# mit-acl/dpgo

Measured on AMD Instinct MI355X. Metric: rbcd_iterations_per_sec, higher is better.
Workload: dtype f64; 1 GPU; synthetic 3-D grid 50x50x40 (100000 poses, 293500 edges), init = perturbed truth; agents=1, agents_per_gpu=1, r=5, d=3, schedule=single agent, poses_per_agent=100000, nnzb_per_agent=687000

## Files before the change

### dpgo_amd/csrc/host.h

```cpp
#pragma once
#include "kernels.h"

#include <algorithm>
#include <atomic>
#include <chrono>
#include <condition_variable>
#include <functional>
#include <memory>
#include <pthread.h>
#include <sched.h>
#include <mutex>
#include <thread>
#include <cmath>
#include <cstdio>
#include <cstdlib>
#include <cstring>
#include <string>
#include <utility>
#include <vector>

#include "../../include/dpgo_hip.h"

using namespace dpgo;

namespace dpgo_host {


inline thread_local std::string g_err;

inline int fail(int code, const std::string& msg) {
  g_err = msg;
  return code;
}

#define HIPC(expr)                                                                              \
  do {                                                                                          \
    hipError_t e_ = (expr);                                                                     \
    if (e_ != hipSuccess)                                                                       \
      return fail(DPGO_ERR_HIP, std::string(#expr) + ": " + hipGetErrorString(e_) + " (" + __FILE__ + \
                                    ":" + std::to_string(__LINE__) + ")");                      \
  } while (0)

#define CHK(expr)                \
  do {                           \
    int rc_ = (expr);            \
    if (rc_ != DPGO_OK) return rc_; \
  } while (0)

#define DPGO_FOR_DR(M) M(2, 2) M(2, 3) M(2, 4) M(2, 5) M(3, 3) M(3, 4) M(3, 5) M(3, 6)

inline bool supported(int d, int r) {
#define M(dd, rr) \
  if (d == dd && r == rr) return true;
  DPGO_FOR_DR(M)
#undef M
  return false;
}

#define DPGO_CASE(dd, rr, ...)   \
  case (dd) * 16 + (rr): {       \
    constexpr int D = dd, R = rr; \
    __VA_ARGS__;                 \
  } break;
#define DISPATCH(d, r, ...)                                                                         \
  switch ((d) * 16 + (r)) {                                                                         \
    DPGO_CASE(2, 2, __VA_ARGS__) DPGO_CASE(2, 3, __VA_ARGS__) DPGO_CASE(2, 4, __VA_ARGS__)          \
    DPGO_CASE(2, 5, __VA_ARGS__) DPGO_CASE(3, 3, __VA_ARGS__) DPGO_CASE(3, 4, __VA_ARGS__)          \
    DPGO_CASE(3, 5, __VA_ARGS__) DPGO_CASE(3, 6, __VA_ARGS__)                                       \
    default:                                                                                        \
      return fail(DPGO_ERR_UNSUPPORTED, "unsupported (d, r)");                                      \
  }

#define LAUNCH_SPLIT(p, KERNEL, GRID, ...)                                                            \
  do {                                                                                                \
    if ((p)->split == 4)                                                                              \
      hipLaunchKernelGGL((KERNEL<D, R, 4>), dim3(GRID), dim3(kBlock), 0, (p)->stream, __VA_ARGS__);   \
    else if ((p)->split == 2)                                                                         \
      hipLaunchKernelGGL((KERNEL<D, R, 2>), dim3(GRID), dim3(kBlock), 0, (p)->stream, __VA_ARGS__);   \
    else                                                                                              \
      hipLaunchKernelGGL((KERNEL<D, R, 1>), dim3(GRID), dim3(kBlock), 0, (p)->stream, __VA_ARGS__);   \
  } while (0)

inline bool aligned8(const void* q) { return ((uintptr_t)q & 7) == 0; }
inline bool aligned16(const void* q) { return ((uintptr_t)q & 15) == 0; }

struct Bsr {
  int nrows = 0, ncols = 0, nnzb = 0;
  int32_t* rowptr = nullptr;
  int32_t* colidx = nullptr;
  double* vals = nullptr;
  BsrDev dev() const { return BsrDev{rowptr, colidx, vals}; }
};

inline int free_bsr(Bsr& m) {
  if (m.rowptr) HIPC(hipFree(m.rowptr));
  if (m.colidx) HIPC(hipFree(m.colidx));
  if (m.vals) HIPC(hipFree(m.vals));
  m = Bsr();
  return DPGO_OK;
}



#define DPGO_OPTIONS(X)                                                                                                  \
  X(split,             "DPGO_SPLIT",              0,  "lane groups per pose of the SpMM-family kernels: 1, 2, 4 (0: by size)")       \
  X(spmm_symmetric,    "DPGO_SPMM_SYMMETRIC",    -1,  "symmetric storage of Q for blocks beyond the Infinity Cache: 0 / 1")          \
  X(stream_nt,         "DPGO_STREAM_NT",         -1,  "non-temporal single-use operands in the tCG-step kernels: 0 / 1")             \
  X(outer_sym,         "DPGO_OUTER_SYM",          1,  "outer RTR iteration (k_grad / k_hess) reads the symmetric copy when tCG does") \
  X(tile_walk,         "DPGO_TILE_WALK",          1,  "symmetric-storage kernels walk each XCD's tiles breadth-first over the tile graph (0: index order)") \
  X(iter_graph,        "DPGO_ITER_GRAPH",         0,  "steady tCG iterations replayed from an instantiated hipGraph (measured slower)") \
  X(tcg_ahead,         "DPGO_TCG_AHEAD",          0,  "iterations the just-in-time feed stays ahead (0: 2 multilevel / 4 otherwise)") \
  X(grid_update,       "DPGO_GRID_UPDATE",        0,  "launch cap of k_tcg_update (0: resident count)")                              \
  X(grid_hess,         "DPGO_GRID_HESS",          0,  "launch cap of k_tcg_hess (0: resident count)")                                \
  X(grid_hess_sym,     "DPGO_GRID_HESS_SYM",      0,  "launch cap of k_tcg_hess_sym (0: resident count)")                            \
  X(grid_retract,      "DPGO_GRID_RETRACT",       0,  "launch cap of k_retract (0: 1024)")                                           \
  X(grid_outer_sym,    "DPGO_GRID_OUTER_SYM",     0,  "launch cap of k_grad / k_hess on the symmetric storage (0: resident count)")  \
  X(grid_spmm_sym,     "DPGO_GRID_SPMM_SYM",      0,  "launch cap of k_spmm_sym (0: resident count, at most 1024)")                  \
  X(grid_ml,           "DPGO_GRID_ML",            0,  "launch cap of the level-0 restriction / post-smoothing (0: resident count)")  \
  X(persist,           "DPGO_PERSIST",           -1,  "one-launch solve (k_rtr_persist) off / on whatever the size: 0 / 1")          \
  X(persist_max_poses, "DPGO_PERSIST_MAX_POSES",  0,  "largest block the one-launch solve takes (0: every block it can hold)")       \
  X(persist_split,     "DPGO_PERSIST_SPLIT",      0,  "lane groups per pose of the one-launch solve: 1, 4 (0: by size)")             \
  X(persist_mt,        "DPGO_PERSIST_MT",         0,  "tiles per workgroup of the one-launch solve: 1, 2 (0: by size)")              \
  X(additive_tiles,    "DPGO_ADDITIVE_TILES",     1,  "workgroup tiles per aggregate of the additive one-launch solve: 1, 2 (opt-in: blocks up to ~28 000 poses)") \
  X(poll_first,        "DPGO_POLL_FIRST",        -1,  "s_sleep units before the first sweep of the in-kernel all-reduce")            \
  X(poll_sleep,        "DPGO_POLL_SLEEP",        -1,  "s_sleep units between sweeps of the in-kernel all-reduce")                    \
  X(poll_first_pay,    "DPGO_POLL_FIRST_PAY",    -1,  "the same before the first sweep of a reduction that carries a payload")       \
  X(persist_verbose,   "DPGO_PERSIST_VERBOSE",    0,  "per-solve phase report of the one-launch solve on stderr")                    \
  X(hess_dma,          "DPGO_HESS_DMA",           0,  "k_tcg_hess_sym's own tiles by LDS-DMA: 1 = double-buffered, 2 waves / SIMD, 4 blocks in flight; 2 = 3 waves, 2 blocks") \
  X(setup_timing,      "DPGO_SETUP_TIMING",       0,  "section times of the hierarchy's symbolic set-up on stderr")                  \
  X(setup_threads,     "DPGO_SETUP_THREADS",      0,  "host threads of the hierarchy's symbolic set-up (0: min(8, cores); 1: serial)") \
  X(setup_pin,         "DPGO_SETUP_PIN",          1,  "set-up worker threads placed in the CPU group of the thread that first used them") \
  X(auto_cost_rule,    "DPGO_AUTO_COST_RULE",     1,  "DPGO_PRECOND_AUTO on coupled blocks: cost rule (0: tCG-budget hysteresis only)") \
  X(ml_graph,          "DPGO_ML_GRAPH",           1,  "graph aggregates in the default hierarchy (0: index runs)")                   \
  X(ml_graph_size,     "DPGO_ML_GRAPH_SIZE",      0,  "growth size of the default graph aggregates (0: by size)")                    \
  X(ml_growth_chunks,  "DPGO_ML_GROWTH_CHUNKS",   0,  "index ranges the graph aggregates grow and merge in (0: 8 from 65 536 poses, else 1)") \
  X(ml_ap,             "DPGO_ML_AP",              1,  "two-level post-smoothing through A P (0: gather through Q; index runs only)") \
  X(ml_dense_sym,      "DPGO_ML_DENSE_SYM",      -1,  "dense level from the packed lower triangle on the matrix cores: 0 / 1")       \
  X(ml_early_stop,     "DPGO_ML_EARLY_STOP",      1,  "tCG's residual test in the restriction kernel, one kernel early")             \
  X(ml_operator_bits,  "DPGO_ML_OPERATOR_BITS",   0,  "level-0 operator copies of the cycle on HBM-bound blocks: 32 / 64 (0: 32)")   \
  X(ml_vector_bits,    "DPGO_ML_VECTOR_BITS",     0,  "cycle-internal vectors (pre-smoothed iterate, kept residual) beside fp32 operator copies: 32 / 64 (0: 32)") \
  X(ml_dense_bits,     "DPGO_ML_DENSE_BITS",      0,  "dense level beside fp32 cycle vectors: 32 / 64 (0: 64 -- fp32 measured neutral)") \
  X(ml_setup_serial,   "DPGO_ML_SETUP_SERIAL",    0,  "one-thread-per-aggregate set-up kernels of round 3")                          \
  X(gj_mfma,           "DPGO_GJ_MFMA",            1,  "rank-64 updates of the dense inverse on the fp64 matrix cores")               \
  X(dense_chunk,       "DPGO_DENSE_CHUNK",        0,  "tiles per workgroup of k_dense_sym_apply (0: default)")                       \
  X(coarse_nodes,      "DPGO_COARSE_NODES",       0,  "nodes per workgroup of k_ml_coarse_prolong: 1-4 (0: by size)")                \
  X(coarse_grid,       "DPGO_COARSE_GRID",        0,  "launch cap of k_ml_coarse_prolong (0: default)")                              \
  X(coarse_nt,         "DPGO_COARSE_NT",         -1,  "non-temporal loads of the dense inverse: 0 / 1")
struct Options {
#define X(field, var, unset, text) int field = unset;
  DPGO_OPTIONS(X)
#undef X
};
inline Options& options_storage() {
  static Options o;
  return o;
}
inline void options_read(Options& o) {
  o = Options();
#define X(field, var, unset, text) \
  if (const char* e_ = std::getenv(var)) o.field = (*e_ == 0) ? 1 : std::atoi(e_);
  DPGO_OPTIONS(X)
#undef X
}
inline const Options& options() {
  static const bool once = (options_read(options_storage()), true);
  (void)once;
  return options_storage();
}
inline std::string options_describe() {
  const Options& o = options();
  std::string s;
#define X(field, var, unset, text) s += std::string(var) + "=" + std::to_string(o.field) + (o.field == (unset) ? "" : " [set]") + "  # " + text + "\n";
  DPGO_OPTIONS(X)
#undef X
  return s;
}

}
using namespace dpgo_host;

struct dpgo_problem_s {
  int r = 0, d = 0, n = 0, b = 0, T = 0;
  int device = 0;
  hipStream_t own_stream = nullptr;
  hipStream_t stream = nullptr;
  Bsr Q;
  Bsr C;
  double* G0 = nullptr;
  double* G = nullptr;
  bool has_G = false;
  double* dinv = nullptr;
  double dinv_shift = -1.0;
  double *x1 = nullptr, *x2 = nullptr, *g1 = nullptr, *g2 = nullptr, *eta = nullptr, *delta = nullptr,
         *Hd = nullptr, *rr = nullptr, *z = nullptr, *S1 = nullptr, *S2 = nullptr;
  struct MlLevel {
    int n = 0;
    int k = 0;
    int split = 1;
    Bsr A;
    int32_t* slot_row = nullptr;
    double *dinv = nullptr, *Pb = nullptr;
    double *r = nullptr, *x1 = nullptr, *x = nullptr;
    Bsr AP;
    double* res1 = nullptr;
    bool graph = false;
    int32_t *lab = nullptr, *agg_ptr = nullptr, *agg_mem = nullptr, *parent = nullptr, *pslot = nullptr;
    int32_t* mem_pos = nullptr;
    int32_t *seg_info = nullptr, *seg_ptr = nullptr;
    int nseg = 0;
    int32_t* tile_perm = nullptr;
    int perm_tile = 0;
    int merge_cap = 0;
    double* tbuf = nullptr;
    float *Pb32 = nullptr, *AP32 = nullptr;
    float *x1f = nullptr, *res1f = nullptr;
    AggMap agg() const { return AggMap{graph ? lab : nullptr, k}; }
  };
  std::vector<MlLevel> ml;
  std::vector<int32_t> h_rowptr, h_colidx;
  bool ml_symbolic = false, ml_ready = false, ml_user_ks = false;
  bool ml_additive_layout = false;
  struct AddPlan {
    int split = 0, tile = 0, S = 0, cap = 0, na = 0;
    bool graph = true;
  } add_plan;
  bool add_plan_known = false;
  int add_tiles = 0;
  struct AggCache {
    int S = 0, cap = 0;
    std::vector<int32_t> lab, ptr, mem, parent, pslot;
  } add_agg;
  double ml_omega = 0.7, ml_shift = 1e-1;
  double* ml_dense = nullptr;
  float* ml_dense32 = nullptr;
  double *ml_packed = nullptr, *ml_pd = nullptr, *ml_pt = nullptr;
  DenseChunk* ml_chunks = nullptr;
  int* ml_chunk_first = nullptr;
  int ml_nchunks = 0;
  bool ml_use_dense_sym() const {
    const int env = options().ml_dense_sym;
    if (!ml_use_ap() || ml_coarse_bits != 64 || !ml_packed || env == 0) return false;
    return env == 1 || ml_lda >= 3072;
  }
  int ml_coarse_bits = 64;
  int ml_operator_bits = 32;
  bool ml_ops32_ready = false;
  bool ml_ops32_suspend = false;
  bool ml_ops32_wanted() const { return ml_operator_bits == 32 && tcg_sym && split == 1 && ml_use_ap() && sym.uvalsT != nullptr; }
  bool ml_ops32_active() const { return !ml_ops32_suspend && ml_ops32_wanted() && ml_ops32_ready; }
  bool ml_vec32_active() const { return ml_ops32_active() && options().ml_vector_bits != 64; }
  bool coarse32_active() const {
    return ml_coarse_bits == 32 || (ml_vec32_active() && !ml_use_dense_sym() && options().ml_dense_bits == 32);
  }
  int ml_lda = 0;
  double *ml_W = nullptr, *ml_Rx = nullptr;
  bool auto_ml = false, auto_decided = false;
  struct AutoCost {
    long long jac_units = 0;
    int ref = 0;
    int state = 0;
    int backoff = 0;
    int switches = 0;
    int last_used = -1, last_products = 0;
    int uj = 10, ua = 18;
  } auto_cost;
  void auto_decide() {
    if (!auto_decided) {
      auto_ml = !(has_G || C.nnzb > 0);
      auto_decided = true;
      auto_cost = AutoCost();
    }
  }
  bool ml_use_ap() const {
    const bool off = options().ml_ap == 0;
    return ml.size() == 2 && ml[0].AP.vals != nullptr && (!off || ml[0].graph);
  }
  struct SymQ {
    int nu = 0, nl = 0;
    int32_t *urow = nullptr, *ucol = nullptr, *usrc = nullptr, *lrow = nullptr, *lcol = nullptr, *lslot = nullptr,
            *lsrc = nullptr;
    double* uvalsT = nullptr;
    float* uvalsT32 = nullptr;
    int32_t* tord = nullptr;
    int* flag = nullptr;
    bool symbolic = false;
    bool pattern_ok = false;
    bool ready = false;
    bool values_ok = false;
    BsrSymDev dev() const { return BsrSymDev{urow, ucol, uvalsT, lrow, lcol, lslot, tord}; }
    BsrSymDev32 dev32() const { return BsrSymDev32{urow, ucol, uvalsT32, lrow, lcol, lslot, tord}; }
  } sym;
  int spmm_variant = DPGO_SPMM_AUTO;
  bool tcg_sym = false;
  int cap_hs = kMaxGrid;
  bool sym_wanted() const {
    if (spmm_variant == DPGO_SPMM_PLAIN || split != 1) return false;
    if (spmm_variant == DPGO_SPMM_SYMMETRIC) return true;
    if (options().spmm_symmetric >= 0) return options().spmm_symmetric != 0;
    return beyond_cache();
  }
  size_t loop_extra_bytes = 0;
  bool want_stream_nt() const {
    return options().stream_nt >= 0 ? options().stream_nt != 0 : beyond_cache();
  }
  bool beyond_cache() const {
    return sizeof(double) * ((size_t)Q.nnzb * b * b + 8 * (size_t)n * T) + sizeof(int32_t) * (size_t)Q.nnzb + loop_extra_bytes >
           ((size_t)256 << 20);
  }
  bool persist = false;
  int persist_share = 1;
  int persist_wgs = 0, persist_split = 0, persist_mt = 0;
  int persist_reserved = 0;
  bool persist_failed_once = false;
  bool stream_nt = false;
  bool persist_add = false;
  bool persist_stream_ordered = false;
  struct Pending {
    bool active = false;
    bool launched = false;
    dpgo_ropt_params resolved{};
    bool is_auto = false;
    const double* dinv = nullptr;
    double* own_x1 = nullptr;
    double* staged_x = nullptr;
    std::chrono::steady_clock::time_point t0;
    dpgo_ropt_result result{};
  } pending;
  PersistCtrl* pctrl = nullptr;
  bool pctrl_dirty = true;
  unsigned long long* pgran = nullptr;
  unsigned gran_cleared_at = 0;
  PersistCtrl* hctrl = nullptr;
  double* partials = nullptr;
  DevState* dstate = nullptr;
  DevState* hstate = nullptr;
  unsigned long long* hflag = nullptr;
  unsigned gen = 0;
  bool saw_rtr_stop = false;
  struct IterGraph {
    hipGraphExec_t exec = nullptr;
    unsigned long long key = 0;
  } iter_graph[2];
  bool capturing = false;
  bool iter_graph_failed = false;
  unsigned launch_gen() const { return capturing ? 0u : gen; }
  int em = 0;
  int32_t *e_p1 = nullptr, *e_p2 = nullptr, *c_ptr = nullptr, *c_edge = nullptr;
  double *e_R = nullptr, *e_t = nullptr, *e_kappa = nullptr, *e_tau = nullptr, *e_w = nullptr, *e_rsq = nullptr,
         *q_base = nullptr;
  uint8_t *e_fixed = nullptr, *c_kind = nullptr, *e_role = nullptr;
  int32_t* e_slot = nullptr;
  int32_t *g_ptr = nullptr, *g_edge = nullptr;
  uint8_t* g_kind = nullptr;
  double* c_base = nullptr;
  int n_shared_edges = 0;
  int* e_counts = nullptr;
  EdgeDev edges() const {
    return EdgeDev{e_p1, e_p2, e_R, e_t, e_kappa, e_tau, e_fixed, e_role, e_slot, e_w, e_rsq, em};
  }
  int cur = 0;
  size_t vec_bytes() const { return (size_t)n * T * sizeof(double); }
  double* pE() const { return partials; }
  double* pA() const { return partials + 1 * kPartialCap * kNP; }
  double* pB() const { return partials + 2 * kPartialCap * kNP; }
  double* pH() const { return partials + 3 * kPartialCap * kNP; }
  int grid() const {
    const int P = (64 / b) * kWaves;
    int tiles = (n + P - 1) / P;
    if (tiles < 1) tiles = 1;
    return tiles < cap_u ? tiles : cap_u;
  }
  int cap_u = kMaxGrid, cap_h = kMaxGrid;
  int cap_u_ml = kMaxGrid;
  int grid_u(bool ml_mode) const {
    const int P = (64 / b) * kWaves;
    const int tiles = std::max(1, (n + P - 1) / P);
    return std::min(tiles, ml_mode ? cap_u_ml : cap_u);
  }
  bool zr_from_post = false;
  int nb_zr() const { return zr_from_post ? grid_post() : grid(); }
  int split = 1;
  int grid_s() const {
    const int P = (64 / (b * split)) * kWaves;
    int tiles = (n + P - 1) / P;
    if (tiles < 1) tiles = 1;
    const int cap = tcg_sym ? cap_hs : cap_h;
    return tiles < cap ? tiles : cap;
  }
  int cap_restrict = kMaxGrid, cap_post = kMaxGrid;
  int grid_tiles(int cap) const {
    const int P = (64 / (b * split)) * kWaves;
    int tiles = (n + P - 1) / P;
    if (tiles < 1) tiles = 1;
    return tiles < cap ? tiles : cap;
  }
  int grid_restrict() const { return grid_tiles(cap_restrict); }
  int grid_post() const { return grid_tiles(cap_post); }
  int cap_outer_sym = kMaxGrid;
  int nb_grad = 0, nb_hess = 0;
  int grid_outer_sym() const {
    const int P = (64 / b) * kWaves;
    const int tiles = std::max(1, (n + P - 1) / P);
    return std::min(tiles, cap_outer_sym);
  }
  int cap_spmm_sym = kMaxGrid;
  int grid_spmm_sym() const {
    const int P = (64 / b) * kWaves;
    const int tiles = std::max(1, (n + P - 1) / P);
    return std::min(tiles, cap_spmm_sym);
  }
  int grid_spmm() const {
    const int P = (64 / (b * split)) * kWaves;
    int tiles = (n + P - 1) / P;
    if (tiles < 1) tiles = 1;
    return tiles < kMaxGrid ? tiles : kMaxGrid;
  }
  int grid_flat() const {
    size_t total = (size_t)n * T;
    size_t g = (total + kBlock - 1) / kBlock;
    if (g < 1) g = 1;
    return g < (size_t)kMaxGrid ? (int)g : kMaxGrid;
  }
};

namespace dpgo_host {

struct Counters {
  int spmm = 0;
  bool vcycle_for_additive = false;
};

template <class Tp>
inline int upload(Tp** dst, const Tp* src, size_t count, hipStream_t s) {
  HIPC(hipMalloc(dst, sizeof(Tp) * (count > 0 ? count : 1)));
  if (count > 0) HIPC(hipMemcpyAsync(*dst, src, sizeof(Tp) * count, hipMemcpyHostToDevice, s));
  return DPGO_OK;
}

class TaskPool {
 public:
  struct Batch {
    std::function<void(int)> fn;
    int count = 0;
    std::atomic<int> next{0}, done{0};
  };
  using Job = std::shared_ptr<Batch>;
  static TaskPool& get() {
    static TaskPool* pool = new TaskPool();
    return *pool;
  }
  Job submit(int count, std::function<void(int)> fn, int max_threads) {
    Job b = std::make_shared<Batch>();
    b->fn = std::move(fn);
    b->count = count;
    const int helpers = std::max(0, std::min(count, max_threads - 1));
    if (helpers > 0) {
      {
        std::lock_guard<std::mutex> lk(mu_);
        while ((int)nworkers_ < std::min(kMaxWorkers, std::max(helpers, (int)nworkers_))) {
          const int id = (int)nworkers_;
          std::thread([this, id] {
            pin(id);
            loop();
          }).detach();
          ++nworkers_;
        }
        for (int k = 0; k < helpers; ++k) queue_.push_back(b);
      }
      cv_.notify_all();
    }
    return b;
  }
  void wait(const Job& b) {
    if (!b) return;
    help(*b);
    while (b->done.load(std::memory_order_acquire) < b->count) std::this_thread::yield();
  }
  void run(int count, const std::function<void(int)>& fn, int max_threads) {
    if (count <= 0) return;
    if (count == 1 || max_threads <= 1) {
      for (int k = 0; k < count; ++k) fn(k);
      return;
    }
    wait(submit(count, fn, max_threads));
  }
  void warm(int threads) {
    bool expected = false;
    if (threads <= 1 || !warmed_.compare_exchange_strong(expected, true)) return;
    std::thread([this, threads] { wait(submit(threads - 1, [](int) {}, threads)); }).detach();
  }

 private:
  static constexpr int kMaxWorkers = 15;
  int home_cpu_ = -1;
  void pin(int) {
    if (!pin_enabled() || home_cpu_ < 0) return;
    cpu_set_t allowed, want;
    CPU_ZERO(&allowed);
    CPU_ZERO(&want);
    if (sched_getaffinity(0, sizeof(allowed), &allowed) != 0) return;
    const int lo = home_cpu_ & ~7;
    int cnt = 0;
    for (int c = lo; c < lo + 8; ++c)
      if (c < CPU_SETSIZE && CPU_ISSET(c, &allowed)) CPU_SET(c, &want), ++cnt;
    if (cnt >= 2) (void)pthread_setaffinity_np(pthread_self(), sizeof(want), &want);
  }
  static bool pin_enabled() { return options().setup_pin != 0; }
  TaskPool() { home_cpu_ = sched_getcpu(); }
  static void help(Batch& b) {
    for (;;) {
      const int k = b.next.fetch_add(1, std::memory_order_relaxed);
      if (k >= b.count) return;
      b.fn(k);
      b.done.fetch_add(1, std::memory_order_release);
    }
  }
  void loop() {
    for (;;) {
      Job b;
      {
        std::unique_lock<std::mutex> lk(mu_);
        cv_.wait(lk, [this] { return !queue_.empty(); });
        b = std::move(queue_.front());
        queue_.erase(queue_.begin());
      }
      help(*b);
    }
  }
  std::mutex mu_;
  std::condition_variable cv_;
  std::vector<Job> queue_;
  unsigned nworkers_ = 0;
  std::atomic<bool> warmed_{false};
};
struct JobGuard {
  TaskPool::Job job;
  ~JobGuard() { TaskPool::get().wait(job); }
};

struct TmpDev {
  std::vector<void*> ptrs;
  ~TmpDev() {
    for (auto q : ptrs) (void)hipFree(q);
  }
  int alloc(double** out, size_t bytes) {
    HIPC(hipMalloc(out, bytes));
    ptrs.push_back(*out);
    return DPGO_OK;
  }
};

template <typename T>
inline int sym_upload(T** dst, const std::vector<T>& v, hipStream_t stream) {
  HIPC(hipMalloc(dst, sizeof(T) * std::max<size_t>(1, v.size())));
  if (!v.empty()) HIPC(hipMemcpyAsync(*dst, v.data(), sizeof(T) * v.size(), hipMemcpyHostToDevice, stream));
  return DPGO_OK;
}

struct PersistGeo {
  int split = 0, mt = 0, wgs = 0, slots = 0;
};

enum { RUN_FULL = 0, RUN_BEGIN = 1, RUN_END = 2 };

int set_device(dpgo_problem_s* p);
int upload_bsr(Bsr& m, int nrows, int ncols, int nnzb, int b, const int32_t* rowptr, const int32_t* colidx,
               const double* vals, hipStream_t s);
int validate_bsr(int nrows, int ncols, int nnzb, const int32_t* rowptr, const int32_t* colidx, bool need_diag);
int build_dinv(dpgo_problem_s* p, double shift);
int poll_state(dpgo_problem_s* p);
int push_state(dpgo_problem_s* p);
void sym_free(dpgo_problem_s* p);
int sym_symbolic_setup(dpgo_problem_s* p);
int sym_ensure(dpgo_problem_s* p, bool* usable);
int launch_spmm_sym(dpgo_problem_s* p, const BsrSymDev& M, const double* V, const double* Gadd, double* OUT);
int launch_spmm(dpgo_problem_s* p, const Bsr& M, const double* V, const double* Gadd, double* OUT, int nrows = -1,
                bool plain_only = false);
bool outer_sym_enabled();
int launch_grad(dpgo_problem_s* p, const double* X, double* RG, double* S, double* EG,
                const DevState* st = nullptr, bool sym = false);
int launch_hess(dpgo_problem_s* p, const double* X, const double* S, const double* V, const double* Gdot,
                double* HV, double* partials, const DevState* st, int check_tcg, bool sym = false);
int launch_retract(dpgo_problem_s* p, const double* X, const double* eta, double scale, double* X2,
                   const DevState* st);
int launch_rtr_update(dpgo_problem_s* p);
int launch_precond(dpgo_problem_s* p, const double* X, const double* V, const double* dinv, double* Z);
int launch_rtr_begin(dpgo_problem_s* p, double tol, double Delta0, double Dmax, int max_inner, int tiny);
int check_ready(dpgo_problem_s* p);
int h2d(dpgo_problem_s* p, double* dst, const double* src);
int d2h(dpgo_problem_s* p, double* dst, const double* src);

int ml_tile(int b, int split);
int additive_tile(const dpgo_problem_s* p);
int ml_level_split(int n);
int ml_default_graph_size(int n, int b);
std::vector<int> ml_default_ks(int n, int b, int split0);
void ml_free(dpgo_problem_s* p);
int ml_graph_aggregates(const std::vector<int32_t>& rowptr, const std::vector<int32_t>& colidx, int n, int S,
                        std::vector<int32_t>& lab, std::vector<int32_t>& ptr, std::vector<int32_t>& mem,
                        std::vector<int32_t>& parent, std::vector<int32_t>& pslot);
int ml_merge_small_aggregates(const std::vector<int32_t>& rowptr, const std::vector<int32_t>& colidx, int n, int S, int cap,
                              std::vector<int32_t>& lab, std::vector<int32_t>& ptr, std::vector<int32_t>& mem,
                              std::vector<int32_t>& parent, std::vector<int32_t>& pslot);
int ml_symbolic_setup(dpgo_problem_s* p, const std::vector<int>& ks_in, int perm_tile = 0);
int setup_threads();
int flat_grid(size_t items);
bool gj_use_mfma();
int dense_spd_inverse(hipStream_t s, double* M, int lda, double* W, double* Rx, bool mfma);
int ml_numeric_setup(dpgo_problem_s* p);
std::vector<int> ml_current_ks(const dpgo_problem_s* p);
const dpgo_problem_s::AddPlan& additive_plan(dpgo_problem_s* p);
int additive_split_of(const dpgo_problem_s* p);
int additive_tiles(const dpgo_problem_s* p);
int additive_mt_of(const dpgo_problem_s* p);
int ml_ensure(dpgo_problem_s* p, double shift, bool additive = false);
int ml_ops32_ensure(dpgo_problem_s* p);
int persist_capacity(int device);
int launch_coarse_prolong(dpgo_problem_s* p, const dpgo_problem_s::MlLevel& L, const dpgo_problem_s::MlLevel& C,
                          const DevState* gate, double* xc_out = nullptr);
int launch_dense_sym(dpgo_problem_s* p, const dpgo_problem_s::MlLevel& C, const DevState* gate);
int launch_ml_restrict0(dpgo_problem_s* p, const double* r, const DevState* gate, int g0, bool stop_check = false);
int launch_ml_post_ap(dpgo_problem_s* p, const double* Xdev, const double* r, double* z, double* pout, const DevState* gate);
int launch_ml_tail(dpgo_problem_s* p, const double* Xdev, const double* r, double* z, double* pout,
                   const DevState* gate, bool stop_check = false);
int launch_ml_apply(dpgo_problem_s* p, const double* Xdev, const double* v, double* z);

int launch_tcg_update(dpgo_problem_s* p, const double* dinv, int first, double* z_out = nullptr,
                      double ml_omega = 0.0);
int launch_tcg_hess(dpgo_problem_s* p, int first);
int launch_tcg_hess_with(dpgo_problem_s* p, const DevState* sin, DevState* sout, int first, unsigned long long* hflag,
                         unsigned gen);
int resolve_tcg_storage(dpgo_problem_s* p);
int persist_capacity(int device);
bool persist_reserve(dpgo_problem_s* p, int slots, int limit);
void persist_release(dpgo_problem_s* p);
bool additive_available(dpgo_problem_s* p);
PersistGeo persist_geometry(const dpgo_problem_s* p, int free_slots, int share = 1, bool additive = false);
bool additive_lds_fits(const dpgo_problem_s* p, int split, int mt, int na);
int launch_rtr_persistent(dpgo_problem_s* p, const dpgo_ropt_params* prm, const double* dinv, bool* used, bool additive);
void persist_report(dpgo_problem_s* p);
int rtr_outer_iteration(dpgo_problem_s* p, const dpgo_ropt_params* prm, const double* dinv, Counters& cnt,
                        bool poll_at_end);
int auto_units_jacobi(dpgo_problem_s* p);
int auto_units_additive(dpgo_problem_s* p);
void auto_update(dpgo_problem_s* p, const dpgo_ropt_params* prm, int used, int products);
int run_optimize(dpgo_problem_s* p, const dpgo_ropt_params* prm, dpgo_ropt_result* res, int phase = RUN_FULL);
int tune_launch_caps(dpgo_problem_s* p);
int tune_persist(dpgo_problem_s* p);

int free_edges(dpgo_problem_s* p);
int rebuild_vals(dpgo_problem_s* p, int nnzb, const int32_t* cptr, const int32_t* cedge, const uint8_t* ckind,
                 const double* base, double sign, double* out);
int rebuild_Q_from_weights(dpgo_problem_s* p, const double* base, double sign, double* out);
int rebuild_C_from_weights(dpgo_problem_s* p, const double* base, double sign, double* out);
int refresh_after_weights(dpgo_problem_s* p);

}
```

### dpgo_amd/csrc/kernels/multilevel.h

```cpp
#pragma once


struct AggMap {
  const int32_t* lab;
  int k;
  __device__ __forceinline__ int of(int i) const { return lab ? lab[i] : i / k; }
};

template <int D, int R>
__global__ __launch_bounds__(kBlock) void k_ml_presmooth(const double* __restrict__ V, const double* __restrict__ dinv,
                                                         double omega, double* __restrict__ OUT,
                                                         const DevState* __restrict__ gate, int n) {
  using GEO = Geo<D, R>;
  if (gate && (gate->tcg_done || gate->rtr_stop)) return;
  __shared__ double sm[kWaves][GEO::G][GEO::T];
  const LaneId L = lane_id<D>();
  const int ntiles = (n + GEO::P - 1) / GEO::P;
  const TileIter ti_ = tile_iter(ntiles);
  for (int tile = ti_.first; tile < ti_.last; tile += ti_.step) {
    const int i = tile * GEO::P + L.wave * GEO::G + L.g;
    const bool ok = (L.g < GEO::G) && (i < n);
    const size_t off = (size_t)i * GEO::T + L.c * R;
    double* vs = ok ? &sm[L.wave][L.g][0] : nullptr;
    double v[R], z[R];
    if (ok) {
      load_col<R>(V + off, v);
      store_col<R>(vs + L.c * R, v);
    }
    wave_sync();
    if (ok) {
      jacobi_col<D, R>(vs, dinv + (size_t)i * GEO::BB + L.c * GEO::B, z);
#pragma unroll
      for (int a = 0; a < R; ++a) z[a] *= omega;
      store_col<R>(OUT + off, z);
    }
    wave_sync();
  }
}

struct TcgStopCheck {
  DevState* state = nullptr;
  const double* pin = nullptr;
  int nb = 0;
  unsigned long long* hflag = nullptr;
  unsigned gen = 0;
};
template <int D, int R, int SPLIT>
struct RestrictWaves {
  static constexpr int kMin = (SPLIT == 1 && D == 3 && R <= 5) ? DPGO_RESTRICT_WAVES : 1;
};
template <int D, int R, int SPLIT, class MAT = BsrDev, class PT = double, class XT = double>
__global__ __launch_bounds__(kBlock) __attribute__((amdgpu_waves_per_eu(RestrictWaves<D, R, SPLIT>::kMin, 8))) void k_ml_restrict(MAT A, const XT* __restrict__ x1,
                                                        const double* __restrict__ r, const PT* __restrict__ Pb,
                                                        double shift, int k, double* __restrict__ rc,
                                                        float* __restrict__ rc32,
                                                        const double* __restrict__ dinv_next, double omega,
                                                        double* __restrict__ x1c, const DevState* gate,
                                                        int n, XT* __restrict__ res_out = nullptr,
                                                        double* __restrict__ tbuf = nullptr,
                                                        const int32_t* __restrict__ tpos = nullptr,
                                                        TcgStopCheck stop = TcgStopCheck()) {
  using GEO = Geo<D, R, SPLIT>;
  DPGO_TL_TILES_DECL;
  if (gate && (gate->tcg_done || gate->rtr_stop)) return;
  DPGO_STAMP_ENTRY_IN(g_tl_restrict);
  __shared__ double res_s[kWaves][GEO::G][GEO::T];
  __shared__ double t_s[GEO::P][GEO::T];
  const LaneId L = lane_id<D, SPLIT>();
  const int ntiles = (n + GEO::P - 1) / GEO::P;
  const TileIter ti_ = tile_iter(ntiles);
  if (stop.state && blockIdx.x == gridDim.x - 1) {
    double rr_sum[1];
    load_partials<1>(stop.pin, stop.nb, rr_sum, &t_s[0][0]);
    if (threadIdx.x == 0) {
      const DevState* st = stop.state;
      const double norm_r = sqrt(rr_sum[0]), nr0 = st->norm_r0, theta = st->theta, kappa = st->kappa;
      const double pw = (theta == 1.0) ? nr0 : pow(nr0, theta);
      const int j = st->tcg_j;
      if (j >= st->min_inner && norm_r <= nr0 * (pw < kappa ? pw : kappa)) {
        stop.state->tcg_status = (kappa < pw) ? TCG_LCON : TCG_SCON;
        stop.state->tcg_done = 1;
        if (stop.hflag) {
          const unsigned g_ = stop.gen ? stop.gen : (unsigned)st->pad0;
          const unsigned long long w = ((unsigned long long)g_ << 32) |
                                       ((unsigned long long)((unsigned)j & 0xFFFFFFu) << 8) | 1ull;
          __hip_atomic_store(stop.hflag, w, __ATOMIC_RELAXED, __HIP_MEMORY_SCOPE_SYSTEM);
        }
      }
    }
    __syncthreads();
  }
  DPGO_STAMP_AT_IN(g_tl_restrict, 1);
  for (int tk = ti_.first; tk < ti_.last; tk += ti_.step) {
    DPGO_STAMP_TILE_IN(g_tl_restrict, 0);
    const int tile = tile_of(A, tk);
    const int lp = L.wave * GEO::G + L.g;
    const int i = tile * GEO::P + lp;
    const bool okp = (L.g < GEO::G) && (i < n);
    const bool ok = okp && (L.s == 0);
    const size_t off = (size_t)i * GEO::T + L.c * R;
    double h[R];
    q_gather<D, R, SPLIT>(A, x1, i, L.s, L.c, okp, h);
    DPGO_TL_USE(h[0]);
    DPGO_STAMP_TILE_IN(g_tl_restrict, 1);
    if constexpr (SPLIT == 1 && Span<D, R, 1>::kOk && DPGO_CYCLE_SPAN) {
      const int p0 = tile * GEO::P + L.wave * GEO::G;
      const int npose = (n - p0) < GEO::G ? (n - p0) : GEO::G;
      const int valid = npose > 0 ? npose * GEO::T : 0;
      const size_t base = (size_t)p0 * GEO::T;
      double* rw = &res_s[L.wave][0][0];
      span_to_lds<D, R>(r + base, rw, valid);
      span_to_lds<D, R>(x1 + base, &t_s[L.wave * GEO::G][0], valid);
      wave_sync();
      if (ok) {
        const double* rr = &res_s[L.wave][L.g][L.c * R];
        const double* xr = &t_s[lp][L.c * R];
#pragma unroll
        for (int a = 0; a < R; ++a) h[a] = rr[a] - h[a] - shift * xr[a];
        store_col<R>(&res_s[L.wave][L.g][L.c * R], h);
      }
      wave_sync();
      if (res_out) span_from_lds<D, R>(res_out + base, rw, valid);
    } else {
      if (ok) {
        XT xr[R];
        double rr[R];
#pragma unroll
        for (int a = 0; a < R; ++a) xr[a] = x1[off + a];
        load_col<R>(r + off, rr);
#pragma unroll
        for (int a = 0; a < R; ++a) h[a] = rr[a] - h[a] - shift * (double)xr[a];
        store_col<R>(&res_s[L.wave][L.g][L.c * R], h);
        if (res_out) store_col_t<R>(res_out + off, h);
      }
      wave_sync();
    }
    DPGO_STAMP_TILE_IN(g_tl_restrict, 2);
    if (L.s == 0 && L.g < GEO::G) {
      double t[R];
#pragma unroll
      for (int a = 0; a < R; ++a) t[a] = 0.0;
      if (ok) {
        const PT* __restrict__ pb = Pb + (size_t)i * GEO::BB;
#pragma unroll
        for (int cc = 0; cc < GEO::B; ++cc) {
          const double pv = (double)pb[cc * GEO::B + L.c];
#pragma unroll
          for (int a = 0; a < R; ++a) t[a] = fma(pv, res_s[L.wave][L.g][cc * R + a], t[a]);
        }
      }
      store_col<R>(&t_s[lp][L.c * R], t);
    }
    DPGO_STAMP_TILE_IN(g_tl_restrict, 3);
    if (tbuf) {
      wave_sync();
      if (ok) {
        const int info = tpos[i];
        if (info >= 0) {
          const int len = info & 31;
          double acc[R];
#pragma unroll
          for (int a = 0; a < R; ++a) acc[a] = t_s[lp][L.c * R + a];
          for (int m = 1; m < len; ++m) {
#pragma unroll
            for (int a = 0; a < R; ++a) acc[a] += t_s[lp + m][L.c * R + a];
          }
          store_col<R>(tbuf + (size_t)(info >> 5) * GEO::T + L.c * R, acc);
        }
      }
      wave_sync();
      DPGO_STAMP_TILE_IN(g_tl_restrict, 4);
      DPGO_TILE_NEXT;
      continue;
    }
    __syncthreads();
    const int mstep = (k >= 16) ? 8 : 1;
    if (mstep == 8) {
      const int nseg = (k + 7) / 8, nagg = GEO::P / k;
      for (int tsk = threadIdx.x; tsk < nagg * nseg * GEO::T; tsk += kBlock) {
        const int e = tsk % GEO::T, sg = (tsk / GEO::T) % nseg, ag = tsk / (GEO::T * nseg);
        const int row0 = ag * k + sg * 8;
        double sacc = t_s[row0][e];
        for (int m = 1; m < 8 && sg * 8 + m < k; ++m) sacc += t_s[row0 + m][e];
        t_s[row0][e] = sacc;
      }
      __syncthreads();
    }
    const bool head = ok && (i % k) == 0;
    double acc[R];
    if (head) {
#pragma unroll
      for (int a = 0; a < R; ++a) acc[a] = 0.0;
      for (int m = 0; m < k && lp + m < GEO::P; m += mstep) {
#pragma unroll
        for (int a = 0; a < R; ++a) acc[a] += t_s[lp + m][L.c * R + a];
      }
      int cr = L.c * R;
      asm volatile("" : "+v"(cr));
      if (rc32) {
#pragma unroll
        for (int a = 0; a < R; ++a) rc32[(size_t)(i / k) * GEO::T + cr + a] = (float)acc[a];
      } else {
        store_col<R>(rc + (size_t)(i / k) * GEO::T + cr, acc);
      }
    }
    __syncthreads();
    if (dinv_next) {
      if (head) store_col<R>(&t_s[lp][L.c * R], acc);
      wave_sync();
      if (head) {
        double z[R];
        jacobi_col<D, R>(&t_s[lp][0], dinv_next + (size_t)(i / k) * GEO::BB + L.c * GEO::B, z);
#pragma unroll
        for (int a = 0; a < R; ++a) z[a] *= omega;
        store_col<R>(x1c + (size_t)(i / k) * GEO::T + L.c * R, z);
      }
      __syncthreads();
    }
  }
}

template <int D, int R>
__global__ __launch_bounds__(kBlock) void k_ml_agg_sum(const double* __restrict__ t, const int32_t* __restrict__ agg_ptr,
                                                       int na, double* __restrict__ rc, float* __restrict__ rc32,
                                                       const DevState* __restrict__ gate) {
  constexpr int T = (D + 1) * R, NG = kBlock / T;
  if (gate && (gate->tcg_done || gate->rtr_stop)) return;
  __shared__ double part[NG][T];
  const int e = threadIdx.x % T, g = threadIdx.x / T;
  for (int a = blockIdx.x; a < na; a += gridDim.x) {
    const int m0 = agg_ptr[a], m1 = agg_ptr[a + 1];
    if (g < NG) {
      double acc = 0.0;
#pragma unroll 8
      for (int m = m0 + g; m < m1; m += NG) acc += t[(size_t)m * T + e];
      part[g][e] = acc;
    }
    __syncthreads();
    if (threadIdx.x < T) {
      double acc = part[0][threadIdx.x];
#pragma unroll
      for (int q = 1; q < NG; ++q) acc += part[q][threadIdx.x];
      if (rc32)
        rc32[(size_t)a * T + threadIdx.x] = (float)acc;
      else
        rc[(size_t)a * T + threadIdx.x] = acc;
    }
    __syncthreads();
  }
}

#ifndef DPGO_COARSE_WAVES
#define DPGO_COARSE_WAVES 2
#endif
#ifndef DPGO_COARSE_UNROLL
#define DPGO_COARSE_UNROLL 1
#endif
template <int D, int R, int NODES, class MT>
__global__ __launch_bounds__(kBlock) __attribute__((amdgpu_waves_per_eu(DPGO_COARSE_WAVES, DPGO_COARSE_WAVES))) void k_ml_coarse_prolong(const MT* __restrict__ M, int lda,
                                                              const MT* __restrict__ rc,
                                                              const double* __restrict__ x1,
                                                              const double* __restrict__ Pb, int k,
                                                              double* __restrict__ x, const DevState* __restrict__ gate,
                                                              int n, int nc, double* __restrict__ xc_out = nullptr,
                                                              int stream_hint = 1) {
  constexpr int B = D + 1, T = B * R, BB = B * B, NR = NODES * B;
  constexpr int CPL = 16 / (int)sizeof(MT);
  struct alignas(16) Pack {
    MT v[CPL];
  };
  if (gate && (gate->tcg_done || gate->rtr_stop)) return;
  constexpr int NV = B * R, SEG = 8, SEGLEN = kBlock / SEG;
  __shared__ double xc_s[NR][R];
  __shared__ double all_s[NV][kBlock];
  __shared__ double seg_s[NV][SEG];
  const int lane = threadIdx.x & 63, wave = threadIdx.x >> 6;
  const int N = nc * B;
  const int ngroups = (nc + NODES - 1) / NODES;
  for (int grp = blockIdx.x; grp < ngroups; grp += gridDim.x) {
    const int a0 = grp * NODES;
    {
      const MT* __restrict__ m = M + (size_t)(a0 * B) * lda;
      double acc[NR][R];
#pragma unroll
      for (int c = 0; c < NR; ++c)
#pragma unroll
        for (int q = 0; q < R; ++q) acc[c][q] = 0.0;
      const int npack = (N + CPL - 1) / CPL;
      const dbl2* __restrict__ rc2 = reinterpret_cast<const dbl2*>(rc);
      struct alignas(16) RPack {
        MT v[CPL * R];
      };
      auto stream_rows = [&](auto nt) {
#pragma unroll DPGO_COARSE_UNROLL
        for (int j = wave * 64 + lane; j < npack; j += kBlock) {
          Pack mv[NR];
#pragma unroll
          for (int c = 0; c < NR; ++c) {
            const dbl2* src = reinterpret_cast<const dbl2*>(m + (size_t)c * lda + CPL * j);
            dbl2 raw;
            if constexpr (decltype(nt)::value)
              raw = __builtin_nontemporal_load(src);
            else
              raw = *src;
            __builtin_memcpy(&mv[c], &raw, 16);
          }
          RPack rp;
          if (CPL * j + CPL <= N) {
            dbl2 raw[R];
#pragma unroll
            for (int q = 0; q < R; ++q) raw[q] = rc2[(size_t)j * R + q];
            __builtin_memcpy(&rp, raw, sizeof(rp));
          } else {
#pragma unroll
            for (int e = 0; e < CPL * R; ++e)
              rp.v[e] = (CPL * j + e / R < N) ? rc[(size_t)(CPL * j) * R + e] : (MT)0;
          }
          double rv[CPL * R];
#pragma unroll
          for (int e = 0; e < CPL * R; ++e) rv[e] = (double)rp.v[e];
#pragma unroll
          for (int c = 0; c < NR; ++c) {
#pragma unroll
            for (int q = 0; q < R; ++q) {
#pragma unroll
              for (int cc = 0; cc < CPL; ++cc) acc[c][q] = fma((double)mv[c].v[cc], rv[cc * R + q], acc[c][q]);
            }
          }
        }
      };
      if (stream_hint)
        stream_rows(std::true_type{});
      else
        stream_rows(std::false_type{});
#pragma unroll
      for (int nd = 0; nd < NODES; ++nd) {
#pragma unroll
        for (int c = 0; c < B; ++c)
#pragma unroll
          for (int q = 0; q < R; ++q) all_s[c * R + q][threadIdx.x] = acc[nd * B + c][q];
        __syncthreads();
        for (int tsk = threadIdx.x; tsk < NV * SEG; tsk += kBlock) {
          const int v = tsk / SEG, sg = tsk % SEG;
          double sum = 0.0;
#pragma unroll 8
          for (int e = 0; e < SEGLEN; ++e)
            sum += all_s[v][sg * SEGLEN + ((e + tsk) & (SEGLEN - 1))];
          seg_s[v][sg] = sum;
        }
        __syncthreads();
        if (threadIdx.x < NV) {
          double sum = seg_s[threadIdx.x][0];
#pragma unroll
          for (int sg = 1; sg < SEG; ++sg) sum += seg_s[threadIdx.x][sg];
          xc_s[nd * B + threadIdx.x / R][threadIdx.x % R] = sum;
        }
      }
    }
    __syncthreads();
    if (xc_out) {
      if (threadIdx.x < NR * R && a0 * B + threadIdx.x / R < N)
        xc_out[(size_t)(a0 * B) * R + threadIdx.x] = xc_s[threadIdx.x / R][threadIdx.x % R];
      __syncthreads();
      continue;
    }
    for (int tsk = threadIdx.x; tsk < NODES * k * B; tsk += kBlock) {
      const int i = a0 * k + tsk / B, c = tsk % B;
      if (i < n) {
        const int an = (tsk / B) / k;
        const double* __restrict__ pb = Pb + (size_t)i * BB + c * B;
        const size_t off = (size_t)i * T + c * R;
#pragma unroll
        for (int q = 0; q < R; ++q) {
          double v = x1[off + q];
#pragma unroll
          for (int cc = 0; cc < B; ++cc) v = fma(pb[cc], xc_s[an * B + cc][q], v);
          x[off + q] = v;
        }
      }
    }
    __syncthreads();
  }
}

template <int D, int R, int SPLIT>
__global__ __launch_bounds__(kBlock) void k_ml_post_mid(BsrDev A, const double* __restrict__ xv,
                                                        const double* __restrict__ r, const double* __restrict__ dinv,
                                                        double omega, const double* __restrict__ x1f,
                                                        const double* __restrict__ Pbf, int kf, double* __restrict__ xf,
                                                        int nf, const DevState* __restrict__ gate, int n) {
  using GEO = Geo<D, R, SPLIT>;
  if (gate && (gate->tcg_done || gate->rtr_stop)) return;
  __shared__ double sm[kWaves][2][GEO::G][GEO::T];
  const LaneId L = lane_id<D, SPLIT>();
  const int ntiles = (n + GEO::P - 1) / GEO::P;
  const TileIter ti_ = tile_iter(ntiles);
  for (int tile = ti_.first; tile < ti_.last; tile += ti_.step) {
    const int i = tile * GEO::P + L.wave * GEO::G + L.g;
    const bool okp = (L.g < GEO::G) && (i < n);
    const bool ok = okp && (L.s == 0);
    const size_t off = (size_t)i * GEO::T + L.c * R;
    double* vs = ok ? &sm[L.wave][0][L.g][0] : nullptr;
    double* zs = ok ? &sm[L.wave][1][L.g][0] : nullptr;
    double h[R], xr[R], z[R];
    spmm_col<D, R, SPLIT>(A.rowptr, A.colidx, A.vals, xv, i, L.s, L.c, okp, h);
    if (ok) {
      double rr[R];
      load_col<R>(xv + off, xr);
      load_col<R>(r + off, rr);
#pragma unroll
      for (int a = 0; a < R; ++a) h[a] = rr[a] - h[a];
      store_col<R>(vs + L.c * R, h);
    }
    wave_sync();
    if (ok) {
      jacobi_col<D, R>(vs, dinv + (size_t)i * GEO::BB + L.c * GEO::B, z);
#pragma unroll
      for (int a = 0; a < R; ++a) z[a] = fma(omega, z[a], xr[a]);
      store_col<R>(zs + L.c * R, z);
    }
    wave_sync();
    if (ok) {
      for (int m = 0; m < kf; ++m) {
        const int fi = i * kf + m;
        if (fi < nf) {
          const double* __restrict__ pb = Pbf + (size_t)fi * GEO::BB + L.c * GEO::B;
          const size_t foff = (size_t)fi * GEO::T + L.c * R;
          double out[R];
          load_col<R>(x1f + foff, out);
#pragma unroll
          for (int cc = 0; cc < GEO::B; ++cc) {
            const double pv = pb[cc];
#pragma unroll
            for (int a = 0; a < R; ++a) out[a] = fma(pv, zs[cc * R + a], out[a]);
          }
          store_col<R>(xf + foff, out);
        }
      }
    }
    wave_sync();
  }
}

#ifndef DPGO_POST_RR_LDS
#define DPGO_POST_RR_LDS 1
#endif
#ifndef DPGO_POST_WAVES
#define DPGO_POST_WAVES 4
#endif
template <int D, int R, int SPLIT, class MAT = BsrDev>
__global__ __launch_bounds__(kBlock) __attribute__((amdgpu_waves_per_eu(SPLIT == 1 ? DPGO_POST_WAVES : 1))) void k_ml_post(MAT Q, const double* __restrict__ X,
                                                    const double* __restrict__ xv, const double* __restrict__ r,
                                                    const double* __restrict__ dinv, double omega, double shift,
                                                    double* __restrict__ Z, double* __restrict__ pout,
                                                    const DevState* __restrict__ gate, int n) {
  using GEO = Geo<D, R, SPLIT>;
  if (gate && (gate->tcg_done || gate->rtr_stop)) return;
  __shared__ double sm[kWaves][3][GEO::G][GEO::T];
  __shared__ double red[kWaves * kNP];
  const LaneId L = lane_id<D, SPLIT>();
  const int ntiles = (n + GEO::P - 1) / GEO::P;
  const TileIter ti_ = tile_iter(ntiles);
  double part[2] = {0.0, 0.0};
  for (int tk = ti_.first; tk < ti_.last; tk += ti_.step) {
    const int tile = tile_of(Q, tk);
    const int i = tile * GEO::P + L.wave * GEO::G + L.g;
    const bool okp = (L.g < GEO::G) && (i < n);
    const bool ok = okp && (L.s == 0);
    const size_t off = (size_t)i * GEO::T + L.c * R;
    double* ys = ok ? &sm[L.wave][0][L.g][0] : nullptr;
    double* vs = ok ? &sm[L.wave][1][L.g][0] : nullptr;
    double* zs = ok ? &sm[L.wave][2][L.g][0] : nullptr;
    double h[R], xr[R], rr[R], z[R];
    q_gather<D, R, SPLIT>(Q, xv, i, L.s, L.c, okp, h);
    if (ok) {
      double x[R];
      load_col<R>(X + off, x);
      load_col<R>(xv + off, xr);
      load_col<R>(r + off, rr);
#pragma unroll
      for (int a = 0; a < R; ++a) {
        h[a] = rr[a] - h[a] - shift * xr[a];
        part[0] = fma(rr[a], rr[a], part[0]);
      }
      store_col<R>(ys + L.c * R, x);
      store_col<R>(vs + L.c * R, h);
    }
    wave_sync();
    if (ok) {
      jacobi_col<D, R>(vs, dinv + (size_t)i * GEO::BB + L.c * GEO::B, z);
#pragma unroll
      for (int a = 0; a < R; ++a) z[a] = fma(omega, z[a], xr[a]);
      store_col<R>(zs + L.c * R, z);
    }
    wave_sync();
    if (ok) {
      double out[R], s[D];
      proj_col<D, R>(ys, zs, L.c, z, out, s);
      store_col<R>(Z + off, out);
#pragma unroll
      for (int a = 0; a < R; ++a) part[1] = fma(out[a], rr[a], part[1]);
    }
    wave_sync();
  }
  if (pout) store_partials<2>(part, pout, red);
}

template <int D, int R, int SPLIT, class VT = double, class RT = VT>
__global__ __launch_bounds__(kBlock) __attribute__((amdgpu_waves_per_eu(SPLIT == 1 ? DPGO_POST_WAVES : 1))) void k_ml_post_ap(BsrDevT<VT> AP, const double* __restrict__ X,
                                                       const double* __restrict__ r, const RT* __restrict__ res1,
                                                       const double* __restrict__ xc, const VT* __restrict__ Pb, AggMap am,
                                                       const double* __restrict__ dinv, double omega,
                                                       double* __restrict__ Z, double* __restrict__ pout,
                                                       const DevState* __restrict__ gate, int n) {
  using GEO = Geo<D, R, SPLIT>;
  DPGO_TL_TILES_DECL;
  if (gate && (gate->tcg_done || gate->rtr_stop)) return;
  DPGO_STAMP_ENTRY_IN(g_tl_post);
  __shared__ double sm[kWaves][3][GEO::G][GEO::T];
  __shared__ double red[kWaves * kNP];
  const LaneId L = lane_id<D, SPLIT>();
  const int ntiles = (n + GEO::P - 1) / GEO::P;
  const TileIter ti_ = tile_iter(ntiles);
  double part[2] = {0.0, 0.0};
  for (int tile = ti_.first; tile < ti_.last; tile += ti_.step) {
    DPGO_STAMP_TILE_IN(g_tl_post, 0);
    const int i = tile * GEO::P + L.wave * GEO::G + L.g;
    const bool okp = (L.g < GEO::G) && (i < n);
    const bool ok = okp && (L.s == 0);
    const size_t off = (size_t)i * GEO::T + L.c * R;
    double* ys = ok ? &sm[L.wave][0][L.g][0] : nullptr;
    double* vs = ok ? &sm[L.wave][1][L.g][0] : nullptr;
    double* zs = ok ? &sm[L.wave][2][L.g][0] : nullptr;
    double h[R], rr[R], xcol[R], z[R], dr[GEO::B];
    spmm_col<D, R, SPLIT>(AP.rowptr, AP.colidx, AP.vals, xc, i, L.s, L.c, okp, h);
    DPGO_TL_USE(h[0]);
    DPGO_STAMP_TILE_IN(g_tl_post, 1);
    constexpr bool kSpan = (SPLIT == 1) && Span<D, R, 1>::kOk && DPGO_CYCLE_SPAN;
    [[maybe_unused]] int valid = 0;
    [[maybe_unused]] size_t base = 0;
    if constexpr (kSpan) {
      const int p0 = tile * GEO::P + L.wave * GEO::G;
      const int npose = (n - p0) < GEO::G ? (n - p0) : GEO::G;
      valid = npose > 0 ? npose * GEO::T : 0;
      base = (size_t)p0 * GEO::T;
      span_to_lds<D, R>(X + base, &sm[L.wave][0][0][0], valid);
      span_to_lds<D, R>(r + base, &sm[L.wave][1][0][0], valid);
      span_to_lds<D, R>(res1 + base, &sm[L.wave][2][0][0], valid);
      if (ok) {
#pragma unroll
        for (int q = 0; q < GEO::B; ++q) dr[q] = dinv[(size_t)i * GEO::BB + L.c * GEO::B + q];
      }
      wave_sync();
      if (ok) {
#pragma unroll
        for (int a = 0; a < R; ++a) {
          rr[a] = vs[L.c * R + a];
          h[a] = zs[L.c * R + a] - h[a];
          part[0] = fma(rr[a], rr[a], part[0]);
        }
        store_col<R>(zs + L.c * R, h);
      }
    } else if (ok) {
      double x[R], rs[R];
      load_col<R>(X + off, x);
      load_col<R>(r + off, rr);
      load_col_t<R>(res1 + off, rs);
#pragma unroll
      for (int q = 0; q < GEO::B; ++q) dr[q] = dinv[(size_t)i * GEO::BB + L.c * GEO::B + q];
#pragma unroll
      for (int a = 0; a < R; ++a) {
        h[a] = rs[a] - h[a];
        part[0] = fma(rr[a], rr[a], part[0]);
      }
      store_col<R>(ys + L.c * R, x);
      store_col<R>(vs + L.c * R, rr);
      store_col<R>(zs + L.c * R, h);
    }
    wave_sync();
    DPGO_STAMP_TILE_IN(g_tl_post, 2);
    if (ok) {
      double x1c[R], zc[R];
      jacobi_col<D, R>(vs, dr, x1c);
      jacobi_col<D, R>(zs, dr, zc);
      const VT* __restrict__ pb = Pb + (size_t)i * GEO::BB + L.c * GEO::B;
      const double* __restrict__ xa = xc + (size_t)am.of(i) * GEO::T;
#pragma unroll
      for (int a = 0; a < R; ++a) xcol[a] = omega * x1c[a];
#pragma unroll
      for (int cc = 0; cc < GEO::B; ++cc) {
        const double pv = (double)pb[cc];
#pragma unroll
        for (int a = 0; a < R; ++a) xcol[a] = fma(pv, xa[cc * R + a], xcol[a]);
      }
#pragma unroll
      for (int a = 0; a < R; ++a) z[a] = fma(omega, zc[a], xcol[a]);
      DPGO_TL_USE(z[0]);
    }
    DPGO_STAMP_TILE_IN(g_tl_post, 3);
    wave_sync();
    if (ok) store_col<R>(zs + L.c * R, z);
    wave_sync();
    DPGO_STAMP_TILE_IN(g_tl_post, 4);
    if (ok) {
      double out[R], sdummy[D];
      proj_col<D, R>(ys, zs, L.c, z, out, sdummy);
      if constexpr (DPGO_POST_RR_LDS) {
#pragma unroll
        for (int a = 0; a < R; ++a) part[1] = fma(out[a], vs[L.c * R + a], part[1]);
      } else {
#pragma unroll
        for (int a = 0; a < R; ++a) part[1] = fma(out[a], rr[a], part[1]);
      }
      if constexpr (kSpan)
        store_col<R>(vs + L.c * R, out);
      else
        store_col<R>(Z + off, out);
    }
    wave_sync();
// ... 417 lines not shown
```

### dpgo_amd/csrc/multilevel.hip

```cpp
#include "host.h"

namespace dpgo_host {

int ml_tile(int b, int split) { return (64 / (b * split)) * kWaves; }
int additive_tile(const dpgo_problem_s* p) { return ml_tile(p->b, 4); }
int ml_level_split(int n) { return n < 40000 ? 4 : 1; }

constexpr int kMlDense = 3200, kMlDenseMax = 6400;
constexpr int kMlGraphMax = 512, kMlGraphUnknownsPerPose = 1600;
int ml_default_graph_size(int n, int b) {
  if (options().ml_graph == 0) return 0;
  if (options().ml_graph_size >= 2) return options().ml_graph_size;
  const long long S = std::max<long long>(4, ((long long)n * b + kMlGraphUnknownsPerPose - 1) / kMlGraphUnknownsPerPose);
  return S <= kMlGraphMax ? (int)S : 0;
}
constexpr int kMlMergeFrom = 12, kMlMergedUnknownsPerPose = 2200;
std::vector<int> ml_default_ks(int n, int b, int split0) {
  if (const int S = ml_default_graph_size(n, b)) {
    const bool forced = options().ml_graph_size >= 2;
    if (!forced && S >= kMlMergeFrom) {
      const int Sm = (int)(((long long)n * b + kMlMergedUnknownsPerPose - 1) / kMlMergedUnknownsPerPose);
      const int cap = Sm + Sm / 2;
      if (cap <= kMlGraphMax) return std::vector<int>{-Sm, -cap};
    }
    return std::vector<int>{-S};
  }
  std::vector<int> ks;
  int cur = n, split = split0;
  for (int guard = 0; guard < 16; ++guard) {
    const int P = ml_tile(b, split);
    int pick = 0;
    for (int limit : {kMlDense, kMlDenseMax}) {
      for (int k = 4; k <= P && !pick; ++k)
        if (P % k == 0 && (long long)((cur + k - 1) / k) * b <= limit) pick = k;
      if (pick) break;
    }
    if (pick) {
      ks.push_back(pick);
      return ks;
    }
    int k = 2;
    for (int c = 2; c <= 8; ++c)
      if (P % c == 0) k = c;
    ks.push_back(k);
    cur = (cur + k - 1) / k;
    split = ml_level_split(cur);
  }
  return ks;
}

void ml_free(dpgo_problem_s* p) {
  p->ml_additive_layout = false;
  for (auto& L : p->ml) {
    free_bsr(L.A);
    free_bsr(L.AP);
    void* ptrs[] = {L.slot_row, L.dinv, L.Pb, L.r, L.x1, L.x, L.res1, L.lab, L.agg_ptr, L.agg_mem, L.parent, L.pslot, L.tbuf, L.tile_perm, L.mem_pos,
                    L.seg_info, L.seg_ptr, L.Pb32, L.AP32, L.x1f, L.res1f};
    for (void* q : ptrs)
      if (q) (void)hipFree(q);
  }
  p->ml.clear();
  void* ptrs[] = {p->ml_dense, p->ml_W, p->ml_Rx, p->ml_dense32, p->ml_packed, p->ml_pd, p->ml_pt, p->ml_chunks,
                  p->ml_chunk_first};
  for (void* q : ptrs)
    if (q) (void)hipFree(q);
  p->ml_dense = p->ml_W = p->ml_Rx = nullptr;
  p->ml_dense32 = nullptr;
  p->ml_packed = p->ml_pd = p->ml_pt = nullptr;
  p->ml_chunks = nullptr;
  p->ml_chunk_first = nullptr;
  p->ml_nchunks = 0;
  p->ml_lda = 0;
  p->ml_symbolic = p->ml_ready = false;
  p->ml_ops32_ready = false;
}

int ml_growth_chunks(int n) {
  const int forced = options().ml_growth_chunks;
  if (forced > 0) return std::max(1, std::min(forced, std::max(1, n / 64)));
  return n >= 65536 ? 8 : 1;
}
namespace {
int grow_range(const std::vector<int32_t>& rowptr, const std::vector<int32_t>& colidx, int lo, int hi, int S,
               std::vector<int32_t>& lab, std::vector<int32_t>& ptr, std::vector<int32_t>& mem,
               std::vector<int32_t>& parent, std::vector<int32_t>& pslot) {
  mem.clear();
  mem.reserve(hi - lo);
  ptr.assign(1, 0);
  int na = 0;
  for (int s = lo; s < hi; ++s) {
    if (lab[s] >= 0) continue;
    const size_t first = mem.size();
    lab[s] = na;
    mem.push_back(s);
    for (size_t head = first; head < mem.size() && (int)(mem.size() - first) < S; ++head) {
      const int u = mem[head];
      for (int t = rowptr[u]; t < rowptr[u + 1] && (int)(mem.size() - first) < S; ++t) {
        const int v = colidx[t];
        if (v < lo || v >= hi || lab[v] >= 0) continue;
        lab[v] = na;
        parent[v] = u;
        pslot[v] = t;
        mem.push_back(v);
      }
    }
    ptr.push_back((int32_t)mem.size());
    ++na;
  }
  return na;
}

int merge_range(const std::vector<int32_t>& rowptr, const std::vector<int32_t>& colidx, int lo, int hi, int S, int cap,
                std::vector<int32_t>& lab, std::vector<int32_t>& ptr, std::vector<int32_t>& mem,
                std::vector<int32_t>& parent, std::vector<int32_t>& pslot) {
  const int na = (int)ptr.size() - 1;
  const int n = hi - lo;
  std::vector<std::vector<int32_t>> members(na);
  for (int a = 0; a < na; ++a) members[a].assign(mem.begin() + ptr[a], mem.begin() + ptr[a + 1]);
  std::vector<int> cnt(na, 0);
  std::vector<int> touched;
  for (bool changed = true; changed;) {
    changed = false;
    for (int a = 0; a < na; ++a) {
      if (members[a].empty() || 2 * (int)members[a].size() > S) continue;
      touched.clear();
      for (int i : members[a])
        for (int t = rowptr[i]; t < rowptr[i + 1]; ++t) {
          const int v = colidx[t];
          if (v < lo || v >= hi) continue;
          const int c = lab[v];
          if (c == a) continue;
          if (cnt[c]++ == 0) touched.push_back(c);
        }
      std::sort(touched.begin(), touched.end());
      int best = -1, best_n = 0;
      for (int c : touched) {
        if ((int)(members[c].size() + members[a].size()) <= cap && cnt[c] > best_n) best = c, best_n = cnt[c];
        cnt[c] = 0;
      }
      if (best >= 0) {
        members[best].insert(members[best].end(), members[a].begin(), members[a].end());
        for (int i : members[a]) lab[i] = best;
        members[a].clear();
        changed = true;
      }
    }
  }
  std::vector<char> grew(na, 0);
  for (int a = 0; a < na; ++a)
    if (!members[a].empty() && (int)members[a].size() != ptr[a + 1] - ptr[a]) grew[a] = 1;
  std::vector<int32_t> first_member(na, -1);
  for (int i = hi - 1; i >= lo; --i) first_member[lab[i]] = i;
  std::vector<int> alive;
  for (int a = 0; a < na; ++a)
    if (!members[a].empty()) alive.push_back(a);
  std::sort(alive.begin(), alive.end(), [&](int x, int y) { return first_member[x] < first_member[y]; });
  std::vector<int32_t> sorted_mem, sorted_ptr(na + 1, 0);
  {
    for (int a = 0; a < na; ++a) sorted_ptr[a + 1] = sorted_ptr[a] + (grew[a] ? (int32_t)members[a].size() : 0);
    sorted_mem.resize(sorted_ptr[na]);
    std::vector<int32_t> fill(sorted_ptr.begin(), sorted_ptr.end() - 1);
    for (int i = lo; i < hi; ++i)
      if (grew[lab[i]]) sorted_mem[fill[lab[i]]++] = i;
  }
  std::vector<int32_t> new_lab(n, -1), new_mem;
  std::vector<int32_t> old_parent(parent.begin() + lo, parent.begin() + hi), old_pslot(pslot.begin() + lo, pslot.begin() + hi);
  std::fill(parent.begin() + lo, parent.begin() + hi, -1);
  std::fill(pslot.begin() + lo, pslot.begin() + hi, 0);
  new_mem.reserve(n);
  std::vector<int32_t> new_ptr(1, 0);
  for (size_t k = 0; k < alive.size(); ++k) {
    const int a = alive[k];
    if (!grew[a]) {
      for (int m = ptr[a]; m < ptr[a + 1]; ++m) {
        const int v = mem[m];
        new_lab[v - lo] = (int32_t)k;
        parent[v] = old_parent[v - lo];
        pslot[v] = old_pslot[v - lo];
        new_mem.push_back(v);
      }
      new_ptr.push_back((int32_t)new_mem.size());
      continue;
    }
    for (int q = sorted_ptr[a]; q < sorted_ptr[a + 1]; ++q) {
      const int root = sorted_mem[q];
      if (new_lab[root - lo] >= 0) continue;
      size_t head = new_mem.size();
      new_lab[root - lo] = (int32_t)k;
      new_mem.push_back(root);
      for (; head < new_mem.size(); ++head) {
        const int u = new_mem[head];
        for (int t = rowptr[u]; t < rowptr[u + 1]; ++t) {
          const int v = colidx[t];
          if (v < lo || v >= hi || lab[v] != a || new_lab[v - lo] >= 0) continue;
          new_lab[v - lo] = (int32_t)k;
          parent[v] = u;
          pslot[v] = t;
          new_mem.push_back(v);
        }
      }
    }
    new_ptr.push_back((int32_t)new_mem.size());
  }
  mem.swap(new_mem);
  ptr.swap(new_ptr);
  std::copy(new_lab.begin(), new_lab.end(), lab.begin() + lo);
  return (int)alive.size();
}
}

template <class F>
void parallel_ranges(int n, int chunks, F&& fn);
int setup_threads();

int ml_grow_and_merge(const std::vector<int32_t>& rowptr, const std::vector<int32_t>& colidx, int n, int S, int cap,
                      bool do_grow, std::vector<int32_t>& lab, std::vector<int32_t>& ptr, std::vector<int32_t>& mem,
                      std::vector<int32_t>& parent, std::vector<int32_t>& pslot, int chunks) {
  chunks = std::max(1, std::min(chunks, std::max(1, n)));
  if (do_grow) {
    lab.assign(n, -1);
    parent.assign(n, -1);
    pslot.assign(n, 0);
  }
  struct Part {
    std::vector<int32_t> ptr, mem;
    int na = 0;
  };
  std::vector<Part> parts(chunks);
  auto bound = [&](int c) { return (int)((long long)n * c / chunks); };
  if (!do_grow) {
    const int na_in = (int)ptr.size() - 1;
    std::vector<int> first_agg(chunks + 1, na_in);
    bool split_ok = chunks > 1;
    if (split_ok) {
      int c = 0;
      first_agg[0] = 0;
      for (int a = 0; a < na_in && split_ok; ++a) {
        if (ptr[a + 1] <= ptr[a]) { split_ok = false; break; }
        int lo_m = n, hi_m = -1;
        for (int m = ptr[a]; m < ptr[a + 1]; ++m) lo_m = std::min(lo_m, (int)mem[m]), hi_m = std::max(hi_m, (int)mem[m]);
        while (c + 1 < chunks && lo_m >= bound(c + 1)) first_agg[++c] = a;
        if (lo_m < bound(c) || hi_m >= bound(c + 1)) split_ok = false;
      }
      while (c + 1 < chunks) first_agg[++c] = na_in;
      first_agg[chunks] = na_in;
    }
    if (!split_ok) {
      chunks = 1;
      parts.resize(1);
      parts[0].ptr = ptr;
      parts[0].mem = mem;
      parts[0].na = na_in;
    } else {
      for (int c = 0; c < chunks; ++c) {
        const int a0 = first_agg[c], a1 = first_agg[c + 1];
        Part& P = parts[c];
        P.na = a1 - a0;
        P.ptr.assign(1, 0);
        for (int a = a0; a < a1; ++a) P.ptr.push_back(ptr[a + 1] - ptr[a0]);
        P.mem.assign(mem.begin() + ptr[a0], mem.begin() + ptr[a1]);
        if (a0 > 0)
          for (int i = bound(c); i < bound(c + 1); ++i) lab[i] -= a0;
      }
    }
  }
  const bool timing_ = options().setup_timing > 1;
  const auto tA = std::chrono::steady_clock::now();
  std::vector<double> tch(chunks, 0.0);
  parallel_ranges(chunks, std::min(chunks, setup_threads()), [&](int, int c0, int c1) {
    for (int c = c0; c < c1; ++c) {
      const auto t0 = std::chrono::steady_clock::now();
      Part& P = parts[c];
      const int lo = bound(c), hi = bound(c + 1);
      if (do_grow) P.na = grow_range(rowptr, colidx, lo, hi, S, lab, P.ptr, P.mem, parent, pslot);
      if (cap > 0) P.na = merge_range(rowptr, colidx, lo, hi, S, cap, lab, P.ptr, P.mem, parent, pslot);
      tch[c] = 1e3 * std::chrono::duration<double>(std::chrono::steady_clock::now() - t0).count();
    }
  });
  const auto tB = std::chrono::steady_clock::now();
  std::vector<int> agg_off(chunks + 1, 0);
  std::vector<size_t> mem_off(chunks + 1, 0);
  for (int c = 0; c < chunks; ++c) agg_off[c + 1] = agg_off[c] + parts[c].na, mem_off[c + 1] = mem_off[c] + parts[c].mem.size();
  const int na = agg_off[chunks];
  mem.resize(mem_off[chunks]);
  ptr.assign((size_t)na + 1, 0);
  parallel_ranges(chunks, std::min(chunks, setup_threads()), [&](int, int c0, int c1) {
    for (int c = c0; c < c1; ++c) {
      const Part& P = parts[c];
      if (agg_off[c] > 0)
        for (int i = bound(c); i < bound(c + 1); ++i) lab[i] += agg_off[c];
      for (int a = 0; a < P.na; ++a) ptr[(size_t)agg_off[c] + a + 1] = (int32_t)(mem_off[c] + P.ptr[a + 1]);
      if (!P.mem.empty()) std::memcpy(mem.data() + mem_off[c], P.mem.data(), sizeof(int32_t) * P.mem.size());
    }
  });
  if (timing_) {
    std::fprintf(stderr, "dpgo_hip: grow / merge (%d ranges): parallel section %.3f ms, join %.3f ms; per range:", chunks,
                 1e3 * std::chrono::duration<double>(tB - tA).count(),
                 1e3 * std::chrono::duration<double>(std::chrono::steady_clock::now() - tB).count());
    for (double t : tch) std::fprintf(stderr, " %.3f", t);
    std::fprintf(stderr, "\n");
  }
  return na;
}
int ml_graph_aggregates(const std::vector<int32_t>& rowptr, const std::vector<int32_t>& colidx, int n, int S,
                        std::vector<int32_t>& lab, std::vector<int32_t>& ptr, std::vector<int32_t>& mem,
                        std::vector<int32_t>& parent, std::vector<int32_t>& pslot) {
  return ml_grow_and_merge(rowptr, colidx, n, S, 0, true, lab, ptr, mem, parent, pslot, ml_growth_chunks(n));
}
int ml_merge_small_aggregates(const std::vector<int32_t>& rowptr, const std::vector<int32_t>& colidx, int n, int S, int cap,
                              std::vector<int32_t>& lab, std::vector<int32_t>& ptr, std::vector<int32_t>& mem,
                              std::vector<int32_t>& parent, std::vector<int32_t>& pslot) {
  return ml_grow_and_merge(rowptr, colidx, n, S, cap, false, lab, ptr, mem, parent, pslot, ml_growth_chunks(n));
}

int setup_threads() {
  const int want = options().setup_threads;
  if (want > 0) return std::min(want, 64);
  const unsigned hw = std::thread::hardware_concurrency();
  return (int)std::max(1u, std::min(8u, hw ? hw : 1u));
}
template <class F>
void parallel_ranges(int n, int chunks, F&& fn) {
  chunks = std::max(1, std::min(chunks, n > 0 ? n : 1));
  TaskPool::get().run(chunks, [&](int c) {
    fn(c, (int)((long long)n * c / chunks), (int)((long long)n * (c + 1) / chunks));
  }, setup_threads());
}
template <class F>
void pattern_by_ranges(int n, int threads, int grain, size_t reserve_hint, F&& row, std::vector<int32_t>& rowptr_out,
                       std::vector<int32_t>& col_out) {
  const int chunks = std::max(1, std::min(threads, n / grain + 1));
  std::vector<std::vector<int32_t>> cols(chunks), cnt(chunks);
  parallel_ranges(n, chunks, [&](int c, int lo, int hi) {
    auto& cc = cols[c];
    auto& nn = cnt[c];
    cc.reserve(reserve_hint / chunks + 16);
    nn.resize(hi - lo);
    for (int i = lo; i < hi; ++i) {
      const size_t first = cc.size();
      row(c, i, cc);
      nn[i - lo] = (int32_t)(cc.size() - first);
    }
  });
  rowptr_out.assign(n + 1, 0);
  size_t total = 0;
  for (auto& cc : cols) total += cc.size();
  col_out.resize(total);
  std::vector<size_t> base(chunks + 1, 0);
  for (int c = 0; c < chunks; ++c) base[c + 1] = base[c] + cols[c].size();
  parallel_ranges(chunks, chunks, [&](int, int c0, int c1) {
    for (int c = c0; c < c1; ++c) {
      const int lo = (int)((long long)n * c / chunks);
      if (!cols[c].empty()) std::memcpy(col_out.data() + base[c], cols[c].data(), sizeof(int32_t) * cols[c].size());
      size_t at = base[c];
      for (size_t k = 0; k < cnt[c].size(); ++k) {
        at += cnt[c][k];
        rowptr_out[lo + k + 1] = (int32_t)at;
      }
    }
  });
}

void ml_ap_pattern(const std::vector<int32_t>& rowptr, const std::vector<int32_t>& colidx, const std::vector<int32_t>& lab,
                   int n, std::vector<int32_t>& arow, std::vector<int32_t>& acol) {
  pattern_by_ranges(n, setup_threads(), 1024, colidx.size(), [&](int, int i, std::vector<int32_t>& out) {
    const size_t first = out.size();
    for (int t = rowptr[i]; t < rowptr[i + 1]; ++t) out.push_back(lab[colidx[t]]);
    std::sort(out.begin() + first, out.end());
    out.erase(std::unique(out.begin() + first, out.end()), out.end());
  }, arow, acol);
}

int ml_run_table(const std::vector<int32_t>& lab, int n, int na, int G, std::vector<int32_t>& seg_info,
                 std::vector<int32_t>& seg_ptr) {
  seg_info.assign(n, -1);
  seg_ptr.assign(na + 1, 0);
  int nruns = 0;
  for (int i = 0; i < n;) {
    int j = i + 1;
    while (j < n && j % G != 0 && lab[j] == lab[i]) ++j;
    seg_info[i] = j - i;
    seg_ptr[lab[i] + 1] += 1;
    ++nruns;
    i = j;
  }
  for (int a = 0; a < na; ++a) seg_ptr[a + 1] += seg_ptr[a];
  std::vector<int32_t> next(seg_ptr.begin(), seg_ptr.end() - 1);
  for (int i = 0; i < n;) {
    const int len = seg_info[i];
    seg_info[i] = len + 32 * next[lab[i]]++;
    i += len;
  }
  return nruns;
}

int ml_symbolic_setup(dpgo_problem_s* p, const std::vector<int>& ks_in, int perm_tile) {
  const bool timing = options().setup_timing != 0;
  auto t_last = std::chrono::steady_clock::now();
  const auto t_first = t_last;
  auto lap = [&](const char* what) {
    if (!timing) return;
    const auto t = std::chrono::steady_clock::now();
    std::fprintf(stderr, "dpgo_hip: symbolic set-up: %-44s %7.3f ms\n", what, 1e3 * std::chrono::duration<double>(t - t_last).count());
    t_last = t;
  };
  ml_free(p);
  lap("previous hierarchy freed");
  if ((int)p->h_rowptr.size() != p->n + 1) return fail(DPGO_ERR_STATE, "multilevel: Q's block pattern is not set");
  const int b = p->b, bb = b * b;
  const size_t tb = sizeof(double) * p->T;
  std::vector<int32_t> rowptr = p->h_rowptr, colidx = p->h_colidx;
  int cur = p->n;
  const bool merged = ks_in.size() == 2 && ks_in[0] < 0 && ks_in[1] < 0;
  const bool graph = (ks_in.size() == 1 && ks_in[0] < 0) || merged;
  std::vector<int> ks = ks_in;
  if (merged) ks.pop_back();
  if (graph) ks[0] = -ks_in[0];
  const int merge_cap = merged ? -ks_in[1] : 0;
  if (merged && merge_cap < ks[0]) return fail(DPGO_ERR_INVALID, "multilevel: the merge bound is at least the growth size");
  for (int k : ks)
    if (k < 0) return fail(DPGO_ERR_INVALID, "multilevel: graph aggregates (a negative size) make a two-level hierarchy");
  p->ml.resize(ks.size() + 1);
  for (size_t l = 0; l <= ks.size(); ++l) {
    auto& L = p->ml[l];
    L.n = cur;
    L.split = (l == 0) ? p->split : ml_level_split(cur);
    L.k = (l < ks.size()) ? ks[l] : 0;
    if (l == 0 && graph) {
      if (L.k < 2) return fail(DPGO_ERR_INVALID, "multilevel: graph aggregates hold at least 2 poses");
      std::vector<int32_t> lab, ptr, mem, parent, pslot;
      int na;
      hipError_t alloc_err = hipSuccess;
      const int dev_ = p->device;
      const int nthreads = setup_threads();
      JobGuard alloc_job{TaskPool::get().submit(1, [&, dev_](int) {
        hipError_t e = hipSetDevice(dev_);
        if (e == hipSuccess) e = hipMalloc(&L.tbuf, tb * cur);
        if (e == hipSuccess) e = hipMalloc(&L.res1, tb * cur);
        if (e == hipSuccess) e = hipMalloc(&L.Pb, sizeof(double) * (size_t)cur * bb);
        if (e == hipSuccess) e = hipMalloc(&L.x1, tb * cur);
        if (e == hipSuccess) e = hipMalloc(&L.x, tb * cur);
        alloc_err = e;
      }, nthreads)};
      if (p->add_plan_known && p->add_agg.S == L.k && p->add_agg.cap == merge_cap && (int)p->add_agg.lab.size() == cur) {
        const auto& A = p->add_agg;
        lab = A.lab, ptr = A.ptr, mem = A.mem, parent = A.parent, pslot = A.pslot;
        na = (int)ptr.size() - 1;
      } else {
        na = ml_graph_aggregates(rowptr, colidx, cur, L.k, lab, ptr, mem, parent, pslot);
        lap("greedy growth of the aggregates");
        if (merge_cap) na = ml_merge_small_aggregates(rowptr, colidx, cur, L.k, merge_cap, lab, ptr, mem, parent, pslot);
        lap("merge of the growth's fragments");
      }
      L.graph = true;
      L.merge_cap = merge_cap;
      std::vector<int32_t> arow, acol, crow, ccol;
      JobGuard pattern_job{TaskPool::get().submit(2, [&](int which) {
        if (which == 0) {
          ml_ap_pattern(rowptr, colidx, lab, cur, arow, acol);
          return;
        }
        const int chunks = std::max(1, std::min(std::max(1, nthreads / 2), na / 16 + 1));
        std::vector<std::vector<int32_t>> marks(chunks);
        pattern_by_ranges(na, chunks, 16, colidx.size() / 8, [&](int c, int a, std::vector<int32_t>& out) {
          auto& mark = marks[c];
          if (mark.empty()) mark.assign(na, -1);
          const size_t first = out.size();
          for (int m = ptr[a]; m < ptr[a + 1]; ++m) {
            const int i = mem[m];
            for (int t = rowptr[i]; t < rowptr[i + 1]; ++t) {
              const int cl = lab[colidx[t]];
              if (mark[cl] != a) {
                mark[cl] = a;
                out.push_back(cl);
              }
            }
          }
          std::sort(out.begin() + first, out.end());
        }, crow, ccol);
      }, nthreads)};
      CHK(upload(&L.lab, lab.data(), lab.size(), p->stream));
      CHK(upload(&L.agg_ptr, ptr.data(), ptr.size(), p->stream));
      CHK(upload(&L.agg_mem, mem.data(), mem.size(), p->stream));
      CHK(upload(&L.parent, parent.data(), parent.size(), p->stream));
      CHK(upload(&L.pslot, pslot.data(), pslot.size(), p->stream));
      std::vector<int32_t> mpos(cur);
      for (int m = 0; m < cur; ++m) mpos[mem[m]] = m;
      CHK(upload(&L.mem_pos, mpos.data(), mpos.size(), p->stream));
      lap("labels, members, trees uploaded");
      std::vector<int32_t> seg_info, seg_ptr;
      L.nseg = ml_run_table(lab, cur, na, 64 / (b * L.split), seg_info, seg_ptr);
      CHK(upload(&L.seg_info, seg_info.data(), seg_info.size(), p->stream));
      CHK(upload(&L.seg_ptr, seg_ptr.data(), seg_ptr.size(), p->stream));
      std::vector<int32_t> tperm;
      if (!perm_tile && !merge_cap && L.k == additive_tile(p)) perm_tile = L.k;
      if (perm_tile) {
        if (std::max(L.k, merge_cap) > perm_tile) return fail(DPGO_ERR_INVALID, "multilevel: aggregates larger than the tile");
        tperm.assign((size_t)na * perm_tile, -1);
        for (int a = 0; a < na; ++a)
          for (int m = ptr[a]; m < ptr[a + 1]; ++m) tperm[(size_t)a * perm_tile + (m - ptr[a])] = mem[m];
        CHK(upload(&L.tile_perm, tperm.data(), tperm.size(), p->stream));
        L.perm_tile = perm_tile;
      }
      lap("run table, tile table");
      TaskPool::get().wait(pattern_job.job);
      lap("patterns of A P and of the dense level joined");
      CHK(upload_bsr(L.AP, cur, na, (int)acol.size(), b, arow.data(), acol.data(), nullptr, p->stream));
      lap("A P allocated, pattern uploaded");
      TaskPool::get().wait(alloc_job.job);
      if (alloc_err != hipSuccess) return fail(DPGO_ERR_HIP, std::string("hipMalloc (level-0 buffers): ") + hipGetErrorString(alloc_err));
      lap("level-0 vectors joined");
      HIPC(hipStreamSynchronize(p->stream));
      lap("stream synchronised");
      rowptr.swap(crow);
      colidx.swap(ccol);
      cur = na;
      continue;
    }
    if (L.k) {
      if (L.k < 2 || ml_tile(b, L.split) % L.k)
        return fail(DPGO_ERR_INVALID, "multilevel: aggregate size must divide the workgroup tile of its level (" +
                                          std::to_string(ml_tile(b, L.split)) + " nodes)");
    }
    if (l > 0) {
      CHK(upload_bsr(L.A, cur, cur, (int)colidx.size(), b, rowptr.data(), colidx.data(), nullptr, p->stream));
      std::vector<int32_t> srow(colidx.size());
      for (int i = 0; i < cur; ++i)
        for (int t = rowptr[i]; t < rowptr[i + 1]; ++t) srow[t] = i;
      CHK(upload(&L.slot_row, srow.data(), srow.size(), p->stream));
      HIPC(hipStreamSynchronize(p->stream));
      HIPC(hipMalloc(&L.r, tb * cur));
      if (!L.k) HIPC(hipMalloc(&L.x, tb * cur));
    }
    if (l == 0 && L.k) {
      const int k = L.k;
      std::vector<int32_t> arow(cur + 1, 0), acol;
      acol.reserve(colidx.size());
      for (int i = 0; i < cur; ++i) {
        const size_t first = acol.size();
        for (int t = rowptr[i]; t < rowptr[i + 1]; ++t) acol.push_back(colidx[t] / k);
        std::sort(acol.begin() + first, acol.end());
        acol.erase(std::unique(acol.begin() + first, acol.end()), acol.end());
        arow[i + 1] = (int32_t)acol.size();
      }
      CHK(upload_bsr(L.AP, cur, (cur + k - 1) / k, (int)acol.size(), b, arow.data(), acol.data(), nullptr, p->stream));
      HIPC(hipMalloc(&L.res1, tb * cur));
    }
    if (L.k) {
      if (l > 0) HIPC(hipMalloc(&L.dinv, sizeof(double) * (size_t)cur * bb));
      HIPC(hipMalloc(&L.Pb, sizeof(double) * (size_t)cur * bb));
      HIPC(hipMalloc(&L.x1, tb * cur));
      HIPC(hipMalloc(&L.x, tb * cur));
      const int k = L.k, nc = (cur + k - 1) / k;
      std::vector<int32_t> crow(nc + 1, 0), ccol;
      std::vector<int32_t> mark(nc, -1);
      for (int a = 0; a < nc; ++a) {
        const size_t first = ccol.size();
        for (int i = a * k; i < std::min(cur, a * k + k); ++i)
          for (int t = rowptr[i]; t < rowptr[i + 1]; ++t) {
            const int c = colidx[t] / k;
            if (mark[c] != a) {
              mark[c] = a;
              ccol.push_back(c);
            }
          }
        std::sort(ccol.begin() + first, ccol.end());
        crow[a + 1] = (int32_t)ccol.size();
      }
      rowptr.swap(crow);
      colidx.swap(ccol);
      cur = nc;
    }
  }
  const int N = cur * b;
  if (N > 16384) return fail(DPGO_ERR_INVALID, "multilevel: dense coarsest operator too large (" + std::to_string(N) +
                                                   " unknowns): use more levels / larger aggregates");
  p->ml_lda = ((N + kNB - 1) / kNB) * kNB;
  HIPC(hipMalloc(&p->ml_dense, sizeof(double) * (size_t)p->ml_lda * (p->ml_lda + 8)));
  HIPC(hipMalloc(&p->ml_dense32, sizeof(float) * (size_t)p->ml_lda * (p->ml_lda + 8)));
  if (p->ml.size() == 2) {
    const int nT = p->ml_lda / kNB;
    int chunk = kDenseChunk;
    if (options().dense_chunk > 0) chunk = options().dense_chunk;
    std::vector<DenseChunk> chunks;
    std::vector<int> first(nT + 1, 0);
    for (int I = 0; I < nT; ++I) {
      first[I] = (int)chunks.size();
      for (int J0 = 0; J0 <= I; J0 += chunk) chunks.push_back(DenseChunk{I, J0, std::min(chunk, I + 1 - J0), 0});
    }
    first[nT] = (int)chunks.size();
    p->ml_nchunks = (int)chunks.size();
    CHK(upload(&p->ml_chunks, chunks.data(), chunks.size(), p->stream));
    CHK(upload(&p->ml_chunk_first, first.data(), first.size(), p->stream));
    HIPC(hipMalloc(&p->ml_packed, sizeof(double) * (size_t)nT * (nT + 1) / 2 * kNB * kNB));
    HIPC(hipMalloc(&p->ml_pd, sizeof(double) * (size_t)p->ml_nchunks * kNB * p->r));
    HIPC(hipMalloc(&p->ml_pt, sizeof(double) * (size_t)nT * p->ml_lda * p->r));
    HIPC(hipStreamSynchronize(p->stream));
  }
  HIPC(hipMalloc(&p->ml_W, sizeof(double) * (size_t)p->ml_lda * kNB));
  HIPC(hipMalloc(&p->ml_Rx, sizeof(double) * (size_t)p->ml_lda * kNB));
  HIPC(hipStreamSynchronize(p->stream));
  lap("coarser levels, dense level allocated");
  if (timing)
    std::fprintf(stderr, "dpgo_hip: symbolic set-up: %-44s %7.3f ms\n", "total",
                 1e3 * std::chrono::duration<double>(std::chrono::steady_clock::now() - t_first).count());
  p->ml_symbolic = true;
  return DPGO_OK;
}

int flat_grid(size_t items) {
  size_t g = (items + kBlock - 1) / kBlock;
  if (g < 1) g = 1;
  return g < (size_t)kMaxGrid ? (int)g : kMaxGrid;
}

bool gj_use_mfma() {
  return options().gj_mfma != 0;
}

int dense_spd_inverse(hipStream_t s, double* M, int lda, double* W, double* Rx, bool mfma) {
  const int nt = lda / kNB;
  for (int kb = 0; kb < nt; ++kb) {
    hipLaunchKernelGGL(k_sweep_panel, dim3(nt), dim3(kBlock), 0, s, M, lda, kb, W, Rx);
    if (mfma)
      hipLaunchKernelGGL(k_sweep_update<true>, dim3(nt, nt), dim3(kBlock), 0, s, M, lda, kb, W, Rx);
    else
      hipLaunchKernelGGL(k_sweep_update<false>, dim3(nt, nt), dim3(kBlock), 0, s, M, lda, kb, W, Rx);
  }
  hipLaunchKernelGGL(k_sweep_finish, dim3(nt, nt), dim3(kBlock), 0, s, M, lda);
  HIPC(hipGetLastError());
  return DPGO_OK;
}

template <int D>
int ml_numeric_setup_d(dpgo_problem_s* p) {
  const int nl = (int)p->ml.size();
  long long stride = 1;
  for (int l = 0; l + 1 < nl; ++l) {
    auto& L = p->ml[l];
    auto& C = p->ml[l + 1];
    const long long span = stride * L.k;
    const bool serial = options().ml_setup_serial != 0;
    auto wave_grid = [](int items) { return std::max(1, std::min(kMaxGrid, (items + kWaves - 1) / kWaves)); };
    if (L.graph && !serial)
      hipLaunchKernelGGL(k_ml_build_P_tree_wave<D>, dim3(wave_grid(C.n)), dim3(kBlock), 0, p->stream, p->Q.dev(), L.agg_ptr,
                         L.agg_mem, L.parent, L.pslot, L.mem_pos, L.Pb, C.n);
    else if (L.graph)
      hipLaunchKernelGGL(k_ml_build_P_tree<D>, dim3(flat_grid(C.n)), dim3(kBlock), 0, p->stream, p->Q.dev(), L.agg_ptr,
                         L.agg_mem, L.parent, L.pslot, L.Pb, C.n);
    else
      hipLaunchKernelGGL(k_ml_build_P<D>, dim3(flat_grid(C.n)), dim3(kBlock), 0, p->stream, p->Q.dev(), p->n, (int)stride,
                         (int)span, L.Pb, C.n);
    const BsrDev A = (l == 0) ? p->Q.dev() : L.A.dev();
    const bool have_ap = l == 0 && L.AP.vals;
    if (have_ap)
      hipLaunchKernelGGL(k_ml_build_AP<D>, dim3(flat_grid(L.n)), dim3(kBlock), 0, p->stream, p->Q.dev(), p->ml_shift, L.Pb,
                         L.agg(), L.n, L.AP.dev(), L.AP.vals);
    if (have_ap && !serial)
      hipLaunchKernelGGL(k_ml_galerkin_ap<D>, dim3(wave_grid(C.A.nnzb)), dim3(kBlock), 0, p->stream, L.AP.dev(), L.Pb,
                         L.agg(), L.agg_ptr, L.agg_mem, L.n, C.slot_row, C.A.colidx, C.A.vals, C.A.nnzb);
    else
      hipLaunchKernelGGL(k_ml_galerkin<D>, dim3(flat_grid(C.A.nnzb)), dim3(kBlock), 0, p->stream, A,
                         (l == 0) ? p->ml_shift : 0.0, L.Pb, L.agg(), L.agg_ptr, L.agg_mem, L.n, C.slot_row, C.A.colidx,
                         C.A.vals, C.A.nnzb);
    if (C.k)
      hipLaunchKernelGGL(k_build_dinv<D>, dim3(flat_grid(C.n)), dim3(kBlock), 0, p->stream, C.A.dev(), 0.0, C.dinv, C.n);
    stride = span;
  }
  HIPC(hipGetLastError());
  auto& Lc = p->ml.back();
  const int lda = p->ml_lda, N = Lc.n * p->b;
  HIPC(hipMemsetAsync(p->ml_dense, 0, sizeof(double) * (size_t)lda * (lda + 8), p->stream));
  hipLaunchKernelGGL(k_dense_pad_identity, dim3(1), dim3(kBlock), 0, p->stream, p->ml_dense, lda, N);
  hipLaunchKernelGGL(k_ml_dense_assemble<D>, dim3(flat_grid(Lc.A.nnzb)), dim3(kBlock), 0, p->stream, Lc.A.dev(),
                     Lc.slot_row, p->ml_dense, lda, Lc.A.nnzb);
  HIPC(hipGetLastError());
  CHK(dense_spd_inverse(p->stream, p->ml_dense, lda, p->ml_W, p->ml_Rx, gj_use_mfma()));
  if (p->ml_packed) {
    const int nT = lda / kNB;
    hipLaunchKernelGGL(k_dense_pack_lower, dim3(nT, nT), dim3(kBlock), 0, p->stream, p->ml_dense, lda, p->ml_packed);
    HIPC(hipGetLastError());
  }
  {
    const size_t total = (size_t)lda * (lda + 8);
    if (p->ml_coarse_bits == 32)
      hipLaunchKernelGGL(k_dense_round_f32, dim3(flat_grid(total)), dim3(kBlock), 0, p->stream, p->ml_dense, p->ml_dense32,
                         total);
    else
      hipLaunchKernelGGL(k_copy_f32, dim3(flat_grid(total)), dim3(kBlock), 0, p->stream, p->ml_dense, p->ml_dense32, total);
    HIPC(hipGetLastError());
  }
  return DPGO_OK;
}

int ml_numeric_setup(dpgo_problem_s* p) {
  if (!p->ml_symbolic) return fail(DPGO_ERR_STATE, "multilevel: symbolic setup missing");
  CHK(build_dinv(p, p->ml_shift));
  if (p->d == 2)
    CHK(ml_numeric_setup_d<2>(p));
  else
    CHK(ml_numeric_setup_d<3>(p));
  p->ml_ready = true;
  p->ml_ops32_ready = false;
  return DPGO_OK;
}

std::vector<int> ml_current_ks(const dpgo_problem_s* p) {
  std::vector<int> ks;
  for (size_t l = 0; l + 1 < p->ml.size(); ++l) ks.push_back(p->ml[l].graph ? -p->ml[l].k : p->ml[l].k);
  if (p->ml.size() == 2 && p->ml[0].graph && p->ml[0].merge_cap) ks.push_back(-p->ml[0].merge_cap);
  return ks;
}

int additive_tiles(const dpgo_problem_s* p) {
  const int t = p->add_tiles ? p->add_tiles : options().additive_tiles;
  return t == 2 ? 2 : 1;
}
const dpgo_problem_s::AddPlan& additive_plan(dpgo_problem_s* p) {
  if (p->add_plan_known) return p->add_plan;
  p->add_plan = dpgo_problem_s::AddPlan();
  p->add_plan_known = true;
  p->add_agg = dpgo_problem_s::AggCache();
  if (p->split != 4 || (int)p->h_rowptr.size() != p->n + 1) return p->add_plan;
  const int P4 = ml_tile(p->b, 4), P1 = ml_tile(p->b, 1), n = p->n;
  const bool graph_ok = options().ml_graph != 0;
  if (graph_ok) {
    auto& A = p->add_agg;
    auto &lab = A.lab, &ptr = A.ptr, &mem = A.mem, &parent = A.parent, &pslot = A.pslot;
    if ((long long)n <= (long long)kPersistMax * P4) {
      const int na = ml_graph_aggregates(p->h_rowptr, p->h_colidx, n, P4, lab, ptr, mem, parent, pslot);
      if (na <= kPersistMax) {
        p->add_plan = dpgo_problem_s::AddPlan{4, P4, P4, 0, na, true};
        A.S = P4, A.cap = 0;
        return p->add_plan;
      }
    }
    if ((long long)n <= (long long)kPersistMax * P1) {
      const int want = (p->persist_share > 1 && (long long)n * 10 <= (long long)(kPersistMax / 2) * P1 * 8) ? kPersistMax / 2 : kPersistMax;
      for (int S = std::max(8, (n + (want * 9) / 10 - 1) / ((want * 9) / 10)); S <= P1; S += std::max(2, S / 8)) {
        const int cap = std::min(P1, S + S / 2);
        ml_graph_aggregates(p->h_rowptr, p->h_colidx, n, S, lab, ptr, mem, parent, pslot);
        const int na = ml_merge_small_aggregates(p->h_rowptr, p->h_colidx, n, S, cap, lab, ptr, mem, parent, pslot);
        if (na <= want) {
          p->add_plan = dpgo_problem_s::AddPlan{1, P1, S, cap, na, true};
          A.S = S, A.cap = cap;
          return p->add_plan;
        }
      }
      if (want < kPersistMax) {
        for (int S = std::max(8, (n + 229) / 230); S <= P1; S += std::max(2, S / 8)) {
          const int cap = std::min(P1, S + S / 2);
          ml_graph_aggregates(p->h_rowptr, p->h_colidx, n, S, lab, ptr, mem, parent, pslot);
          const int na = ml_merge_small_aggregates(p->h_rowptr, p->h_colidx, n, S, cap, lab, ptr, mem, parent, pslot);
          if (na <= kPersistMax) {
            p->add_plan = dpgo_problem_s::AddPlan{1, P1, S, cap, na, true};
            A.S = S, A.cap = cap;
            return p->add_plan;
          }
        }
      }
    }
    p->add_agg = dpgo_problem_s::AggCache();
  }
  if ((n + P4 - 1) / P4 <= kPersistMax)
    p->add_plan = dpgo_problem_s::AddPlan{4, P4, P4, 0, (n + P4 - 1) / P4, false};
  else if ((n + P1 - 1) / P1 <= kPersistMax)
    p->add_plan = dpgo_problem_s::AddPlan{1, P1, P1, 0, (n + P1 - 1) / P1, false};
  const int P2 = 2 * P1;
  if (!p->add_plan.split && graph_ok && additive_tiles(p) == 2 && (long long)n <= (long long)kPersistMax * P2) {
    auto& A = p->add_agg;
    for (int S = std::max(8, (n + 229) / 230); S <= P2; S += std::max(2, S / 8)) {
      const int cap = std::min(P2, S + S / 2);
      ml_graph_aggregates(p->h_rowptr, p->h_colidx, n, S, A.lab, A.ptr, A.mem, A.parent, A.pslot);
      const int na = ml_merge_small_aggregates(p->h_rowptr, p->h_colidx, n, S, cap, A.lab, A.ptr, A.mem, A.parent, A.pslot);
      if (na <= kPersistMax) {
        if (!additive_lds_fits(p, 1, 2, na)) break;
        p->add_plan = dpgo_problem_s::AddPlan{1, P2, S, cap, na, true};
        A.S = S, A.cap = cap;
        return p->add_plan;
      }
    }
    p->add_agg = dpgo_problem_s::AggCache();
  }
  return p->add_plan;
}

int additive_split_of(const dpgo_problem_s* p) {
  if (!p->ml_symbolic || p->ml.size() != 2 || p->split != 4 || p->ml[1].n > kPersistMax) return 0;
  const auto& L = p->ml[0];
  const int P4 = ml_tile(p->b, 4), P1 = ml_tile(p->b, 1);
  const int tile = L.graph ? (L.tile_perm ? L.perm_tile : 0) : L.k;
  return tile == P4 ? 4 : (tile == P1 || (tile == 2 * P1 && L.graph && additive_tiles(p) == 2) ? 1 : 0);
}
int additive_mt_of(const dpgo_problem_s* p) {
  return additive_split_of(p) == 1 && p->ml[0].perm_tile == 2 * ml_tile(p->b, 1) ? 2 : 1;
}

int ml_ensure(dpgo_problem_s* p, double shift, bool additive) {
  if (additive && !additive_split_of(p)) {
    const auto& plan = additive_plan(p);
    if (!plan.split) return fail(DPGO_ERR_UNSUPPORTED, "additive preconditioner: the block does not fit 256 aggregates of one workgroup tile" +
                                                           std::string(additive_tiles(p) == 2 ? " or two" : ""));
    std::vector<int> ks{plan.graph ? -plan.S : plan.S};
    if (plan.graph && plan.cap) ks.push_back(-plan.cap);
    CHK(ml_symbolic_setup(p, ks, plan.graph ? plan.tile : 0));
    if (!additive_split_of(p)) return fail(DPGO_ERR_STATE, "additive preconditioner: hierarchy does not match its plan");
    p->ml_additive_layout = true;
    p->ml_user_ks = false;
  } else if (!additive && p->ml_additive_layout && !p->ml_user_ks) {
    CHK(ml_symbolic_setup(p, ml_default_ks(p->n, p->b, p->split)));
    p->ml_additive_layout = false;
  }
  if (p->ml_ready && p->ml_shift == shift) return build_dinv(p, shift);
  if (!p->ml_symbolic) CHK(ml_symbolic_setup(p, ml_default_ks(p->n, p->b, p->split)));
  p->ml_shift = shift;
  return ml_numeric_setup(p);
}

int ml_ops32_ensure(dpgo_problem_s* p) {
  if (!p->ml_ops32_wanted() || p->ml_ops32_ready) return DPGO_OK;
  auto& L0 = p->ml[0];
  const size_t bb = (size_t)p->b * p->b;
  const size_t nu = (size_t)p->sym.nu * bb, nap = (size_t)L0.AP.nnzb * bb, npb = (size_t)L0.n * bb;
  if (!p->sym.uvalsT32) HIPC(hipMalloc(&p->sym.uvalsT32, sizeof(float) * nu));
  if (!L0.AP32) HIPC(hipMalloc(&L0.AP32, sizeof(float) * nap));
  if (!L0.Pb32) HIPC(hipMalloc(&L0.Pb32, sizeof(float) * npb));
  if (!L0.x1f) HIPC(hipMalloc(&L0.x1f, sizeof(float) * (size_t)L0.n * p->T));
  if (!L0.res1f) HIPC(hipMalloc(&L0.res1f, sizeof(float) * (size_t)L0.n * p->T));
  auto copy = [&](const double* in, float* out, size_t total) {
    hipLaunchKernelGGL(k_copy_f32, dim3(flat_grid(total)), dim3(kBlock), 0, p->stream, in, out, total);
  };
  copy(p->sym.uvalsT, p->sym.uvalsT32, nu);
  copy(L0.AP.vals, L0.AP32, nap);
  copy(L0.Pb, L0.Pb32, npb);
  HIPC(hipGetLastError());
  p->ml_ops32_ready = true;
  return DPGO_OK;
}

int persist_capacity(int device);
int launch_coarse_prolong(dpgo_problem_s* p, const dpgo_problem_s::MlLevel& L, const dpgo_problem_s::MlLevel& C,
                          const DevState* gate, double* xc_out) {
  const bool f32 = p->coarse32_active();
  const int cus = persist_capacity(p->device) / 2;
  int nodes = C.n >= 512 ? 2 : 1;
  if (nodes == 2 && !f32 && (C.n + 1) / 2 > cus && (C.n + 2) / 3 <= cus) nodes = 3;
  if (const int v = options().coarse_nodes)
    nodes = (v == 4 || v == 2 || (v == 3 && !f32)) ? v : 1;
  const int groups = (C.n + nodes - 1) / nodes;
  int cap = kMaxGrid;
  if (options().coarse_grid > 0) cap = options().coarse_grid;
  const int rounds = (groups + cap - 1) / cap;
  const int gc = std::max(1, (groups + rounds - 1) / rounds);
  int hint = p->beyond_cache();
  if (options().coarse_nt >= 0) hint = options().coarse_nt != 0;
#define COARSE_LAUNCH(NODES, MT, MPTR)                                                                               \
  hipLaunchKernelGGL((k_ml_coarse_prolong<D, R, NODES, MT>), dim3(gc), dim3(kBlock), 0, p->stream, MPTR, p->ml_lda,   \
                     reinterpret_cast<const MT*>(C.r), L.x1, L.Pb, L.k, L.x, gate, L.n, C.n, xc_out, hint)
  DISPATCH(p->d, p->r, {
    if (nodes == 4 && f32)
      COARSE_LAUNCH(4, float, p->ml_dense32);
    else if (nodes == 4)
      COARSE_LAUNCH(4, double, p->ml_dense);
    else if (nodes == 3)
      COARSE_LAUNCH(3, double, p->ml_dense);
    else if (nodes == 2 && f32)
      COARSE_LAUNCH(2, float, p->ml_dense32);
    else if (nodes == 2)
      COARSE_LAUNCH(2, double, p->ml_dense);
    else if (f32)
      COARSE_LAUNCH(1, float, p->ml_dense32);
    else
      COARSE_LAUNCH(1, double, p->ml_dense);
  });
#undef COARSE_LAUNCH
  HIPC(hipGetLastError());
  return DPGO_OK;
}

int launch_dense_sym(dpgo_problem_s* p, const dpgo_problem_s::MlLevel& C, const DevState* gate) {
  const int N = C.n * p->b, nT = p->ml_lda / kNB;
  switch (p->r) {
#define DENSE_SYM_CASE(RR)                                                                                              \
  case RR:                                                                                                              \
    hipLaunchKernelGGL((k_dense_sym_apply<RR>), dim3(p->ml_nchunks), dim3(kBlock), 0, p->stream, p->ml_packed,          \
                       p->ml_chunks, C.r, N, p->ml_lda, p->ml_pd, p->ml_pt, gate);                                       \
    hipLaunchKernelGGL((k_dense_sym_finish<RR>), dim3(nT, 4), dim3(kBlock), 0, p->stream, p->ml_pd, p->ml_pt,            \
                       p->ml_chunk_first, nT, N, p->ml_lda, C.x, gate);                                                  \
    break;
    DENSE_SYM_CASE(2)
    DENSE_SYM_CASE(3)
    DENSE_SYM_CASE(4)
    DENSE_SYM_CASE(5)
    DENSE_SYM_CASE(6)
#undef DENSE_SYM_CASE
    default:
      return fail(DPGO_ERR_UNSUPPORTED, "unsupported r");
  }
  HIPC(hipGetLastError());
  return DPGO_OK;
}

int launch_ml_restrict0(dpgo_problem_s* p, const double* r, const DevState* gate, int g0, bool stop_check) {
  auto& L = p->ml[0];
  auto& C = p->ml[1];
  TcgStopCheck stop;
  if (stop_check && gate) {
    stop.state = const_cast<DevState*>(gate);
    stop.pin = p->pB();
    stop.nb = p->grid_u(true);
    stop.hflag = p->hflag;
    stop.gen = p->launch_gen();
  }
  float* rc32 = (C.k == 0 && p->coarse32_active()) ? reinterpret_cast<float*>(C.r) : (float*)nullptr;
  double* res_out = p->ml_use_ap() ? L.res1 : nullptr;
  const double* dnext = C.k ? C.dinv : (const double*)nullptr;
  if (p->ml_vec32_active()) {
    DISPATCH(p->d, p->r, hipLaunchKernelGGL((k_ml_restrict<D, R, 1, BsrSymDev32, float, float>), dim3(g0), dim3(kBlock), 0,
                                            p->stream, p->sym.dev32(), L.x1f, r, L.Pb32, p->ml_shift, L.k, C.r, rc32, dnext,
                                            p->ml_omega, C.x1, gate, L.n, L.res1f, L.tbuf, L.seg_info, stop));
  } else if (p->ml_ops32_active()) {
    DISPATCH(p->d, p->r, hipLaunchKernelGGL((k_ml_restrict<D, R, 1, BsrSymDev32, float, double>), dim3(g0), dim3(kBlock), 0,
                                            p->stream, p->sym.dev32(), L.x1, r, L.Pb32, p->ml_shift, L.k, C.r, rc32, dnext,
                                            p->ml_omega, C.x1, gate, L.n, res_out, L.tbuf, L.seg_info, stop));
  } else if (p->tcg_sym) {
    DISPATCH(p->d, p->r, hipLaunchKernelGGL((k_ml_restrict<D, R, 1, BsrSymDev>), dim3(g0), dim3(kBlock), 0, p->stream,
                                            p->sym.dev(), L.x1, r, L.Pb, p->ml_shift, L.k, C.r, rc32, dnext, p->ml_omega,
                                            C.x1, gate, L.n, res_out, L.tbuf, L.seg_info, stop));
  } else {
    DISPATCH(p->d, p->r, LAUNCH_SPLIT(p, k_ml_restrict, g0, p->Q.dev(), L.x1, r, L.Pb, p->ml_shift, L.k, C.r, rc32, dnext,
                                      p->ml_omega, C.x1, gate, L.n, res_out, L.tbuf, L.seg_info, stop));
  }
  if (L.graph)
    DISPATCH(p->d, p->r, hipLaunchKernelGGL((k_ml_agg_sum<D, R>), dim3(std::min(C.n, kMaxGrid)), dim3(kBlock), 0, p->stream,
                                            L.tbuf, L.seg_ptr, C.n, C.r, rc32, gate));
  HIPC(hipGetLastError());
  return DPGO_OK;
}

int launch_ml_post_ap(dpgo_problem_s* p, const double* Xdev, const double* r, double* z, double* pout, const DevState* gate) {
  auto& L0 = p->ml[0];
  if (p->ml_ops32_active()) {
    const BsrDev32 ap32{L0.AP.rowptr, L0.AP.colidx, L0.AP32};
    if (p->ml_vec32_active()) {
      DISPATCH(p->d, p->r, hipLaunchKernelGGL((k_ml_post_ap<D, R, 1, float, float>), dim3(p->grid_post()), dim3(kBlock), 0,
                                              p->stream, ap32, Xdev, r, L0.res1f, p->ml[1].x, L0.Pb32, L0.agg(), p->dinv,
                                              p->ml_omega, z, pout, gate, p->n));
    } else {
      DISPATCH(p->d, p->r, hipLaunchKernelGGL((k_ml_post_ap<D, R, 1, float, double>), dim3(p->grid_post()), dim3(kBlock), 0,
                                              p->stream, ap32, Xdev, r, L0.res1, p->ml[1].x, L0.Pb32, L0.agg(), p->dinv,
                                              p->ml_omega, z, pout, gate, p->n));
    }
    HIPC(hipGetLastError());
    return DPGO_OK;
  }
  DISPATCH(p->d, p->r, LAUNCH_SPLIT(p, k_ml_post_ap, p->grid_post(), L0.AP.dev(), Xdev, r, L0.res1, p->ml[1].x, L0.Pb,
                                    L0.agg(), p->dinv, p->ml_omega, z, pout, gate, p->n));
  HIPC(hipGetLastError());
  return DPGO_OK;
}

int launch_ml_tail(dpgo_problem_s* p, const double* Xdev, const double* r, double* z, double* pout,
                   const DevState* gate, bool stop_check) {
  const int nl = (int)p->ml.size();
  auto rc32_of = [&](const dpgo_problem_s::MlLevel& C) {
    return (C.k == 0 && p->coarse32_active()) ? reinterpret_cast<float*>(C.r) : (float*)nullptr;
  };
  auto A_of = [&](int l) { return l == 0 ? p->Q.dev() : p->ml[l].A.dev(); };
  auto r_of = [&](int l) { return l == 0 ? r : (const double*)p->ml[l].r; };
  int g0 = p->grid_restrict();
  auto grid_of = [&](const dpgo_problem_s::MlLevel& L) {
    if (&L == &p->ml[0]) return g0;
    const int P = ml_tile(p->b, L.split);
    return std::max(1, std::min(kMaxGrid, (L.n + P - 1) / P));
  };
#define ML_SPLIT_LAUNCH(L, KERNEL, ...)                                                                  \
  do {                                                                                                   \
    const int g_ = grid_of(L);                                                                           \
    if ((L).split == 4)                                                                                  \
      hipLaunchKernelGGL((KERNEL<D, R, 4>), dim3(g_), dim3(kBlock), 0, p->stream, __VA_ARGS__);          \
    else if ((L).split == 2)                                                                             \
      hipLaunchKernelGGL((KERNEL<D, R, 2>), dim3(g_), dim3(kBlock), 0, p->stream, __VA_ARGS__);          \
    else                                                                                                 \
      hipLaunchKernelGGL((KERNEL<D, R, 1>), dim3(g_), dim3(kBlock), 0, p->stream, __VA_ARGS__);          \
  } while (0)
  const bool ap = p->ml_use_ap();
  CHK(launch_ml_restrict0(p, r, gate, g0, stop_check));
  for (int l = 1; l + 1 < nl; ++l) {
    auto& L = p->ml[l];
    auto& C = p->ml[l + 1];
    DISPATCH(p->d, p->r, ML_SPLIT_LAUNCH(L, k_ml_restrict, A_of(l), L.x1, r_of(l), L.Pb, 0.0, L.k, C.r, rc32_of(C),
                                         C.k ? C.dinv : (const double*)nullptr, p->ml_omega, C.x1, gate, L.n,
                                         (double*)nullptr, (double*)nullptr, (const int32_t*)nullptr));
  }
  {
    auto& L = p->ml[nl - 2];
    auto& C = p->ml[nl - 1];
    if (p->ml_use_dense_sym())
      CHK(launch_dense_sym(p, C, gate));
    else
      CHK(launch_coarse_prolong(p, L, C, gate, ap ? C.x : nullptr));
  }
  g0 = p->grid_post();
  if (ap) return launch_ml_post_ap(p, Xdev, r, z, pout, gate);
  for (int l = nl - 2; l >= 1; --l) {
    auto& L = p->ml[l];
    auto& F = p->ml[l - 1];
    DISPATCH(p->d, p->r, ML_SPLIT_LAUNCH(L, k_ml_post_mid, L.A.dev(), L.x, L.r, L.dinv, p->ml_omega, F.x1, F.Pb, F.k, F.x,
                                         F.n, gate, L.n));
  }
  if (p->tcg_sym) {
    DISPATCH(p->d, p->r, hipLaunchKernelGGL((k_ml_post<D, R, 1, BsrSymDev>), dim3(g0), dim3(kBlock), 0, p->stream,
                                            p->sym.dev(), Xdev, p->ml[0].x, r, p->dinv, p->ml_omega, p->ml_shift, z, pout,
                                            gate, p->n));
  } else {
    DISPATCH(p->d, p->r, ML_SPLIT_LAUNCH(p->ml[0], k_ml_post, p->Q.dev(), Xdev, p->ml[0].x, r, p->dinv, p->ml_omega,
                                         p->ml_shift, z, pout, gate, p->n));
  }
#undef ML_SPLIT_LAUNCH
  HIPC(hipGetLastError());
  return DPGO_OK;
}

int launch_ml_apply(dpgo_problem_s* p, const double* Xdev, const double* v, double* z) {
  DISPATCH(p->d, p->r, hipLaunchKernelGGL((k_ml_presmooth<D, R>), dim3(p->grid()), dim3(kBlock), 0, p->stream, v, p->dinv,
                                          p->ml_omega, p->ml[0].x1, (const DevState*)nullptr, p->n));
  HIPC(hipGetLastError());
  p->ml_ops32_suspend = true;
  const int rc = launch_ml_tail(p, Xdev, v, z, nullptr, nullptr);
  p->ml_ops32_suspend = false;
  return rc;
}

}

extern "C" {


int dpgo_multilevel_default_ks(int n, int d, int* ks, int* nks) {
  if (n <= 0 || d < 2 || d > 3 || !nks) return fail(DPGO_ERR_INVALID, "bad arguments");
  int split = (n < 40000) ? 4 : 1;
  if (const int v = options().split)
    if (v == 1 || v == 2 || v == 4) split = v;
  const std::vector<int> v = ml_default_ks(n, d + 1, split);
  if (ks)
    for (size_t l = 0; l < v.size() && (int)l < *nks; ++l) ks[l] = v[l];
  *nks = (int)v.size();
  return DPGO_OK;
}


int dpgo_multilevel_graph_aggregates(int n, const int32_t* rowptr, const int32_t* colidx, int max_size, int32_t* label,
                                     int32_t* parent, int* n_aggregates) {
  if (n <= 0 || !rowptr || !colidx || max_size < 2 || !label) return fail(DPGO_ERR_INVALID, "bad arguments");
  const std::vector<int32_t> rp(rowptr, rowptr + n + 1), ci(colidx, colidx + rowptr[n]);
  for (int32_t c : ci)
    if (c < 0 || c >= n) return fail(DPGO_ERR_INVALID, "block column out of range");
  std::vector<int32_t> lab, ptr, mem, par, pslot;
  const int na = ml_graph_aggregates(rp, ci, n, max_size, lab, ptr, mem, par, pslot);
  std::copy(lab.begin(), lab.end(), label);
  if (parent) std::copy(par.begin(), par.end(), parent);
  if (n_aggregates) *n_aggregates = na;
  return DPGO_OK;
}


int dpgo_multilevel_merged_aggregates(int n, const int32_t* rowptr, const int32_t* colidx, int max_size, int merge_cap,
                                      int32_t* label, int32_t* parent, int* n_aggregates) {
  if (n <= 0 || !rowptr || !colidx || max_size < 2 || merge_cap < max_size || !label) return fail(DPGO_ERR_INVALID, "bad arguments");
  const std::vector<int32_t> rp(rowptr, rowptr + n + 1), ci(colidx, colidx + rowptr[n]);
  for (int32_t c : ci)
    if (c < 0 || c >= n) return fail(DPGO_ERR_INVALID, "block column out of range");
  std::vector<int32_t> lab, ptr, mem, par, pslot;
  ml_graph_aggregates(rp, ci, n, max_size, lab, ptr, mem, par, pslot);
  const int na = ml_merge_small_aggregates(rp, ci, n, max_size, merge_cap, lab, ptr, mem, par, pslot);
  std::copy(lab.begin(), lab.end(), label);
  if (parent) std::copy(par.begin(), par.end(), parent);
  if (n_aggregates) *n_aggregates = na;
  return DPGO_OK;
}


int dpgo_problem_additive_plan(dpgo_problem_t p, int* lane_groups, int* tile, int* growth, int* merge_cap, int* aggregates,
                               int* graph) {
  if (!p) return fail(DPGO_ERR_INVALID, "null handle");
  if ((int)p->h_rowptr.size() != p->n + 1) return fail(DPGO_ERR_STATE, "Q's block pattern is not set");
  const auto& plan = additive_plan(p);
  if (lane_groups) *lane_groups = plan.split;
  if (tile) *tile = plan.tile;
  if (growth) *growth = plan.S;
  if (merge_cap) *merge_cap = plan.cap;
  if (aggregates) *aggregates = plan.na;
  if (graph) *graph = plan.graph ? 1 : 0;
  return DPGO_OK;
}


int dpgo_problem_additive_tiles(dpgo_problem_t p, int* tiles) {
  if (!p || !tiles) return fail(DPGO_ERR_INVALID, "null handle / pointer");
  if (*tiles < 0 || *tiles > 2) return fail(DPGO_ERR_INVALID, "additive tiles: 1 or 2 (0 queries)");
  if (*tiles > 0 && *tiles != additive_tiles(p)) {
    p->add_tiles = *tiles;
    p->add_plan_known = false;
    p->add_agg = dpgo_problem_s::AggCache();
    if (p->ml_additive_layout && !p->ml_user_ks) ml_free(p);
  }
  *tiles = additive_tiles(p);
  return DPGO_OK;
}


int dpgo_problem_setup_multilevel(dpgo_problem_t p, int nks, const int* ks, double omega, double shift) {
  CHK(check_ready(p));
  if (nks < 0 || nks > 8 || (nks > 0 && !ks) || !(omega > 0.0) || !(shift >= 0.0))
    return fail(DPGO_ERR_INVALID, "bad multilevel arguments");
  std::vector<int> v = nks > 0 ? std::vector<int>(ks, ks + nks) : ml_default_ks(p->n, p->b, p->split);
  const bool same = p->ml_symbolic && ml_current_ks(p) == v;
  if (!same) {
    int perm_tile = 0;
    if (v.size() == 2 && v[0] < 0 && v[1] < 0 && p->split == 4)
      perm_tile = -v[1] <= ml_tile(p->b, 4) ? ml_tile(p->b, 4) : (-v[1] <= ml_tile(p->b, 1) ? ml_tile(p->b, 1) : 0);
    if (!perm_tile && v.size() == 2 && v[0] < 0 && v[1] < 0 && p->split == 4 && additive_tiles(p) == 2 && -v[1] <= 2 * ml_tile(p->b, 1))
      perm_tile = 2 * ml_tile(p->b, 1);
    CHK(ml_symbolic_setup(p, v, perm_tile));
  }
  p->ml_user_ks = nks > 0;
  p->ml_additive_layout = false;
  p->ml_omega = omega;
  p->ml_shift = shift;
  CHK(ml_numeric_setup(p));
  HIPC(hipStreamSynchronize(p->stream));
  return DPGO_OK;
}


int dpgo_problem_multilevel_path(dpgo_problem_t p, int* flags) {
  if (!p || !flags) return fail(DPGO_ERR_INVALID, "null handle / pointer");
  if (!p->ml_symbolic) return fail(DPGO_ERR_STATE, "multilevel hierarchy not set up");
  *flags = (p->ml_use_ap() ? DPGO_ML_PATH_AP : 0) | (p->ml_use_dense_sym() ? DPGO_ML_PATH_PACKED_DENSE : 0);
  return DPGO_OK;
}


int dpgo_problem_multilevel_coarse_bits(dpgo_problem_t p, int* bits) {
  if (!p || !bits) return fail(DPGO_ERR_INVALID, "null handle / pointer");
  if (*bits < 0) {
    *bits = p->ml_coarse_bits;
    return DPGO_OK;
  }
  if (*bits != 32 && *bits != 64) return fail(DPGO_ERR_INVALID, "the coarsest inverse is stored in 32 or 64 bits");
  if (*bits != p->ml_coarse_bits) {
    p->ml_coarse_bits = *bits;
    p->ml_ready = false;
  }
  return DPGO_OK;
}


int dpgo_problem_multilevel_operator_bits(dpgo_problem_t p, int* bits, int* active) {
  if (!p || !bits) return fail(DPGO_ERR_INVALID, "null handle / pointer");
  if (*bits >= 0) {
    if (*bits != 32 && *bits != 64) return fail(DPGO_ERR_INVALID, "the cycle's operator copies are stored in 32 or 64 bits");
    p->ml_operator_bits = *bits;
  }
  *bits = p->ml_operator_bits;
  if (active) *active = (p->ml_ops32_active() ? 1 : 0) | (p->ml_vec32_active() ? 2 : 0) | (p->coarse32_active() ? 4 : 0);
  return DPGO_OK;
}

int dpgo_problem_multilevel_info(dpgo_problem_t p, int* nlevels, int* sizes, int* ks, int* nnzb) {
  if (!p) return fail(DPGO_ERR_INVALID, "null handle");
  if (!p->ml_symbolic) return fail(DPGO_ERR_STATE, "multilevel hierarchy not set up");
  const int cap = nlevels ? *nlevels : 0;
  for (int l = 0; l < (int)p->ml.size() && l < cap; ++l) {
    if (sizes) sizes[l] = p->ml[l].n;
    if (ks) ks[l] = p->ml[l].graph ? -p->ml[l].k : p->ml[l].k;
    if (ks && l > 0 && l + 1 == (int)p->ml.size() && p->ml[0].graph && p->ml[0].merge_cap) ks[l] = -p->ml[0].merge_cap;
    if (nnzb) nnzb[l] = (l == 0) ? p->Q.nnzb : p->ml[l].A.nnzb;
  }
  if (nlevels) *nlevels = (int)p->ml.size();
  return DPGO_OK;
}


int dpgo_problem_multilevel_get(dpgo_problem_t p, int level, int what, void* out_host) {
  CHK(check_ready(p));
  if (!p->ml_ready) return fail(DPGO_ERR_STATE, "multilevel hierarchy not built");
  if (!out_host || level < 0 || level >= (int)p->ml.size()) return fail(DPGO_ERR_INVALID, "bad level / null pointer");
  auto& L = p->ml[level];
  const int bb = p->b * p->b;
  const void* src = nullptr;
  size_t bytes = 0;
  switch (what) {
    case DPGO_ML_P_BLOCKS:
      src = L.Pb, bytes = sizeof(double) * (size_t)L.n * bb;
      break;
    case DPGO_ML_A_ROWPTR:
      src = L.A.rowptr, bytes = sizeof(int32_t) * ((size_t)L.n + 1);
      break;
    case DPGO_ML_A_COLIDX:
      src = L.A.colidx, bytes = sizeof(int32_t) * (size_t)L.A.nnzb;
      break;
    case DPGO_ML_A_VALUES:
      src = L.A.vals, bytes = sizeof(double) * (size_t)L.A.nnzb * bb;
      break;
    case DPGO_ML_AGG_LABELS:
      src = L.graph ? L.lab : nullptr, bytes = sizeof(int32_t) * (size_t)L.n;
      break;
    case DPGO_ML_AP_NNZB: {
      if (!L.AP.vals) return fail(DPGO_ERR_INVALID, "this level does not hold that item");
      *static_cast<int32_t*>(out_host) = L.AP.nnzb;
      return DPGO_OK;
    }
    case DPGO_ML_RESTRICT_PARTIALS: {
      if (!L.graph) return fail(DPGO_ERR_INVALID, "this level does not hold that item");
      *static_cast<int32_t*>(out_host) = L.nseg;
      return DPGO_OK;
    }
    case DPGO_ML_DENSE_INVERSE: {
      if (level + 1 != (int)p->ml.size()) return fail(DPGO_ERR_INVALID, "the dense inverse belongs to the last level");
      const int N = L.n * p->b;
      HIPC(hipMemcpy2DAsync(out_host, sizeof(double) * N, p->ml_dense, sizeof(double) * p->ml_lda, sizeof(double) * N, N,
                            hipMemcpyDeviceToHost, p->stream));
      HIPC(hipStreamSynchronize(p->stream));
      return DPGO_OK;
    }
    default:
      return fail(DPGO_ERR_INVALID, "unknown item");
  }
  if (!src) return fail(DPGO_ERR_INVALID, "this level does not hold that item");
  HIPC(hipMemcpyAsync(out_host, src, bytes, hipMemcpyDeviceToHost, p->stream));
  HIPC(hipStreamSynchronize(p->stream));
  return DPGO_OK;
}


int dpgo_dense_spd_inverse(int N, const double* A_host, double* Ainv_host, int device, int use_mfma) {
  if (N <= 0 || N > 16384 || !A_host || !Ainv_host) return fail(DPGO_ERR_INVALID, "bad arguments");
  int cnt = 0;
  CHK(dpgo_device_count(&cnt));
  if (cnt <= 0) return fail(DPGO_ERR_HIP, "no HIP device (this library has no CPU fallback)");
  if (device < 0 || device >= cnt) return fail(DPGO_ERR_INVALID, "device index out of range");
  HIPC(hipSetDevice(device));
  const int lda = ((N + kNB - 1) / kNB) * kNB;
  TmpDev tmp;
  double *M = nullptr, *W = nullptr, *Rx = nullptr;
  CHK(tmp.alloc(&M, sizeof(double) * (size_t)lda * lda));
  CHK(tmp.alloc(&W, sizeof(double) * (size_t)lda * kNB));
  CHK(tmp.alloc(&Rx, sizeof(double) * (size_t)lda * kNB));
  HIPC(hipMemset(M, 0, sizeof(double) * (size_t)lda * lda));
  HIPC(hipMemcpy2D(M, sizeof(double) * lda, A_host, sizeof(double) * N, sizeof(double) * N, N, hipMemcpyHostToDevice));
  hipLaunchKernelGGL(k_dense_pad_identity, dim3(1), dim3(kBlock), 0, (hipStream_t) nullptr, M, lda, N);
  CHK(dense_spd_inverse(nullptr, M, lda, W, Rx, use_mfma != 0));
  HIPC(hipMemcpy2D(Ainv_host, sizeof(double) * N, M, sizeof(double) * lda, sizeof(double) * N, N, hipMemcpyDeviceToHost));
  return DPGO_OK;
}
#ifdef DPGO_TIMELINE
int dpgo_debug_timeline_cycle(long long* out ) {
  HIPC(hipDeviceSynchronize());
  HIPC(hipMemcpyFromSymbol(out, HIP_SYMBOL(g_tl_restrict), sizeof(long long) * 3 * 64));
  HIPC(hipMemcpyFromSymbol(out + 3 * 64, HIP_SYMBOL(g_tl_post), sizeof(long long) * 3 * 64));
  return DPGO_OK;
}
#endif

}
```

### dpgo_amd/csrc/solve.hip

```cpp
#include "host.h"

namespace dpgo_host {

int launch_tcg_update(dpgo_problem_s* p, const double* dinv, int first, double* z_out,
                      double ml_omega) {
  const bool ml_mode = ml_omega > 0.0;
  const int g = p->grid_u(ml_mode);
  double* zt = z_out ? z_out : p->z;
  float* z32 = (ml_omega > 0.0 && !p->ml.empty() && z_out == p->ml[0].x1 && p->ml_vec32_active()) ? p->ml[0].x1f : nullptr;
  DISPATCH(p->d, p->r, {
    if constexpr (Span<D, R, 1>::kOk) {
      if (ml_mode)
        hipLaunchKernelGGL((k_tcg_update_span<D, R, 1>), dim3(g), dim3(kBlock), 0, p->stream, p->x1, p->g1, dinv, p->delta,
                           p->Hd, p->eta, p->rr, zt, p->pA(), p->grid_s(), p->pB(), p->dstate + p->cur,
                           p->dstate + (p->cur ^ 1), first, p->n, p->hflag, p->launch_gen(), ml_omega, z32);
      else
        hipLaunchKernelGGL((k_tcg_update_span<D, R, 0>), dim3(g), dim3(kBlock), 0, p->stream, p->x1, p->g1, dinv, p->delta,
                           p->Hd, p->eta, p->rr, zt, p->pA(), p->grid_s(), p->pB(), p->dstate + p->cur,
                           p->dstate + (p->cur ^ 1), first, p->n, p->hflag, p->launch_gen(), ml_omega, z32);
    } else {
      if (z32) return fail(DPGO_ERR_STATE, "fp32 cycle vectors need the span kernels (even pose tile size)");
      hipLaunchKernelGGL((k_tcg_update<D, R>), dim3(g), dim3(kBlock), 0, p->stream, p->x1, p->g1, dinv, p->delta,
                         p->Hd, p->eta, p->rr, zt, p->pA(), p->grid_s(), p->pB(), p->dstate + p->cur,
                         p->dstate + (p->cur ^ 1), first, p->n, p->hflag, p->launch_gen(), ml_omega);
    }
  });
  HIPC(hipGetLastError());
  p->cur ^= 1;
  return DPGO_OK;
}

#define LAUNCH_TCG_HESS(p, SIN, SOUT, FIRST, HFLAG, GEN)                                                          \
  do {                                                                                                            \
    if constexpr (Span<D, R, 1>::kOk) {                                                                           \
      if ((p)->tcg_sym && options().hess_dma == 1)                                                                \
        hipLaunchKernelGGL((k_tcg_hess_sym_dma<D, R, 1, 2, 4, 1>), dim3((p)->grid_s()), dim3(kBlock), 0,          \
                           (p)->stream, (p)->sym.dev(), (p)->x1, (p)->S1, (p)->z, (p)->delta, (p)->Hd, (p)->pB(), \
                           (p)->nb_zr(), (p)->pA(), SIN, SOUT, FIRST, (p)->n, HFLAG, GEN);                         \
      else if ((p)->tcg_sym && options().hess_dma == 2)                                                           \
        hipLaunchKernelGGL((k_tcg_hess_sym_dma<D, R, 1, 3, 2, 0>), dim3((p)->grid_s()), dim3(kBlock), 0,          \
                           (p)->stream, (p)->sym.dev(), (p)->x1, (p)->S1, (p)->z, (p)->delta, (p)->Hd, (p)->pB(), \
                           (p)->nb_zr(), (p)->pA(), SIN, SOUT, FIRST, (p)->n, HFLAG, GEN);                         \
      else if ((p)->tcg_sym && (p)->stream_nt)                                                                    \
        hipLaunchKernelGGL((k_tcg_hess_sym<D, R, 1>), dim3((p)->grid_s()), dim3(kBlock), 0, (p)->stream,          \
                           (p)->sym.dev(), (p)->x1, (p)->S1, (p)->z, (p)->delta, (p)->Hd, (p)->pB(), (p)->nb_zr(), \
                           (p)->pA(), SIN, SOUT, FIRST, (p)->n, HFLAG, GEN);                                      \
      else if ((p)->tcg_sym)                                                                                      \
        hipLaunchKernelGGL((k_tcg_hess_sym<D, R, 0>), dim3((p)->grid_s()), dim3(kBlock), 0, (p)->stream,          \
                           (p)->sym.dev(), (p)->x1, (p)->S1, (p)->z, (p)->delta, (p)->Hd, (p)->pB(), (p)->nb_zr(), \
                           (p)->pA(), SIN, SOUT, FIRST, (p)->n, HFLAG, GEN);                                      \
      else if ((p)->stream_nt && (p)->split == 1)                                                                 \
        hipLaunchKernelGGL((k_tcg_hess_span<D, R, 1, 1>), dim3((p)->grid_s()), dim3(kBlock), 0, (p)->stream,      \
                           (p)->Q.dev(), (p)->x1, (p)->S1, (p)->z, (p)->delta, (p)->Hd, (p)->pB(), (p)->nb_zr(),   \
                           (p)->pA(), SIN, SOUT, FIRST, (p)->n, HFLAG, GEN);                                      \
      else                                                                                                        \
      LAUNCH_SPLIT(p, k_tcg_hess_span, (p)->grid_s(), (p)->Q.dev(), (p)->x1, (p)->S1, (p)->z, (p)->delta, (p)->Hd, \
                   (p)->pB(), (p)->nb_zr(), (p)->pA(), SIN, SOUT, FIRST, (p)->n, HFLAG, GEN);                   \
    } else                                                                                                        \
      LAUNCH_SPLIT(p, k_tcg_hess, (p)->grid_s(), (p)->Q.dev(), (p)->x1, (p)->S1, (p)->z, (p)->delta, (p)->Hd,      \
                   (p)->pB(), (p)->nb_zr(), (p)->pA(), SIN, SOUT, FIRST, (p)->n, HFLAG, GEN);                   \
  } while (0)

int launch_tcg_hess_with(dpgo_problem_s* p, const DevState* sin, DevState* sout, int first, unsigned long long* hflag,
                         unsigned gen) {
  DISPATCH(p->d, p->r, LAUNCH_TCG_HESS(p, sin, sout, first, hflag, gen));
  HIPC(hipGetLastError());
  return DPGO_OK;
}
int launch_tcg_hess(dpgo_problem_s* p, int first) {
  CHK(launch_tcg_hess_with(p, p->dstate + p->cur, p->dstate + (p->cur ^ 1), first, p->hflag, p->launch_gen()));
  p->cur ^= 1;
  return DPGO_OK;
}

int resolve_tcg_storage(dpgo_problem_s* p) {
  p->tcg_sym = false;
  p->stream_nt = p->want_stream_nt();
  bool span = false;
  DISPATCH(p->d, p->r, { span = Span<D, R, 1>::kOk; });
  if (!span || !p->sym_wanted()) return DPGO_OK;
  bool usable = false;
  CHK(sym_ensure(p, &usable));
  p->tcg_sym = usable;
  return DPGO_OK;
}

constexpr int kMaxDevices = 64;
std::atomic<int> g_warnings{0};
std::atomic<int> g_persist_used[kMaxDevices];
std::atomic<int> g_persist_cap[kMaxDevices];

int persist_capacity(int device) {
  int cap = g_persist_cap[device % kMaxDevices].load();
  if (cap == 0) {
    int cus = 0;
    if (hipDeviceGetAttribute(&cus, hipDeviceAttributeMultiprocessorCount, device) != hipSuccess || cus <= 0) cus = 1;
    cap = 2 * cus;
    g_persist_cap[device % kMaxDevices].store(cap);
  }
  return cap;
}
bool persist_reserve(dpgo_problem_s* p, int slots, int limit) {
  auto& used = g_persist_used[p->device % kMaxDevices];
  int cur = used.load();
  while (cur + slots <= limit)
    if (used.compare_exchange_weak(cur, cur + slots)) {
      p->persist_reserved = slots;
      return true;
    }
  return false;
}
void persist_release(dpgo_problem_s* p) {
  if (p->persist_reserved > 0) g_persist_used[p->device % kMaxDevices].fetch_sub(p->persist_reserved);
  p->persist_reserved = 0;
}

bool additive_available(dpgo_problem_s* p) {
  return p->persist && !p->persist_failed_once && additive_plan(p).split != 0;
}
constexpr size_t kPersistLds = 160 * 1024;
bool additive_lds_fits(const dpgo_problem_s* p, int split, int mt, int na) {
  hipFuncAttributes a{};
  bool ok = false;
  auto query = [&]() -> int {
    DISPATCH(p->d, p->r, {
      const void* f = split == 4 ? reinterpret_cast<const void*>(&k_rtr_persist<D, R, 4, 1, true>)
                                 : mt == 2 ? reinterpret_cast<const void*>(&k_rtr_persist<D, R, 1, 2, true>)
                                           : reinterpret_cast<const void*>(&k_rtr_persist<D, R, 1, 1, true>);
      ok = hipFuncGetAttributes(&a, f) == hipSuccess;
    });
    return DPGO_OK;
  };
  if (query() != DPGO_OK || !ok) return false;
  return a.sharedSizeBytes + sizeof(double) * (size_t)p->b * p->b * na <= kPersistLds;
}
PersistGeo persist_geometry(const dpgo_problem_s* p, int free_slots, int share, bool additive) {
  if (additive) {
    const int sp = additive_split_of(p);
    if (!sp) return PersistGeo();
    PersistGeo g{sp, additive_mt_of(p), p->ml[1].n, 0};
    if (g.mt == 2 && !additive_lds_fits(p, sp, g.mt, g.wgs)) return PersistGeo();
    g.slots = g.wgs * persist_slots_per_wg(sp, 1, true);
    if (g.wgs > kPersistMax || g.slots > free_slots) return PersistGeo();
    return g;
  }
  const int env_split = options().persist_split, env_mt = options().persist_mt;
  const int cand[4][2] = {{4, 1}, {4, 2}, {1, 1}, {1, 2}};
  PersistGeo compact;
  for (auto& c : cand) {
    if (env_split && c[0] != env_split) continue;
    if (env_mt && c[1] != env_mt) continue;
    const int P = (64 / (p->b * c[0])) * kWaves;
    const int tiles = std::max(1, (p->n + P - 1) / P);
    const int wgs = (tiles + c[1] - 1) / c[1];
    const int slots = wgs * persist_slots_per_wg(c[0], c[1]);
    if (wgs > kPersistMax || slots > free_slots) continue;
    const PersistGeo g{c[0], c[1], wgs, slots};
    if ((long long)slots * std::max(1, share) <= free_slots) return g;
    if (compact.wgs == 0 || slots < compact.slots) compact = g;
  }
  return compact;
}

int launch_rtr_persistent(dpgo_problem_s* p, const dpgo_ropt_params* prm, const double* dinv, bool* used, bool additive) {
  *used = false;
  p->gen += 1;
  if (p->persist_stream_ordered) {
    const PersistGeo g = persist_geometry(p, persist_capacity(p->device), 1, additive);
    if (g.wgs <= 0) return DPGO_OK;
    p->persist_split = g.split;
    p->persist_mt = g.mt;
    p->persist_wgs = g.wgs;
    p->persist_add = additive;
  } else if (p->persist_reserved == 0) {
    const int cap = persist_capacity(p->device);
    auto& used = g_persist_used[p->device % kMaxDevices];
    PersistGeo g;
    if (p->persist_share <= 1) {
      g = persist_geometry(p, cap - used.load(), 1, additive);
      if (g.wgs <= 0 || !persist_reserve(p, g.slots, cap)) return DPGO_OK;
    } else {
      const int limit = additive ? cap : cap - cap / 5;
      g = persist_geometry(p, limit, p->persist_share, additive);
      if (g.wgs <= 0) return DPGO_OK;
      const auto t0 = std::chrono::steady_clock::now();
      while (!persist_reserve(p, g.slots, limit)) {
        if (std::chrono::duration<double>(std::chrono::steady_clock::now() - t0).count() > 0.05) return DPGO_OK;
        std::this_thread::yield();
      }
    }
    p->persist_split = g.split;
    p->persist_mt = g.mt;
    p->persist_wgs = g.wgs;
    p->persist_add = additive;
  }
  if (p->pctrl_dirty) {
    HIPC(hipMemsetAsync(p->pctrl, 0, sizeof(PersistCtrl), p->stream));
    p->pctrl_dirty = false;
  }
  if (p->gen - p->gran_cleared_at >= 0x7ffu) {
    HIPC(hipMemsetAsync(p->pgran, 0, sizeof(unsigned long long) * kGranWords, p->stream));
    p->gran_cleared_at = p->gen;
  }
  const unsigned salt = ((p->gen & 0x7ffu) + 1u) << 20;
  const int env_first = options().poll_first, env_sleep = options().poll_sleep;
  const int first = env_first >= 0 ? std::min(255, env_first)
                                   : (p->persist_split == 4 ? (p->persist_wgs <= 160 ? kPollFirstSleep : 30) : 32);
  const int between = env_sleep >= 0 ? std::min(255, env_sleep) : kPollSleep;
  const int env_first_pay = options().poll_first_pay;
  const int first_pay = env_first_pay >= 0 ? std::min(255, env_first_pay) : kPollFirstPaySleep;
  const int poll = (first_pay << 16) | (first << 8) | between;

  AddDev add{};
  size_t lds = 0;
  if (additive) {
    auto& L0 = p->ml[0];
    auto& C = p->ml[1];
    add = AddDev{L0.Pb, p->ml_dense, p->ml_lda, C.n, C.r, 1.0, L0.graph ? L0.tile_perm : nullptr,
                 L0.graph ? L0.lab : nullptr, L0.graph ? L0.mem_pos : nullptr, L0.graph ? L0.agg_ptr : nullptr};
    lds = sizeof(double) * (size_t)p->b * C.n * p->b;
  }
  const RtrArgs ra{prm->gradnorm_tol, prm->RTR_initial_radius, 5.0 * prm->RTR_initial_radius, prm->RTR_tCG_iterations,
                   prm->RTR_iterations, prm->accept_tiny_decrease};
  const double* Glin = p->has_G ? p->G : nullptr;
#define PERSIST_LAUNCH(SP, MT_, ADD_, LDS_)                                                                           \
  do {                                                                                                                \
    if ((LDS_) > 0) {               \
      static std::atomic<int> hw_[kMaxDevices];                                                                       \
      auto& h_ = hw_[p->device % kMaxDevices];                                                                        \
      if ((int)(LDS_) > h_.load()) {                                                                                  \
        HIPC(hipFuncSetAttribute(reinterpret_cast<const void*>(&k_rtr_persist<D, R, SP, MT_, ADD_>),                   \
                                 hipFuncAttributeMaxDynamicSharedMemorySize, (int)(LDS_)));                           \
        int cur_ = h_.load();                                                                                         \
        while (cur_ < (int)(LDS_) && !h_.compare_exchange_weak(cur_, (int)(LDS_))) {}                                 \
      }                                                                                                               \
    }                                                                                                                 \
    hipLaunchKernelGGL((k_rtr_persist<D, R, SP, MT_, ADD_>), dim3(p->persist_wgs), dim3(kBlock), LDS_, p->stream,     \
                       p->Q.dev(), p->x1, Glin, dinv, p->x2, p->eta, p->z, p->pgran, salt, p->dstate, p->pctrl, p->n, \
                       p->hflag, p->gen, poll, ra, add);                                                              \
  } while (0)
  DISPATCH(p->d, p->r, {
    if (additive && p->persist_split == 4) PERSIST_LAUNCH(4, 1, true, lds);
    else if (additive && p->persist_mt == 2) PERSIST_LAUNCH(1, 2, true, lds);
    else if (additive) PERSIST_LAUNCH(1, 1, true, lds);
    else if (p->persist_split == 4 && p->persist_mt == 1) PERSIST_LAUNCH(4, 1, false, 0);
    else if (p->persist_split == 4) PERSIST_LAUNCH(4, 2, false, 0);
    else if (p->persist_mt == 1) PERSIST_LAUNCH(1, 1, false, 0);
    else PERSIST_LAUNCH(1, 2, false, 0);
  });
#undef PERSIST_LAUNCH
  {
    const size_t count = (size_t)p->n * p->T;
    const int grid = (int)std::min<size_t>(1024, (count + kBlock - 1) / kBlock);
    hipLaunchKernelGGL(k_persist_commit, dim3(grid), dim3(kBlock), 0, p->stream, p->dstate, p->pctrl, p->x2, p->x1, count,
                       p->hstate, p->hctrl);
  }
  HIPC(hipGetLastError());
  p->cur = 0;
  *used = true;
  return DPGO_OK;
}

void persist_report(dpgo_problem_s* p) {
  if (!options().persist_verbose) return;
  const double it = std::max<double>(1.0, (double)p->hctrl->ticks[4]);
  std::fprintf(stderr,
               "dpgo_hip: persistent tCG: %u workgroups (%d lane groups per pose, %d tiles each)%s, %u iterations; per "
               "iteration (us): Hessian phase %.2f, all-reduce %.2f, update phase %.2f, all-reduce %.2f; per solve (us): "
               "set-up + initial statistics %.1f, first updates %.1f, retraction / trial point / rho test %.1f\n",
               p->hctrl->members, p->persist_split, p->persist_mt, p->hctrl->error ? " TIMED OUT" : "", p->hctrl->iters,
               0.01 * (double)p->hctrl->ticks[0] / it, 0.01 * (double)p->hctrl->ticks[1] / it,
               0.01 * (double)p->hctrl->ticks[2] / it, 0.01 * (double)p->hctrl->ticks[3] / it,
               0.01 * (double)p->hctrl->ticks[5], 0.01 * (double)p->hctrl->ticks[6], 0.01 * (double)p->hctrl->ticks[7]);
}

struct KeyHash {
  unsigned long long h = 1469598103934665603ull;
  void add(const void* ptr) { mix((unsigned long long)(uintptr_t)ptr); }
  void add(long long v) { mix((unsigned long long)v); }
  void add(double v) {
    unsigned long long u;
    std::memcpy(&u, &v, sizeof(u));
    mix(u);
  }
  void mix(unsigned long long v) {
    for (int k = 0; k < 8; ++k) {
      h ^= (v >> (8 * k)) & 0xffull;
      h *= 1099511628211ull;
    }
  }
};
void key_bsr(KeyHash& k, const Bsr& m) {
  k.add((long long)m.nrows), k.add((long long)m.ncols), k.add((long long)m.nnzb);
  k.add(m.rowptr), k.add(m.colidx), k.add(m.vals);
}
unsigned long long iter_graph_key(const dpgo_problem_s* p, const double* dinv, bool ml, bool early_stop) {
  KeyHash k;
  k.add((long long)p->d), k.add((long long)p->r), k.add((long long)p->n), k.add((long long)p->split), k.add((long long)p->cur);
  k.add((long long)p->tcg_sym), k.add((long long)p->stream_nt), k.add((long long)ml), k.add((long long)early_stop);
  k.add((long long)p->grid()), k.add((long long)p->grid_u(true)), k.add((long long)p->grid_s()), k.add((long long)p->grid_restrict()), k.add((long long)p->grid_post());
  k.add((long long)p->zr_from_post), k.add((long long)p->nb_zr()), k.add((long long)p->device);
  key_bsr(k, p->Q);
  const auto& y = p->sym;
  k.add(y.urow), k.add(y.ucol), k.add(y.uvalsT), k.add(y.lrow), k.add(y.lcol), k.add(y.lslot), k.add(y.tord);
  const void* vecs[] = {p->x1, p->g1, p->S1, p->z, p->delta, p->Hd, p->eta, p->rr, dinv, p->dinv, p->partials, p->dstate, p->hflag};
  for (auto v : vecs) k.add(v);
  if (!ml) return k.h;
  k.add(p->ml_omega), k.add(p->ml_shift), k.add((long long)p->ml_coarse_bits), k.add((long long)p->ml_lda);
  k.add((long long)p->ml_use_ap()), k.add((long long)p->ml_use_dense_sym()), k.add((long long)p->beyond_cache());
  k.add(p->ml_dense), k.add(p->ml_dense32), k.add(p->ml_packed), k.add(p->ml_pd), k.add(p->ml_pt), k.add(p->ml_chunks);
  k.add(p->ml_chunk_first), k.add((long long)p->ml_nchunks), k.add((long long)p->ml.size());
  k.add((long long)p->ml_ops32_active()), k.add((long long)p->ml_vec32_active()), k.add((long long)p->coarse32_active());
  k.add(p->sym.uvalsT32);
  for (const auto& L : p->ml) {
    k.add((long long)L.n), k.add((long long)L.k), k.add((long long)L.split), k.add((long long)L.graph), k.add((long long)L.nseg);
    key_bsr(k, L.A), key_bsr(k, L.AP);
    const void* ptrs[] = {L.slot_row, L.dinv, L.Pb, L.r, L.x1, L.x, L.res1, L.lab, L.agg_ptr, L.agg_mem, L.parent, L.pslot,
                          L.mem_pos, L.seg_info, L.seg_ptr, L.tile_perm, L.tbuf, L.Pb32, L.AP32, L.x1f, L.res1f};
    for (auto v : ptrs) k.add(v);
  }
  return k.h;
}

int rtr_outer_iteration(dpgo_problem_s* p, const dpgo_ropt_params* prm, const double* dinv, Counters& cnt,
                        bool poll_at_end) {
  p->gen += 1;
  const bool add = prm->precond == DPGO_PRECOND_ADDITIVE;
  const bool ml = prm->precond == DPGO_PRECOND_MULTILEVEL || add;
  p->zr_from_post = ml;
  if (add) cnt.vcycle_for_additive = true;
  auto update = [&](int first) -> int {
    if (ml) {
      CHK(launch_tcg_update(p, dinv, first, p->ml[0].x1, p->ml_omega));
      const bool early_stop = options().ml_early_stop != 0;
      return launch_ml_tail(p, p->x1, p->rr, p->z, p->pB(), p->dstate + p->cur, early_stop && !first);
    }
    return launch_tcg_update(p, dinv, first);
  };
  CHK(update(1));
  const int max_inner = prm->RTR_tCG_iterations;
  const bool graph_wanted = options().iter_graph != 0, early_stop_ = options().ml_early_stop != 0;
  const bool use_graph = graph_wanted && !p->iter_graph_failed && prm->tcg_poll_interval <= 0 && max_inner > 1 && p->own_stream;
  auto replay = [&]() -> int {
    auto& g = p->iter_graph[p->cur & 1];
    const unsigned long long key = iter_graph_key(p, dinv, ml, early_stop_);
    if (!g.exec || g.key != key) {
      if (g.exec) (void)hipGraphExecDestroy(g.exec);
      g.exec = nullptr;
      hipStream_t own = p->own_stream, keep = p->stream;
      const int cur0 = p->cur;
      if (keep == own) HIPC(hipStreamSynchronize(own));
      if (hipStreamBeginCapture(own, hipStreamCaptureModeThreadLocal) != hipSuccess) {
        (void)hipGetLastError();
        p->iter_graph_failed = true;
        return DPGO_ERR_UNSUPPORTED;
      }
      p->stream = own;
      p->capturing = true;
      int rc = launch_tcg_hess(p, 0);
      if (rc == DPGO_OK) rc = update(0);
      p->capturing = false;
      p->stream = keep;
      p->cur = cur0;
      hipGraph_t graph = nullptr;
      const hipError_t e1 = hipStreamEndCapture(own, &graph);
      hipError_t e2 = hipSuccess;
      if (rc == DPGO_OK && e1 == hipSuccess && graph) e2 = hipGraphInstantiate(&g.exec, graph, nullptr, nullptr, 0);
      if (graph) (void)hipGraphDestroy(graph);
      if (rc != DPGO_OK || e1 != hipSuccess || e2 != hipSuccess || !g.exec) {
        (void)hipGetLastError();
        g.exec = nullptr;
        p->iter_graph_failed = true;
        return DPGO_ERR_UNSUPPORTED;
      }
      g.key = key;
    }
    if (hipGraphLaunch(g.exec, p->stream) != hipSuccess) {
      (void)hipGetLastError();
      p->iter_graph_failed = true;
      return DPGO_ERR_UNSUPPORTED;
    }
    return DPGO_OK;
  };
  auto step = [&](int j) -> int {
    if (j >= 1 && use_graph && !p->iter_graph_failed) {
      if (replay() == DPGO_OK) return DPGO_OK;
      if (options().persist_verbose) std::fprintf(stderr, "dpgo_hip: hipGraph replay of a tCG iteration unavailable; plain launches\n");
    }
    CHK(launch_tcg_hess(p, j == 0 ? 1 : 0));
    return update(0);
  };
  if (max_inner <= 0) CHK(launch_tcg_hess(p, 1));
  bool done = false;
  if (prm->tcg_poll_interval > 0) {
    const int poll = prm->tcg_poll_interval;
    int j = 0;
    while (j < max_inner) {
      const int chunk = (max_inner - j) < poll ? (max_inner - j) : poll;
      for (int c = 0; c < chunk; ++c) CHK(step(j + c));
      j += chunk;
      CHK(poll_state(p));
      if (p->hstate->tcg_done || p->hstate->rtr_stop) {
        done = true;
        break;
      }
    }
  } else {
    int kAhead = ml ? 2 : 4;
    if (options().tcg_ahead > 0) kAhead = std::max(2, options().tcg_ahead);
    int enq = 0, last_j = -1;
    auto t_progress = std::chrono::steady_clock::now();
    while (true) {
      const unsigned long long w = __atomic_load_n(p->hflag, __ATOMIC_ACQUIRE);
      int dev_j = 0;
      if ((unsigned)(w >> 32) == p->gen) {
        dev_j = (int)((w >> 8) & 0xFFFFFFu);
        if (w & 3ull) {
          done = true;
          if (w & 2ull) p->saw_rtr_stop = true;
          break;
        }
      }
      if (enq >= max_inner) break;
      if (dev_j != last_j) {
        last_j = dev_j;
        t_progress = std::chrono::steady_clock::now();
      }
      if (enq < dev_j + kAhead) {
        CHK(step(enq));
        enq += 1;
      } else {
        __builtin_ia32_pause();
        if (std::chrono::duration<double>(std::chrono::steady_clock::now() - t_progress).count() > 60.0) {
          HIPC(hipStreamSynchronize(p->stream));
          return fail(DPGO_ERR_HIP, "tCG progress word did not advance for 60 s");
        }
      }
    }
  }
  if (!done) CHK(launch_tcg_hess(p, 0));
  if (p->saw_rtr_stop) return DPGO_OK;
  CHK(launch_retract(p, p->x1, p->eta, 1.0, p->x2, p->dstate + p->cur));
  CHK(launch_grad(p, p->x2, p->g2, p->S2, nullptr, p->dstate + p->cur, p->tcg_sym && outer_sym_enabled()));
  cnt.spmm += 1;
  CHK(launch_hess(p, p->x1, p->S1, p->eta, p->g1, p->Hd, p->pH(), p->dstate + p->cur, 0, p->tcg_sym && outer_sym_enabled()));
  cnt.spmm += 1;
  CHK(launch_rtr_update(p));
  if (poll_at_end) CHK(poll_state(p));
  return DPGO_OK;
}

constexpr int kAutoUnitsJacobi = 10, kAutoUnitsAdditive = 13, kAutoSetupUnits = 2800, kAutoMinProducts = 6;
constexpr int kAutoUnitsAdditive2 = 22;
int auto_units_jacobi(dpgo_problem_s* p) {
  const int share = std::max(1, p->persist_share);
  if (share == 1 || !p->persist) return kAutoUnitsJacobi;
  const int cap = persist_capacity(p->device), limit = cap - cap / 5;
  const PersistGeo g = persist_geometry(p, limit, share, false);
  if (g.wgs <= 0) return kAutoUnitsJacobi;
  const double part = std::max((double)g.slots / limit, 1.0 / share);
  const double two_tiles = g.mt == 2 ? (g.split == 1 ? 2.1 : 1.25) : 1.0;
  return std::max(1, (int)std::lround(kAutoUnitsJacobi * two_tiles * part * share));
}
int auto_units_additive(dpgo_problem_s* p) {
  const int share = std::max(1, p->persist_share);
  const int units = p->add_plan.tile == 2 * ml_tile(p->b, 1) ? kAutoUnitsAdditive2 : kAutoUnitsAdditive;
  if (share == 1) return units;
  const int cap = persist_capacity(p->device);
  const double part = std::max((double)(p->add_plan.na * persist_slots_per_wg(p->add_plan.split, 1, true)) / cap, 1.0 / share);
  return std::max(1, (int)std::lround(units * part * share));
}
void auto_update(dpgo_problem_s* p, const dpgo_ropt_params* prm, int used, int products) {
  const int budget = std::max(1, prm->RTR_iterations) * std::max(1, prm->RTR_tCG_iterations);
  const bool coupled = p->has_G || p->C.nnzb > 0;
  auto& a = p->auto_cost;
  a.last_used = used;
  a.last_products = products;
  if (!coupled) {
    if (!p->auto_ml && 2 * products >= budget) p->auto_ml = true;
    return;
  }
  const bool cost_rule = options().auto_cost_rule != 0;
  if (!p->auto_ml) {
    a.state = 0;
    a.uj = auto_units_jacobi(p);
    a.jac_units += (long long)kAutoUnitsJacobi * products;
    const bool binds = 2 * products >= budget;
    const bool paid = cost_rule && products >= kAutoMinProducts && a.jac_units >= ((long long)kAutoSetupUnits << a.backoff);
    if (binds || paid) {
      const bool add = cost_rule && !p->ml_user_ks && additive_available(p);
      if (add) a.ua = auto_units_additive(p);
      const bool hopeless = add && !binds && (long long)a.ua * kAutoMinProducts >= (long long)a.uj * products;
      if (hopeless) {
        a.jac_units = 0;
        a.backoff = std::min(a.backoff + 1, 6);
      } else if (binds || add) {
        p->auto_ml = true;
        if (add) {
          a.state = 1;
          a.ref = products;
          a.switches += 1;
        }
      }
    }
    return;
  }
  if (a.state == 0) {
    if (10 * products <= budget) p->auto_ml = false;
    return;
  }
  a.ua = auto_units_additive(p);
  const long long cost = (long long)a.ua * products * 100, ref = (long long)a.uj * a.ref * (a.state == 2 ? 115 : 100);
  if (cost < ref) {
    a.state = 2;
  } else {
    p->auto_ml = false;
    a.state = 0;
    a.jac_units = 0;
    a.backoff = std::min(a.backoff + 1, 6);
  }
}

int run_optimize(dpgo_problem_s* p, const dpgo_ropt_params* prm, dpgo_ropt_result* res, int phase) {
  auto t0 = std::chrono::steady_clock::now();
  Counters cnt;
  std::memset(res, 0, sizeof(*res));
  res->tCGStatus = DPGO_TCG_MAXITER;
  const bool resume = phase == RUN_END;
  if (p->hctrl && !resume) std::memset(p->hctrl, 0, sizeof(PersistCtrl));
  struct SlotGuard {
    dpgo_problem_s* p;
    bool armed;
    ~SlotGuard() {
      if (armed) persist_release(p);
    }
  } slot_guard{p, true};
  dpgo_ropt_params resolved = resume ? p->pending.resolved : *prm;
  if (!resume) {
    if (prm->precond == DPGO_PRECOND_AUTO) p->auto_decide();
    if (prm->precond == DPGO_PRECOND_AUTO)
      resolved.precond = (p->auto_ml && prm->method == DPGO_METHOD_RTR)
                             ? ((additive_available(p) && !p->ml_user_ks) ? DPGO_PRECOND_ADDITIVE : DPGO_PRECOND_MULTILEVEL)
                             : DPGO_PRECOND_BLOCK_JACOBI;
  }
  const bool is_auto = resume ? p->pending.is_auto : prm->precond == DPGO_PRECOND_AUTO;
  if (resume) t0 = p->pending.t0;
  prm = &resolved;
  const double* dinv = nullptr;
  if (resume) {
    dinv = p->pending.dinv;
  } else
  if (prm->precond == DPGO_PRECOND_BLOCK_JACOBI) {
    CHK(build_dinv(p, prm->precond_shift));
    dinv = p->dinv;
  } else if (prm->precond == DPGO_PRECOND_MULTILEVEL) {
    CHK(ml_ensure(p, prm->precond_shift));
    dinv = p->dinv;
  } else if (prm->precond == DPGO_PRECOND_ADDITIVE) {
    if (prm->method != DPGO_METHOD_RTR) return fail(DPGO_ERR_UNSUPPORTED, "the additive preconditioner exists inside the tCG loop only");
    if (!additive_split_of(p) && !additive_plan(p).split)
      return fail(DPGO_ERR_UNSUPPORTED, "additive preconditioner: block too large (at most 256 aggregates of one workgroup tile, " +
                                            std::to_string(ml_tile(p->b, 1)) + " poses" +
                                            (additive_tiles(p) == 2 ? ", or of two" : "; dpgo_problem_additive_tiles: two") + ")");
    CHK(ml_ensure(p, prm->precond_shift, true));
    dinv = p->dinv;
  } else if (prm->precond != DPGO_PRECOND_NONE) {
    return fail(DPGO_ERR_INVALID, "unknown preconditioner");
  }
  if (!resume) {
    p->loop_extra_bytes = 0;
    if (prm->precond == DPGO_PRECOND_MULTILEVEL && !p->ml.empty()) {
      const size_t nd = (size_t)p->ml_lda;
      size_t bytes = nd * nd * (size_t)(p->ml_coarse_bits / 8) / (p->ml_use_dense_sym() ? 2 : 1);
      const auto& L0 = p->ml[0];
      bytes += (size_t)L0.AP.nnzb * (sizeof(double) * p->b * p->b + sizeof(int32_t)) + sizeof(double) * (size_t)p->n * p->b * p->b;
      bytes += 3 * p->vec_bytes();
      p->loop_extra_bytes = bytes;
    }
    CHK(resolve_tcg_storage(p));
    if (prm->precond == DPGO_PRECOND_MULTILEVEL) CHK(ml_ops32_ensure(p));
  }
  const bool add = prm->precond == DPGO_PRECOND_ADDITIVE;
  const bool epochs_fit = (long long)std::max(1, prm->RTR_iterations) * (3LL * std::max(0, prm->RTR_tCG_iterations) + 4) + 1 < (1LL << 20);
  if (resume || (prm->method == DPGO_METHOD_RTR && prm->RTR_iterations != 1 && prm->tcg_poll_interval <= 0 && p->persist && epochs_fit &&
                 !p->persist_failed_once && (add || prm->precond == DPGO_PRECOND_BLOCK_JACOBI || prm->precond == DPGO_PRECOND_NONE))) {
    bool used = resume;
    if (!resume) CHK(launch_rtr_persistent(p, prm, dinv, &used, add));
    if (used) {
      if (!resume) {
        if (phase == RUN_BEGIN) {
          auto& pd = p->pending;
          pd.launched = true;
          pd.resolved = resolved;
          pd.is_auto = is_auto;
          pd.dinv = dinv;
          pd.t0 = t0;
          slot_guard.armed = false;
          return DPGO_OK;
        }
      }
      HIPC(hipStreamSynchronize(p->stream));
      persist_report(p);
      if (p->hstate->rtr_stop != kPersistPoison && !p->hctrl->error) {
        const DevState& h = *p->hstate;
        res->fInit = h.fInit;
        res->gradNormInit = h.gnInit;
        res->fOpt = h.f1;
        res->gradNormOpt = h.ngf;
        res->tCGStatus = h.outer_iter > 0 ? h.tcg_status : DPGO_TCG_MAXITER;
        res->rtr_iterations = h.outer_iter;
        res->rtr_accepted = h.n_accept;
        res->latest_step_accepted = h.accepted_last;
        res->tcg_iterations = h.n_hess;
        res->precond_used = prm->precond;
        res->spmm_count = 1 + 2 * h.outer_iter + h.n_hess;
        if (is_auto) auto_update(p, prm, prm->precond, h.n_hess);
        res->success = 1;
        res->elapsedMs = 1e3 * std::chrono::duration<double>(std::chrono::steady_clock::now() - t0).count();
        return DPGO_OK;
      }
      p->persist_failed_once = true;
// ... 529 lines not shown
```

Baseline: 261.7 it/s.

## Fuse graph-aggregate restriction into one kernel with per-aggregate work items

```diff
diff --git a/dpgo_amd/csrc/host.h b/dpgo_amd/csrc/host.h
--- a/dpgo_amd/csrc/host.h
+++ b/dpgo_amd/csrc/host.h
@@ -206,12 +206,14 @@
     bool graph = false;
     int32_t *lab = nullptr, *agg_ptr = nullptr, *agg_mem = nullptr, *parent = nullptr, *pslot = nullptr;
     int32_t* mem_pos = nullptr;
-    int32_t *seg_info = nullptr, *seg_ptr = nullptr;
-    int nseg = 0;
+    struct ItemPlan {
+      int4* dev = nullptr;
+      int n = 0, S = 1, grid = 1;
+      int lo[9] = {0, 0, 0, 0, 0, 0, 0, 0, 0};
+    } items1, items2;
     int32_t* tile_perm = nullptr;
     int perm_tile = 0;
     int merge_cap = 0;
-    double* tbuf = nullptr;
     float *Pb32 = nullptr, *AP32 = nullptr;
     float *x1f = nullptr, *res1f = nullptr;
     AggMap agg() const { return AggMap{graph ? lab : nullptr, k}; }
@@ -620,6 +622,8 @@
                           const DevState* gate, double* xc_out = nullptr);
 int launch_dense_sym(dpgo_problem_s* p, const dpgo_problem_s::MlLevel& C, const DevState* gate);
 int launch_ml_restrict0(dpgo_problem_s* p, const double* r, const DevState* gate, int g0, bool stop_check = false);
+const dpgo_problem_s::MlLevel::ItemPlan& ml_restrict_plan(const dpgo_problem_s* p);
+inline size_t ml_rc_stride(int na, int T) { return ((size_t)na * T + 1) & ~(size_t)1; }
 int launch_ml_post_ap(dpgo_problem_s* p, const double* Xdev, const double* r, double* z, double* pout, const DevState* gate);
 int launch_ml_tail(dpgo_problem_s* p, const double* Xdev, const double* r, double* z, double* pout,
                    const DevState* gate, bool stop_check = false);
diff --git a/dpgo_amd/csrc/kernels/multilevel.h b/dpgo_amd/csrc/kernels/multilevel.h
--- a/dpgo_amd/csrc/kernels/multilevel.h
+++ b/dpgo_amd/csrc/kernels/multilevel.h
@@ -45,6 +45,27 @@
   unsigned long long* hflag = nullptr;
   unsigned gen = 0;
 };
+__device__ __forceinline__ void tcg_stop_check(const TcgStopCheck& stop, double* red) {
+  double rr_sum[1];
+  load_partials<1>(stop.pin, stop.nb, rr_sum, red);
+  if (threadIdx.x == 0) {
+    const DevState* st = stop.state;
+    const double norm_r = sqrt(rr_sum[0]), nr0 = st->norm_r0, theta = st->theta, kappa = st->kappa;
+    const double pw = (theta == 1.0) ? nr0 : pow(nr0, theta);
+    const int j = st->tcg_j;
+    if (j >= st->min_inner && norm_r <= nr0 * (pw < kappa ? pw : kappa)) {
+      stop.state->tcg_status = (kappa < pw) ? TCG_LCON : TCG_SCON;
+      stop.state->tcg_done = 1;
+      if (stop.hflag) {
+        const unsigned g_ = stop.gen ? stop.gen : (unsigned)st->pad0;
+        const unsigned long long w = ((unsigned long long)g_ << 32) |
+                                     ((unsigned long long)((unsigned)j & 0xFFFFFFu) << 8) | 1ull;
+        __hip_atomic_store(stop.hflag, w, __ATOMIC_RELAXED, __HIP_MEMORY_SCOPE_SYSTEM);
+      }
+    }
+  }
+  __syncthreads();
+}
 template <int D, int R, int SPLIT>
 struct RestrictWaves {
   static constexpr int kMin = (SPLIT == 1 && D == 3 && R <= 5) ? DPGO_RESTRICT_WAVES : 1;
@@ -57,8 +78,6 @@
                                                         const double* __restrict__ dinv_next, double omega,
                                                         double* __restrict__ x1c, const DevState* gate,
                                                         int n, XT* __restrict__ res_out = nullptr,
-                                                        double* __restrict__ tbuf = nullptr,
-                                                        const int32_t* __restrict__ tpos = nullptr,
                                                         TcgStopCheck stop = TcgStopCheck()) {
   using GEO = Geo<D, R, SPLIT>;
   DPGO_TL_TILES_DECL;
@@ -69,27 +88,7 @@
   const LaneId L = lane_id<D, SPLIT>();
   const int ntiles = (n + GEO::P - 1) / GEO::P;
   const TileIter ti_ = tile_iter(ntiles);
-  if (stop.state && blockIdx.x == gridDim.x - 1) {
-    double rr_sum[1];
-    load_partials<1>(stop.pin, stop.nb, rr_sum, &t_s[0][0]);
-    if (threadIdx.x == 0) {
-      const DevState* st = stop.state;
-      const double norm_r = sqrt(rr_sum[0]), nr0 = st->norm_r0, theta = st->theta, kappa = st->kappa;
-      const double pw = (theta == 1.0) ? nr0 : pow(nr0, theta);
-      const int j = st->tcg_j;
-      if (j >= st->min_inner && norm_r <= nr0 * (pw < kappa ? pw : kappa)) {
-        stop.state->tcg_status = (kappa < pw) ? TCG_LCON : TCG_SCON;
-        stop.state->tcg_done = 1;
-        if (stop.hflag) {
-          const unsigned g_ = stop.gen ? stop.gen : (unsigned)st->pad0;
-          const unsigned long long w = ((unsigned long long)g_ << 32) |
-                                       ((unsigned long long)((unsigned)j & 0xFFFFFFu) << 8) | 1ull;
-          __hip_atomic_store(stop.hflag, w, __ATOMIC_RELAXED, __HIP_MEMORY_SCOPE_SYSTEM);
-        }
-      }
-    }
-    __syncthreads();
-  }
+  if (stop.state && blockIdx.x == gridDim.x - 1) tcg_stop_check(stop, &t_s[0][0]);
   DPGO_STAMP_AT_IN(g_tl_restrict, 1);
   for (int tk = ti_.first; tk < ti_.last; tk += ti_.step) {
     DPGO_STAMP_TILE_IN(g_tl_restrict, 0);
@@ -152,27 +151,6 @@
       store_col<R>(&t_s[lp][L.c * R], t);
     }
     DPGO_STAMP_TILE_IN(g_tl_restrict, 3);
-    if (tbuf) {
-      wave_sync();
-      if (ok) {
-        const int info = tpos[i];
-        if (info >= 0) {
-          const int len = info & 31;
-          double acc[R];
-#pragma unroll
-          for (int a = 0; a < R; ++a) acc[a] = t_s[lp][L.c * R + a];
-          for (int m = 1; m < len; ++m) {
-#pragma unroll
-            for (int a = 0; a < R; ++a) acc[a] += t_s[lp + m][L.c * R + a];
-          }
-          store_col<R>(tbuf + (size_t)(info >> 5) * GEO::T + L.c * R, acc);
-        }
-      }
-      wave_sync();
-      DPGO_STAMP_TILE_IN(g_tl_restrict, 4);
-      DPGO_TILE_NEXT;
-      continue;
-    }
     __syncthreads();
     const int mstep = (k >= 16) ? 8 : 1;
     if (mstep == 8) {
@@ -220,31 +198,115 @@
   }
 }
 
-template <int D, int R>
-__global__ __launch_bounds__(kBlock) void k_ml_agg_sum(const double* __restrict__ t, const int32_t* __restrict__ agg_ptr,
-                                                       int na, double* __restrict__ rc, float* __restrict__ rc32,
-                                                       const DevState* __restrict__ gate) {
-  constexpr int T = (D + 1) * R, NG = kBlock / T;
+struct MlItems {
+  const int4* item;
+  int n;
+  int S;
+  int stride;
+  int lo[9];
+};
+__device__ __forceinline__ TileIter item_iter(const MlItems& it) {
+  TileIter ti;
+  const int G = gridDim.x;
+  if (G < 16 || it.n < 16) {
+    ti.first = blockIdx.x;
+    ti.last = it.n;
+    ti.step = G;
+    return ti;
+  }
+  const int x = blockIdx.x & 7;
+  ti.first = it.lo[x] + (blockIdx.x >> 3);
+  ti.last = it.lo[x + 1];
+  ti.step = (G - x + 7) >> 3;
+  return ti;
+}
+template <int D, int R, int SPLIT, class MAT = BsrDev, class PT = double, class XT = double>
+__global__ __launch_bounds__(kBlock) __attribute__((amdgpu_waves_per_eu(RestrictWaves<D, R, SPLIT>::kMin, 8))) void k_ml_restrict_agg(
+    MAT A, const XT* __restrict__ x1, const double* __restrict__ r, const PT* __restrict__ Pb, double shift,
+    const int32_t* __restrict__ agg_mem, MlItems it, double* __restrict__ rc, float* __restrict__ rc32,
+    const DevState* gate, int n, XT* __restrict__ res_out, TcgStopCheck stop) {
+  using GEO = Geo<D, R, SPLIT>;
+  constexpr int SEG = 8;
+  static_assert(GEO::T * SEG <= kBlock, "one thread per (value, segment)");
+  DPGO_TL_TILES_DECL;
   if (gate && (gate->tcg_done || gate->rtr_stop)) return;
-  __shared__ double part[NG][T];
-  const int e = threadIdx.x % T, g = threadIdx.x / T;
-  for (int a = blockIdx.x; a < na; a += gridDim.x) {
-    const int m0 = agg_ptr[a], m1 = agg_ptr[a + 1];
-    if (g < NG) {
-      double acc = 0.0;
-#pragma unroll 8
-      for (int m = m0 + g; m < m1; m += NG) acc += t[(size_t)m * T + e];
-      part[g][e] = acc;
-    }
+  DPGO_STAMP_ENTRY_IN(g_tl_restrict);
+  __shared__ double res_s[kWaves][GEO::G][GEO::T];
+  __shared__ double t_s[GEO::P][GEO::T];
+  __shared__ double seg_s[SEG][GEO::T];
+  const LaneId L = lane_id<D, SPLIT>();
+  if (stop.state && blockIdx.x == gridDim.x - 1) tcg_stop_check(stop, &t_s[0][0]);
+  DPGO_STAMP_AT_IN(g_tl_restrict, 1);
+  const TileIter ii = item_iter(it);
+  const int lp = L.wave * GEO::G + L.g;
+  for (int w = ii.first; w < ii.last; w += ii.step) {
+    const int4 item = it.item[w];
+    const int a = item.x, m0 = item.y, cnt = item.z, slice = item.w & 1;
+    double acc[R];
+#pragma unroll
+    for (int q = 0; q < R; ++q) acc[q] = 0.0;
+    for (int c0 = 0; c0 < cnt; c0 += GEO::P) {
+      DPGO_STAMP_TILE_IN(g_tl_restrict, 0);
+      const bool okp = (L.g < GEO::G) && (c0 + lp < cnt);
+      const bool ok = okp && (L.s == 0);
+      const int i = okp ? agg_mem[m0 + c0 + lp] : 0;
+      const size_t off = (size_t)i * GEO::T + L.c * R;
+      double h[R];
+      q_gather<D, R, SPLIT>(A, x1, i, L.s, L.c, okp, h);
+      DPGO_TL_USE(h[0]);
+      DPGO_STAMP_TILE_IN(g_tl_restrict, 1);
+      if (ok) {
+        XT xr[R];
+        double rr[R];
+#pragma unroll
+        for (int q = 0; q < R; ++q) xr[q] = x1[off + q];
+        load_col<R>(r + off, rr);
+#pragma unroll
+        for (int q = 0; q < R; ++q) h[q] = rr[q] - h[q] - shift * (double)xr[q];
+        store_col<R>(&res_s[L.wave][L.g][L.c * R], h);
+        if (res_out) store_col_t<R>(res_out + off, h);
+      }
+      wave_sync();
+      DPGO_STAMP_TILE_IN(g_tl_restrict, 2);
+      if (ok) {
+        const PT* __restrict__ pb = Pb + (size_t)i * GEO::BB;
+        double t[R];
+#pragma unroll
+        for (int q = 0; q < R; ++q) t[q] = 0.0;
+#pragma unroll
+        for (int cc = 0; cc < GEO::B; ++cc) {
+          const double pv = (double)pb[cc * GEO::B + L.c];
+#pragma unroll
+          for (int q = 0; q < R; ++q) t[q] = fma(pv, res_s[L.wave][L.g][cc * R + q], t[q]);
+        }
+#pragma unroll
+        for (int q = 0; q < R; ++q) acc[q] += t[q];
+      }
+      wave_sync();
+      DPGO_STAMP_TILE_IN(g_tl_restrict, 3);
+      DPGO_TILE_NEXT;
+    }
+    if (L.s == 0 && L.g < GEO::G) store_col<R>(&t_s[lp][L.c * R], acc);
     __syncthreads();
-    if (threadIdx.x < T) {
-      double acc = part[0][threadIdx.x];
-#pragma unroll
-      for (int q = 1; q < NG; ++q) acc += part[q][threadIdx.x];
-      if (rc32)
-        rc32[(size_t)a * T + threadIdx.x] = (float)acc;
-      else
-        rc[(size_t)a * T + threadIdx.x] = acc;
+    if (threadIdx.x < GEO::T * SEG) {
+      const int e = threadIdx.x % GEO::T, sg = threadIdx.x / GEO::T;
+      const int s0 = sg * GEO::P / SEG, s1 = (sg + 1) * GEO::P / SEG;
+      double sum = t_s[s0][e];
+      for (int q = s0 + 1; q < s1; ++q) sum += t_s[q][e];
+      seg_s[sg][e] = sum;
+    }
+    __syncthreads();
+    if (threadIdx.x < GEO::T) {
+      const int e = threadIdx.x;
+      double sum = seg_s[0][e];
+#pragma unroll
+      for (int sg = 1; sg < SEG; ++sg) sum += seg_s[sg][e];
+      if (rc32) {
+        rc32[(size_t)a * GEO::T + e] = (float)sum;
+      } else {
+        rc[(size_t)slice * it.stride + (size_t)a * GEO::T + e] = sum;
+        if (it.S == 2 && (item.w & 2)) rc[(size_t)it.stride + (size_t)a * GEO::T + e] = 0.0;
+      }
     }
     __syncthreads();
   }
@@ -263,7 +325,7 @@
                                                               const double* __restrict__ Pb, int k,
                                                               double* __restrict__ x, const DevState* __restrict__ gate,
                                                               int n, int nc, double* __restrict__ xc_out = nullptr,
-                                                              int stream_hint = 1) {
+                                                              int stream_hint = 1, int rc_stride = 0) {
   constexpr int B = D + 1, T = B * R, BB = B * B, NR = NODES * B;
   constexpr int CPL = 16 / (int)sizeof(MT);
   struct alignas(16) Pack {
@@ -310,11 +372,20 @@
             dbl2 raw[R];
 #pragma unroll
             for (int q = 0; q < R; ++q) raw[q] = rc2[(size_t)j * R + q];
+            if (rc_stride) {
+              dbl2 raw1[R];
+#pragma unroll
+              for (int q = 0; q < R; ++q) raw1[q] = rc2[(size_t)(rc_stride / 2) + (size_t)j * R + q];
+#pragma unroll
+              for (int q = 0; q < R; ++q) raw[q] += raw1[q];
+            }
             __builtin_memcpy(&rp, raw, sizeof(rp));
           } else {
 #pragma unroll
-            for (int e = 0; e < CPL * R; ++e)
-              rp.v[e] = (CPL * j + e / R < N) ? rc[(size_t)(CPL * j) * R + e] : (MT)0;
+            for (int e = 0; e < CPL * R; ++e) {
+              const size_t at = (size_t)(CPL * j) * R + e;
+              rp.v[e] = (CPL * j + e / R < N) ? (rc_stride ? rc[at] + rc[(size_t)rc_stride + at] : rc[at]) : (MT)0;
+            }
           }
           double rv[CPL * R];
 #pragma unroll
diff --git a/dpgo_amd/csrc/multilevel.hip b/dpgo_amd/csrc/multilevel.hip
--- a/dpgo_amd/csrc/multilevel.hip
+++ b/dpgo_amd/csrc/multilevel.hip
@@ -54,8 +54,8 @@
   for (auto& L : p->ml) {
     free_bsr(L.A);
     free_bsr(L.AP);
-    void* ptrs[] = {L.slot_row, L.dinv, L.Pb, L.r, L.x1, L.x, L.res1, L.lab, L.agg_ptr, L.agg_mem, L.parent, L.pslot, L.tbuf, L.tile_perm, L.mem_pos,
-                    L.seg_info, L.seg_ptr, L.Pb32, L.AP32, L.x1f, L.res1f};
+    void* ptrs[] = {L.slot_row, L.dinv, L.Pb, L.r, L.x1, L.x, L.res1, L.lab, L.agg_ptr, L.agg_mem, L.parent, L.pslot, L.tile_perm, L.mem_pos,
+                    L.items1.dev, L.items2.dev, L.Pb32, L.AP32, L.x1f, L.res1f};
     for (void* q : ptrs)
       if (q) (void)hipFree(q);
   }
@@ -371,27 +371,34 @@
   }, arow, acol);
 }
 
-int ml_run_table(const std::vector<int32_t>& lab, int n, int na, int G, std::vector<int32_t>& seg_info,
-                 std::vector<int32_t>& seg_ptr) {
-  seg_info.assign(n, -1);
-  seg_ptr.assign(na + 1, 0);
-  int nruns = 0;
-  for (int i = 0; i < n;) {
-    int j = i + 1;
-    while (j < n && j % G != 0 && lab[j] == lab[i]) ++j;
-    seg_info[i] = j - i;
-    seg_ptr[lab[i] + 1] += 1;
-    ++nruns;
-    i = j;
-  }
-  for (int a = 0; a < na; ++a) seg_ptr[a + 1] += seg_ptr[a];
-  std::vector<int32_t> next(seg_ptr.begin(), seg_ptr.end() - 1);
-  for (int i = 0; i < n;) {
-    const int len = seg_info[i];
-    seg_info[i] = len + 32 * next[lab[i]]++;
-    i += len;
-  }
-  return nruns;
+void ml_item_plan(const std::vector<int32_t>& ptr, const std::vector<int32_t>& mem, int n, int P, int S,
+                  std::vector<int4>& items, dpgo_problem_s::MlLevel::ItemPlan& plan) {
+  const int na = (int)ptr.size() - 1;
+  std::vector<std::vector<int4>> eighth(8);
+  for (int a = 0; a < na; ++a) {
+    const int m0 = ptr[a], cnt = ptr[a + 1] - m0, tiles = (cnt + P - 1) / P, root = mem[m0];
+    int x = 7;
+    while (x > 0 && (int)((long long)n * x / 8) > root) --x;
+    if (S == 2 && tiles >= 2) {
+      const int first = std::min(cnt, (tiles + 1) / 2 * P);
+      eighth[x].push_back(make_int4(a, m0, first, 0));
+      eighth[x].push_back(make_int4(a, m0 + first, cnt - first, 1));
+    } else {
+      eighth[x].push_back(make_int4(a, m0, cnt, S == 2 ? 2 : 0));
+    }
+  }
+  items.clear();
+  int most = 0;
+  for (int x = 0; x < 8; ++x) {
+    std::stable_sort(eighth[x].begin(), eighth[x].end(), [](const int4& u, const int4& v) { return u.z > v.z; });
+    plan.lo[x] = (int)items.size();
+    items.insert(items.end(), eighth[x].begin(), eighth[x].end());
+    most = std::max(most, (int)eighth[x].size());
+  }
+  plan.lo[8] = (int)items.size();
+  plan.n = (int)items.size();
+  plan.S = S;
+  plan.grid = std::max(1, plan.n < 16 ? plan.n : 8 * most);
 }
 
 int ml_symbolic_setup(dpgo_problem_s* p, const std::vector<int>& ks_in, int perm_tile) {
@@ -435,7 +442,6 @@
       const int nthreads = setup_threads();
       JobGuard alloc_job{TaskPool::get().submit(1, [&, dev_](int) {
         hipError_t e = hipSetDevice(dev_);
-        if (e == hipSuccess) e = hipMalloc(&L.tbuf, tb * cur);
         if (e == hipSuccess) e = hipMalloc(&L.res1, tb * cur);
         if (e == hipSuccess) e = hipMalloc(&L.Pb, sizeof(double) * (size_t)cur * bb);
         if (e == hipSuccess) e = hipMalloc(&L.x1, tb * cur);
@@ -488,10 +494,12 @@
       for (int m = 0; m < cur; ++m) mpos[mem[m]] = m;
       CHK(upload(&L.mem_pos, mpos.data(), mpos.size(), p->stream));
       lap("labels, members, trees uploaded");
-      std::vector<int32_t> seg_info, seg_ptr;
-      L.nseg = ml_run_table(lab, cur, na, 64 / (b * L.split), seg_info, seg_ptr);
-      CHK(upload(&L.seg_info, seg_info.data(), seg_info.size(), p->stream));
-      CHK(upload(&L.seg_ptr, seg_ptr.data(), seg_ptr.size(), p->stream));
+      for (int S = 1; S <= 2; ++S) {
+        auto& plan = (S == 1) ? L.items1 : L.items2;
+        std::vector<int4> items;
+        ml_item_plan(ptr, mem, cur, ml_tile(b, L.split), S, items, plan);
+        CHK(upload(&plan.dev, items.data(), items.size(), p->stream));
+      }
       std::vector<int32_t> tperm;
       if (!perm_tile && !merge_cap && L.k == additive_tile(p)) perm_tile = L.k;
       if (perm_tile) {
@@ -502,7 +510,7 @@
         CHK(upload(&L.tile_perm, tperm.data(), tperm.size(), p->stream));
         L.perm_tile = perm_tile;
       }
-      lap("run table, tile table");
+      lap("item plans, tile table");
       TaskPool::get().wait(pattern_job.job);
       lap("patterns of A P and of the dense level joined");
       CHK(upload_bsr(L.AP, cur, na, (int)acol.size(), b, arow.data(), acol.data(), nullptr, p->stream));
@@ -529,7 +537,7 @@
         for (int t = rowptr[i]; t < rowptr[i + 1]; ++t) srow[t] = i;
       CHK(upload(&L.slot_row, srow.data(), srow.size(), p->stream));
       HIPC(hipStreamSynchronize(p->stream));
-      HIPC(hipMalloc(&L.r, tb * cur));
+      HIPC(hipMalloc(&L.r, p->ml[0].graph ? sizeof(double) * 2 * ml_rc_stride(cur, p->T) : tb * cur));
       if (!L.k) HIPC(hipMalloc(&L.x, tb * cur));
     }
     if (l == 0 && L.k) {
@@ -842,6 +850,7 @@
 int launch_coarse_prolong(dpgo_problem_s* p, const dpgo_problem_s::MlLevel& L, const dpgo_problem_s::MlLevel& C,
                           const DevState* gate, double* xc_out) {
   const bool f32 = p->coarse32_active();
+  const int rc_stride = (L.graph && ml_restrict_plan(p).S == 2) ? (int)ml_rc_stride(C.n, p->T) : 0;
   const int cus = persist_capacity(p->device) / 2;
   int nodes = C.n >= 512 ? 2 : 1;
   if (nodes == 2 && !f32 && (C.n + 1) / 2 > cus && (C.n + 2) / 3 <= cus) nodes = 3;
@@ -856,7 +865,7 @@
   if (options().coarse_nt >= 0) hint = options().coarse_nt != 0;
 #define COARSE_LAUNCH(NODES, MT, MPTR)                                                                               \
   hipLaunchKernelGGL((k_ml_coarse_prolong<D, R, NODES, MT>), dim3(gc), dim3(kBlock), 0, p->stream, MPTR, p->ml_lda,   \
-                     reinterpret_cast<const MT*>(C.r), L.x1, L.Pb, L.k, L.x, gate, L.n, C.n, xc_out, hint)
+                     reinterpret_cast<const MT*>(C.r), L.x1, L.Pb, L.k, L.x, gate, L.n, C.n, xc_out, hint, rc_stride)
   DISPATCH(p->d, p->r, {
     if (nodes == 4 && f32)
       COARSE_LAUNCH(4, float, p->ml_dense32);
@@ -901,6 +910,12 @@
   return DPGO_OK;
 }
 
+const dpgo_problem_s::MlLevel::ItemPlan& ml_restrict_plan(const dpgo_problem_s* p) {
+  const auto& L = p->ml[0];
+  const bool two = p->ml.size() == 2 && !p->ml_use_dense_sym() && !p->coarse32_active() && L.items2.dev;
+  return two ? L.items2 : L.items1;
+}
+
 int launch_ml_restrict0(dpgo_problem_s* p, const double* r, const DevState* gate, int g0, bool stop_check) {
   auto& L = p->ml[0];
   auto& C = p->ml[1];
@@ -914,26 +929,48 @@
   }
   float* rc32 = (C.k == 0 && p->coarse32_active()) ? reinterpret_cast<float*>(C.r) : (float*)nullptr;
   double* res_out = p->ml_use_ap() ? L.res1 : nullptr;
+  if (L.graph) {
+    const auto& plan = ml_restrict_plan(p);
+    MlItems it;
+    it.item = plan.dev, it.n = plan.n, it.S = plan.S, it.stride = (int)ml_rc_stride(C.n, p->T);
+    for (int x = 0; x < 9; ++x) it.lo[x] = plan.lo[x];
+    const int g = options().grid_ml > 0 ? std::min(plan.grid, p->cap_restrict) : plan.grid;
+    if (p->ml_vec32_active()) {
+      DISPATCH(p->d, p->r, hipLaunchKernelGGL((k_ml_restrict_agg<D, R, 1, BsrSymDev32, float, float>), dim3(g), dim3(kBlock),
+                                              0, p->stream, p->sym.dev32(), L.x1f, r, L.Pb32, p->ml_shift, L.agg_mem, it, C.r,
+                                              rc32, gate, L.n, L.res1f, stop));
+    } else if (p->ml_ops32_active()) {
+      DISPATCH(p->d, p->r, hipLaunchKernelGGL((k_ml_restrict_agg<D, R, 1, BsrSymDev32, float, double>), dim3(g), dim3(kBlock),
+                                              0, p->stream, p->sym.dev32(), L.x1, r, L.Pb32, p->ml_shift, L.agg_mem, it, C.r,
+                                              rc32, gate, L.n, res_out, stop));
+    } else if (p->tcg_sym) {
+      DISPATCH(p->d, p->r, hipLaunchKernelGGL((k_ml_restrict_agg<D, R, 1, BsrSymDev>), dim3(g), dim3(kBlock), 0, p->stream,
+                                              p->sym.dev(), L.x1, r, L.Pb, p->ml_shift, L.agg_mem, it, C.r, rc32, gate, L.n,
+                                              res_out, stop));
+    } else {
+      DISPATCH(p->d, p->r, LAUNCH_SPLIT(p, k_ml_restrict_agg, g, p->Q.dev(), L.x1, r, L.Pb, p->ml_shift, L.agg_mem, it, C.r,
+                                        rc32, gate, L.n, res_out, stop));
+    }
+    HIPC(hipGetLastError());
+    return DPGO_OK;
+  }
   const double* dnext = C.k ? C.dinv : (const double*)nullptr;
   if (p->ml_vec32_active()) {
     DISPATCH(p->d, p->r, hipLaunchKernelGGL((k_ml_restrict<D, R, 1, BsrSymDev32, float, float>), dim3(g0), dim3(kBlock), 0,
                                             p->stream, p->sym.dev32(), L.x1f, r, L.Pb32, p->ml_shift, L.k, C.r, rc32, dnext,
-                                            p->ml_omega, C.x1, gate, L.n, L.res1f, L.tbuf, L.seg_info, stop));
+                                            p->ml_omega, C.x1, gate, L.n, L.res1f, stop));
   } else if (p->ml_ops32_active()) {
     DISPATCH(p->d, p->r, hipLaunchKernelGGL((k_ml_restrict<D, R, 1, BsrSymDev32, float, double>), dim3(g0), dim3(kBlock), 0,
                                             p->stream, p->sym.dev32(), L.x1, r, L.Pb32, p->ml_shift, L.k, C.r, rc32, dnext,
-                                            p->ml_omega, C.x1, gate, L.n, res_out, L.tbuf, L.seg_info, stop));
+                                            p->ml_omega, C.x1, gate, L.n, res_out, stop));
   } else if (p->tcg_sym) {
     DISPATCH(p->d, p->r, hipLaunchKernelGGL((k_ml_restrict<D, R, 1, BsrSymDev>), dim3(g0), dim3(kBlock), 0, p->stream,
                                             p->sym.dev(), L.x1, r, L.Pb, p->ml_shift, L.k, C.r, rc32, dnext, p->ml_omega,
-                                            C.x1, gate, L.n, res_out, L.tbuf, L.seg_info, stop));
+                                            C.x1, gate, L.n, res_out, stop));
   } else {
     DISPATCH(p->d, p->r, LAUNCH_SPLIT(p, k_ml_restrict, g0, p->Q.dev(), L.x1, r, L.Pb, p->ml_shift, L.k, C.r, rc32, dnext,
-                                      p->ml_omega, C.x1, gate, L.n, res_out, L.tbuf, L.seg_info, stop));
-  }
-  if (L.graph)
-    DISPATCH(p->d, p->r, hipLaunchKernelGGL((k_ml_agg_sum<D, R>), dim3(std::min(C.n, kMaxGrid)), dim3(kBlock), 0, p->stream,
-                                            L.tbuf, L.seg_ptr, C.n, C.r, rc32, gate));
+                                      p->ml_omega, C.x1, gate, L.n, res_out, stop));
+  }
   HIPC(hipGetLastError());
   return DPGO_OK;
 }
@@ -991,7 +1028,7 @@
     auto& C = p->ml[l + 1];
     DISPATCH(p->d, p->r, ML_SPLIT_LAUNCH(L, k_ml_restrict, A_of(l), L.x1, r_of(l), L.Pb, 0.0, L.k, C.r, rc32_of(C),
                                          C.k ? C.dinv : (const double*)nullptr, p->ml_omega, C.x1, gate, L.n,
-                                         (double*)nullptr, (double*)nullptr, (const int32_t*)nullptr));
+                                         (double*)nullptr));
   }
   {
     auto& L = p->ml[nl - 2];
@@ -1214,7 +1251,7 @@
     }
     case DPGO_ML_RESTRICT_PARTIALS: {
       if (!L.graph) return fail(DPGO_ERR_INVALID, "this level does not hold that item");
-      *static_cast<int32_t*>(out_host) = L.nseg;
+      *static_cast<int32_t*>(out_host) = ml_restrict_plan(p).S * p->ml[1].n;
       return DPGO_OK;
     }
     case DPGO_ML_DENSE_INVERSE: {
diff --git a/dpgo_amd/csrc/solve.hip b/dpgo_amd/csrc/solve.hip
--- a/dpgo_amd/csrc/solve.hip
+++ b/dpgo_amd/csrc/solve.hip
@@ -313,10 +313,10 @@
   k.add((long long)p->ml_ops32_active()), k.add((long long)p->ml_vec32_active()), k.add((long long)p->coarse32_active());
   k.add(p->sym.uvalsT32);
   for (const auto& L : p->ml) {
-    k.add((long long)L.n), k.add((long long)L.k), k.add((long long)L.split), k.add((long long)L.graph), k.add((long long)L.nseg);
+    k.add((long long)L.n), k.add((long long)L.k), k.add((long long)L.split), k.add((long long)L.graph), k.add((long long)L.items1.n), k.add((long long)L.items2.n);
     key_bsr(k, L.A), key_bsr(k, L.AP);
     const void* ptrs[] = {L.slot_row, L.dinv, L.Pb, L.r, L.x1, L.x, L.res1, L.lab, L.agg_ptr, L.agg_mem, L.parent, L.pslot,
-                          L.mem_pos, L.seg_info, L.seg_ptr, L.tile_perm, L.tbuf, L.Pb32, L.AP32, L.x1f, L.res1f};
+                          L.mem_pos, L.items1.dev, L.items2.dev, L.tile_perm, L.Pb32, L.AP32, L.x1f, L.res1f};
     for (auto v : ptrs) k.add(v);
   }
   return k.h;
```

New measurement: 255.7 it/s (median of 2 runs). -2.3%, worse.
